# ducha-aiki/affnet

Hardware: AMD Instinct MI355X
Metric: keypoints/sec (detect+AffNet+OriNet+HardNet) per image, 2000 kp @1024x768 (higher is better)
Workload: dtype f32

## Files before the change

affnet_amd/_lib.py:

```python
import ctypes as C
import os

_HERE = os.path.dirname(os.path.abspath(__file__))
LIB_PATH = os.environ.get("AFFNET_HIP_LIB") or os.path.join(_HERE, "libaffnet_hip.so")
PROBES_LIB_PATH = os.path.join(_HERE, "libaffnet_hip_probes.so")

MAX_OCTAVES, MAX_LEVELS, MAX_TAPS = 16, 8, 37
NET_AFFNET, NET_ORINET, NET_HARDNET, NET_AFFNET_FULLCONV = 0, 1, 2, 3
ARITH_FP32_MFMA, ARITH_FP32_SPLIT3, ARITH_FP32_SPLIT2H = 0, 1, 2
ARITH_NAMES = {"fp32": ARITH_FP32_MFMA, "fp32_mfma": ARITH_FP32_MFMA, "fp32_split3": ARITH_FP32_SPLIT3, "split3": ARITH_FP32_SPLIT3,
               "fp32_split2h": ARITH_FP32_SPLIT2H, "split2h": ARITH_FP32_SPLIT2H}


def arith_code(arith):
    if arith is None:
        return ARITH_FP32_MFMA
    if isinstance(arith, str):
        if arith.lower() not in ARITH_NAMES:
            raise ValueError("arith must be one of %s" % sorted(ARITH_NAMES))
        return ARITH_NAMES[arith.lower()]
    if int(arith) not in (ARITH_FP32_MFMA, ARITH_FP32_SPLIT3, ARITH_FP32_SPLIT2H):
        raise ValueError("arith must be AFFNET_ARITH_FP32_MFMA (0), AFFNET_ARITH_FP32_SPLIT3 (1) or AFFNET_ARITH_FP32_SPLIT2H (2)")
    return int(arith)
SHAPE_FORM_DIRECT, SHAPE_FORM_WINOGRAD = 0, 1
DESC_FORM_DIRECT, DESC_FORM_POLYPHASE, DESC_FORM_F43 = 0, 1, 2
OK, ERR_INVALID, ERR_HIP, ERR_CAPACITY, ERR_EMPTY = 0, -1, -2, -3, -4


class Config(C.Structure):
    _fields_ = [
        ("height", C.c_int32), ("width", C.c_int32), ("n_octaves", C.c_int32), ("levels_per_octave", C.c_int32),
        ("oct_h", C.c_int32 * MAX_OCTAVES), ("oct_w", C.c_int32 * MAX_OCTAVES),
        ("level_sigma", (C.c_float * MAX_LEVELS) * MAX_OCTAVES),
        ("level_sigma4", (C.c_float * MAX_LEVELS) * MAX_OCTAVES),
        ("level_sigma_px", (C.c_double * MAX_LEVELS) * MAX_OCTAVES),
        ("first_blur_taps", C.c_int32), ("first_blur", C.c_float * (MAX_TAPS * MAX_TAPS)),
        ("level_blur_taps", C.c_int32 * MAX_LEVELS),
        ("level_blur", (C.c_float * (MAX_TAPS * MAX_TAPS)) * MAX_LEVELS),
        ("level_blur0_taps", C.c_int32 * MAX_LEVELS),
        ("level_blur0", (C.c_float * (MAX_TAPS * MAX_TAPS)) * MAX_LEVELS),
        ("lazy_shape_rows", C.c_int32),
        ("onepass", C.c_int32),
        ("mr_size", C.c_float), ("threshold", C.c_float),
        ("num_features", C.c_int32), ("num_prefilter", C.c_int32),
        ("max_raw_per_octave_div", C.c_int32), ("max_keep", C.c_int32), ("batch", C.c_int32), ("baum_iters", C.c_int32),
        ("arith", C.c_int32),
    ]


class Nets(C.Structure):
    _fields_ = [("d_affnet", C.c_void_p), ("d_orinet", C.c_void_p), ("d_hardnet", C.c_void_p),
                ("h_orientation_window", C.c_void_p), ("h_baumberg_window", C.c_void_p)]


_P, _I, _SZ = C.c_void_p, C.c_int, C.c_size_t
SYMBOLS = {
    "affnet_config_fill": (_I, [C.POINTER(Config), _I, _I, _I, C.c_double, _I, C.c_double, C.c_double, _I, _I, _I, _I]),
    "affnet_ctx_create": (_I, [C.POINTER(_P), _I, C.POINTER(Config)]),
    "affnet_ctx_destroy": (None, [_P]),
    "affnet_last_error": (C.c_char_p, [_P]),
    "affnet_version": (C.c_char_p, []),
    "affnet_set_arith": (_I, [_P, _I]),
    "affnet_get_arith": (_I, [_P]),
    "affnet_set_shape_form": (_I, [_P, _I]),
    "affnet_get_shape_form": (_I, [_P]),
    "affnet_set_desc_form": (_I, [_P, _I]),
    "affnet_get_desc_form": (_I, [_P]),
    "affnet_workspace_bytes": (_SZ, [_P]),
    "affnet_bind_workspace": (_I, [_P, _P, _SZ]),
    "affnet_pyramid_level_offset": (C.c_int64, [_P, _I, _I]),
    "affnet_pyramid_image_stride": (C.c_int64, [_P]),
    "affnet_batch": (_I, [_P]),
    "affnet_capacity_prefilter": (_I, [_P]),
    "affnet_capacity_final": (_I, [_P]),
    "affnet_gauss_blur": (_I, [_P, _P, _P, _I, _I, C.POINTER(C.c_float), _I, _P]),
    "affnet_pyramid_build": (_I, [_P, _P, _P]),
    "affnet_hessian_response": (_I, [_P, _P, _P, _I, _I, C.c_float, _P]),
    "affnet_detect": (_I, [_P, _P, _P, _P, _P, _P]),
    "affnet_detect_responses": (_I, [_P, _P, _P, _P, _P, _P, _P]),
    "affnet_laf_grid_sample": (_I, [_P, _P, _I, _I, _P, _I, _I, _P, _P]),
    "affnet_pyr_grid_sample": (_I, [_P, _P, _P, _P, _I, _I, _P, _P]),
    "affnet_cnn32_packed_floats": (_SZ, [_I]),
    "affnet_cnn32_winograd_offset": (C.c_int64, [_I, _I]),
    "affnet_cnn32_pack_weights": (_I, [_I, C.POINTER(_P), C.POINTER(_P), C.POINTER(_P), _P, _P, _P, _P, _P]),
    "affnet_cnn32_forward": (_I, [_P, _I, _P, _P, _P, _I, _P, _P, _P]),
    "affnet_cnn32_forward_pyr": (_I, [_P, _I, _P, _P, _P, _P, _I, _P, _P, _P]),
    "affnet_local_norm": (_I, [_P, _P, _P, _I, _I, _P]),
    "affnet_fullconv_scratch_bytes": (_SZ, [_I, _I]),
    "affnet_fullconv_forward": (_I, [_P, _P, _P, _I, _I, _P, _P, _P]),
    "affnet_nms2d": (_I, [_P, _P, _P, _I, _I, C.c_float, _P]),
    "affnet_shape_filter_select": (_I, [_P, _P, _P, _P, _P, _P, _P, _P, _P, _P, _P]),
    "affnet_apply_rotation": (_I, [_P, _P, _P, _P, _I, _P]),
    "affnet_scale_lafs": (_I, [_P, _P, _P, _P, _I, _I, _I, _I, _P]),
    "affnet_lafs_to_ellipses": (_I, [_P, _P, _P, _I, _P, _P]),
    "affnet_ellipses_to_lafs": (_I, [_P, _P, _P, _I, _P, _P]),
    "affnet_level_select": (_I, [_P, _P, _P, _I, _I, _P, _P, _P]),
    "affnet_handcrafted_forward": (_I, [_P, _I, _P, _I, _P, _P, _P, _P]),
    "affnet_handcrafted_forward_pyr": (_I, [_P, _I, _P, _P, _P, _I, _P, _P, _P]),
    "affnet_sift_host_window": (_I, [_I, C.POINTER(C.c_float)]),
    "affnet_sift_forward": (_I, [_P, _P, _I, _P, C.c_float, _P, _P]),
    "affnet_sift_forward_pyr": (_I, [_P, _P, _P, _P, _I, _P, C.c_float, _P, _P]),
    "affnet_tfeat_packed_floats": (_SZ, []),
    "affnet_tfeat_pack_weights": (_I, [_P, _P, _P, _P, _P, _P, _P]),
    "affnet_tfeat_scratch_floats": (_SZ, [_I]),
    "affnet_tfeat_forward": (_I, [_P, _P, _P, _P, _I, _P, _P, _P]),
    "affnet_tfeat_forward_pyr": (_I, [_P, _P, _P, _P, _P, _I, _P, _P, _P]),
    "affnet_match_scratch_bytes": (_SZ, [_I, _I]),
    "affnet_distance_matrix": (_I, [_P, _P, _I, _P, _I, _I, _P, _P, _P]),
    "affnet_match_snn": (_I, [_P, _P, _I, _P, _I, _I, C.c_float, _P, _P, _P, _P, _P, _P, _P]),
    "affnet_reproject_lafs": (_I, [_P, _P, _I, C.POINTER(C.c_float), _P, _P]),
    "affnet_centre_nn": (_I, [_P, _P, _I, _P, _I, _P, _P, _P]),
    "affnet_extract_features": (_I, [_P, C.POINTER(Nets), _P, _I, _P, _P, _P, _P, _P, _P]),
    "affnet_detect_image": (_I, [_P, _P, _P]),
    "affnet_detect_image_responses": (_I, [_P, _P, _P]),
    "affnet_detect_image_onepass": (_I, [_P, _P, _P, _P]),
    "affnet_detect_image_onepass_responses": (_I, [_P, _P, _P, _P]),
    "affnet_detected_list": (_I, [_P, _P, _P, _P, _P, _P]),
    "affnet_load_frames": (_I, [_P, _P, _I, _P, _P, _P, _I, _I, _P]),
    "affnet_describe_frames": (_I, [_P, C.POINTER(Nets), _P, _P, _P, _P, _I, _I, _P, _P, _P, _P, _P, _P]),
    "affnet_shape_iterate": (_I, [_P, _P, _P, _P, _P, _I, _P, _P]),
    "affnet_affmap_offset": (C.c_int64, [_P, _I]),
    "affnet_affmap_image_stride": (C.c_int64, [_P]),
    "affnet_describe_detected": (_I, [_P, C.POINTER(Nets), _I, _P, _P, _P, _P, _P, _P]),
    "affnet_graph_capture_extract": (_I, [_P, C.POINTER(Nets), _P, _I, _P, _P, _P, _P, _P, _P]),
    "affnet_graph_launch": (_I, [_P, _P]),
    "affnet_profile_enable": (_I, [_P, _I]),
    "affnet_profile_read": (_I, [_P, C.POINTER(C.c_double * 8), C.POINTER(C.c_int32)]),
    "affnet_read_counts": (_I, [_P, C.POINTER(C.c_int32 * 4), _P]),
    "affnet_counter_offset": (C.c_int64, [_P, _I]),
    "affnet_counter_stride": (C.c_int64, [_P]),
    "affnet_host_base_grid": (_I, [_I, C.POINTER(C.c_float)]),
}

DEBUG_SYMBOLS = {
    "affnet_cnn32_debug_timing": (_I, [_P, _P]),
    "affnet_cnn32_debug_layer": (_I, [_P, _I, _P, _P, _I, _P, _P]),
    "affnet_cnn32_debug_winograd_u": (_I, [_P, _I, _P, _I, _P, _P]),
    "affnet_selftest_mfma": (_I, [_P, _P, _P, _P]),
    "affnet_debug_split3_variant": (_I, [_P, _I]),
}

PROBE_SYMBOLS = {
    "affnet_cnn32_probe": (_I, [_P, _I, _I, _I, _I, _P, _P]),
    "affnet_split3_gemm": (_I, [_P, _P, _I, _I, _I, _I, _P, _P]),
    "affnet_split3_rate": (_I, [_I, _I, _I, _P, _P]),
    "affnet_debug_stream": (_I, [_P, _P, _SZ, _I, _I, _I, _P]),
    "affnet_probe_shape_offsets": (_I, [_P, C.POINTER(C.c_int64 * 3)]),
    "affnet_probe_affnet_wino_layer": (_I, [_P, _I, _P, _P, _I, _P, _P]),
    "affnet_probe_affnet_wino_partials": (_I, [_P, _P, _P, _I, _P, _P]),
    "affnet_probe_hardnet_poly_layer": (_I, [_P, _P, _P, _I, _P, _P]),
    "affnet_probe_hardnet_poly_forward": (_I, [_P, _P, _P, _I, _P, _P, _P]),
    "affnet_probe_hardnet_poly_u": (_I, [_P, _P, _I, _P, _P]),
    "affnet_probe_hardnet_f43_layer": (_I, [_P, _P, _P, _I, _P, _P]),
    "affnet_probe_hardnet_f43_forward": (_I, [_P, _P, _P, _I, _P, _P, _P]),
    "affnet_probe_hardnet_f43_u": (_I, [_P, _P, _I, _P, _P]),
}


class AffnetHipError(RuntimeError):
    pass


class AffnetEmptyError(AffnetHipError):
    """AFFNET_ERR_EMPTY: no image of the call produced a detection (the reference raises in torch.cat([]),
    SparseImgRepresenter.py:100)."""


def _load():
    if not os.path.isfile(LIB_PATH):
        if os.path.basename(LIB_PATH) == os.path.basename(PROBES_LIB_PATH):
            raise ImportError("affnet_amd: %s is missing - the tools under tools/ need the probe build of the library: "
                              "AFFNET_PROBES=1 bash affnet_amd/csrc/build.sh" % LIB_PATH)
        raise ImportError(
            "affnet_amd: %s is missing - the HIP extension is the only implementation of this path "
            "(no CPU fallback). Build it: bash affnet_amd/csrc/build.sh" % LIB_PATH)
    lib = C.CDLL(LIB_PATH)
    for table in (SYMBOLS, DEBUG_SYMBOLS):
        for name, (res, args) in table.items():
            fn = getattr(lib, name)
            fn.restype, fn.argtypes = res, args
    for name, (res, args) in PROBE_SYMBOLS.items():
        if hasattr(lib, name):
            fn = getattr(lib, name)
            fn.restype, fn.argtypes = res, args
    return lib


lib = _load()


def check(rc, ctx=None, what=""):
    if rc != OK:
        msg = lib.affnet_last_error(ctx).decode() if ctx else ""
        if rc == ERR_EMPTY:
            raise AffnetEmptyError("%s: %s" % (what or "libaffnet_hip call", msg))
        raise AffnetHipError("%s failed (code %d): %s" % (what or "libaffnet_hip call", rc, msg))


def ptr(t):
    return None if t is None else C.c_void_p(t.data_ptr())


def current_stream(device):
    import torch
    return C.c_void_p(torch.cuda.current_stream(device).cuda_stream)
```

affnet_amd/csrc/cnn32.hip:

```cpp
#include "common.h"

static void aff_fill_pyr_src(const affnet_ctx* ctx, PyrSrc* s) {
    memset(s, 0, sizeof(*s));
    if (ctx->ws) aff_fill_pyr_table(ctx, &s->t);
    aff_base_grid(32, s->base);
}

static int cnn_check(affnet_ctx* ctx, const CnnCall& c, int* rows) {
    *rows = 0;
    if (c.kind < 0 || c.kind > 2) return aff_fail(ctx, AFFNET_ERR_INVALID, "cnn32: unknown net kind %d", c.kind);
    if (!c.packed || !c.out || c.n_max < 0 || (!c.patches && (!c.lafs || !c.ids))) return aff_fail(ctx, AFFNET_ERR_INVALID, "cnn32: null argument");
    if (!c.patches && !ctx->ws) return aff_fail(ctx, AFFNET_ERR_INVALID, "cnn32: sampling from the pyramid needs a bound workspace");
    if (c.dbg_layer < 0 && !c.scratch)
        return aff_fail(ctx, AFFNET_ERR_INVALID, "cnn32: d_scratch is required (HardNet n*(8192+512) floats, AffNet / OriNet n*144 floats)");
    if (c.dbg_layer >= 0 && ctx->arith != AFFNET_ARITH_FP32_MFMA)
        return aff_fail(ctx, AFFNET_ERR_INVALID, "cnn32: layer dumps exist for AFFNET_ARITH_FP32_MFMA only (context is in arithmetic mode %d)", ctx->arith);
    if (c.n_max == 0) return AFFNET_OK;
    if (c.kind == AFFNET_NET_HARDNET && c.n_max > 65535)
        return aff_fail(ctx, AFFNET_ERR_INVALID, "cnn32: n_max=%d (HardNet head: max 65535 rows per image)", c.n_max);
    const int row_count = c.row_count < 0 ? c.n_max - c.row_begin : c.row_count;
    if (c.row_begin < 0 || row_count < 0 || c.row_begin + row_count > c.n_max) return aff_fail(ctx, AFFNET_ERR_INVALID, "cnn32: bad row window");
    *rows = row_count;
    return AFFNET_OK;
}

int aff_arith_index(const affnet_ctx* ctx) {
    return ctx->arith == AFFNET_ARITH_FP32_SPLIT2H ? 2 : (ctx->arith == AFFNET_ARITH_FP32_SPLIT3 ? 1 : 0);
}

static int trunk_launch(affnet_ctx* ctx, const CnnCall& c, const NetLayout& L, dim3 grid, bool wino, const int32_t* reeval, int shape_op) {
    CnnArgs a;
    a.packed = c.packed; a.off = to_offsets(L, ctx->arith);
    a.wino_u = nullptr; a.reeval = reeval;
    if ((c.kind == AFFNET_NET_ORINET || wino) && ctx->arith == AFFNET_ARITH_FP32_MFMA) {
        const int rc = aff_wino_derive_u(ctx, c.kind, c.packed, L, c.st, &a.wino_u);
        if (rc) return rc;
    }
    const bool poly = c.desc_form != AFFNET_DESC_FORM_DIRECT && c.kind == AFFNET_NET_HARDNET && ctx->arith == AFFNET_ARITH_FP32_MFMA;
    const bool f43 = poly && c.desc_form == AFFNET_DESC_FORM_F43;
    if (poly) {
        int rc = aff_poly_derive_u(ctx, c.packed, L, c.st, &a.wino_u);
        if (!rc && f43) rc = aff_f43_derive_u(ctx, c.packed, L, c.st);
        if (rc) return rc;
    }
    a.patches = c.patches; a.lafs = c.lafs; a.ids = c.ids; a.count = c.count; a.n_max = c.n_max;
    a.out = (c.dbg_layer < 0) ? c.scratch : c.out;
    a.dbg_layer = c.dbg_layer; a.dbg_out = c.dbg_out; a.dbg_time = ctx->dbg_time;
    a.row_begin = c.row_begin; a.skip_cnt = c.skip_cnt; a.skip_n = c.skip_n;
    a.shape_cnt = (c.fuse && shape_op) ? c.fuse->cnt : nullptr; a.shape_op = shape_op;
    a.s3_alt = ctx->split3_variant;
    PyrSrc ps;
    aff_fill_pyr_src(ctx, &ps);
    static_assert(AFFNET_NET_AFFNET == 0 && AFFNET_NET_ORINET == 1 && AFFNET_NET_HARDNET == 2, "trunk getter order");
    static TrunkKernel (*const trunk_of[3])(int, bool) = {aff_trunk_affnet, aff_trunk_orinet, aff_trunk_hardnet};
    const bool stamps = a.dbg_time || c.dbg_layer >= 0;
    hipLaunchKernelGGL(wino ? aff_trunk_affnet_wino(stamps) : (poly ? (f43 ? aff_trunk_hardnet_f43(stamps) : aff_trunk_hardnet_poly(stamps)) : trunk_of[c.kind](aff_arith_index(ctx), stamps)), grid, dim3(512), 0, c.st, a, ps);
    AFF_LAUNCH_CHECK(ctx);
    return AFFNET_OK;
}

static int cnn_launch(affnet_ctx* ctx, const CnnCall& c) {
    int rows;
    int rc = cnn_check(ctx, c, &rows);
    if (rc || rows == 0) return rc;
    const NetLayout L = net_layout(c.kind);
    const int B = c.patches ? 1 : ctx->B;
    const bool form1 = c.wino_reeval && c.kind == AFFNET_NET_AFFNET && c.fuse && c.dbg_layer < 0 && ctx->arith == AFFNET_ARITH_FP32_MFMA;
    rc = trunk_launch(ctx, c, L, dim3(rows, B), form1, nullptr, c.shape_op);
    if (rc) return rc;
    if (form1) {
        int32_t* flags = reinterpret_cast<int32_t*>(c.scratch + (size_t)B * c.n_max * HEAD_PART_AFF);
        rc = aff_margin_affnet(ctx, c, L, rows, B, flags);
        if (rc) return rc;
        rc = trunk_launch(ctx, c, L, dim3(rows, B), false, flags, 0);
        if (rc) return rc;
    }
    if (c.dbg_layer < 0 && c.kind != AFFNET_NET_HARDNET) {
        rc = c.kind == AFFNET_NET_AFFNET ? aff_finish_affnet(ctx, c, L, rows, B) : aff_finish_orinet(ctx, c, L, rows, B);
        if (rc) return rc;
    }
    if (c.mark_head) aff_prof_mark(ctx, 7, c.st);
    if (c.dbg_layer < 0 && c.kind == AFFNET_NET_HARDNET) return aff_hardnet_head(ctx, c, L, B);
    return AFFNET_OK;
}

extern "C" int affnet_cnn32_forward(affnet_ctx* ctx, int net_kind, const float* d_packed, const float* d_patches, const int32_t* d_count,
                                    int n_max, float* d_out, float* d_scratch, void* stream) {
    AFF_DEVICE(ctx);
    if (!ctx || !d_patches) return aff_fail(ctx, AFFNET_ERR_INVALID, "cnn32_forward: null argument");
    CnnCall c;
    c.kind = net_kind; c.packed = d_packed; c.patches = d_patches; c.count = d_count; c.n_max = n_max; c.out = d_out; c.scratch = d_scratch; c.st = (hipStream_t)stream;
    return cnn_launch(ctx, c);
}

extern "C" int affnet_cnn32_forward_pyr(affnet_ctx* ctx, int net_kind, const float* d_packed, const float* d_lafs, const int32_t* d_ids,
                                        const int32_t* d_count, int n_max, float* d_out, float* d_scratch, void* stream) {
    AFF_DEVICE(ctx);
    if (!ctx) return AFFNET_ERR_INVALID;
    CnnCall c;
    c.kind = net_kind; c.packed = d_packed; c.lafs = d_lafs; c.ids = d_ids; c.count = d_count; c.n_max = n_max; c.out = d_out; c.scratch = d_scratch; c.st = (hipStream_t)stream;
    return cnn_launch(ctx, c);
}

int aff_affnet_filter_rows(affnet_ctx* ctx, const float* packed, const float* resp, const float* lafs, const int32_t* ids, const int32_t* count,
                           float* out, float* scratch, int row_begin, int row_count, bool lazy, int shape_op, hipStream_t st) {
    ShapeFuse sf;
    sf.resp = resp; sf.lafs = lafs; sf.key = ctx->st_key; sf.good = ctx->st_good; sf.cnt = ctx->cnt;
    CnnCall c;
    c.kind = AFFNET_NET_AFFNET; c.packed = packed; c.lafs = lafs; c.ids = ids; c.count = count; c.n_max = ctx->cap_pre; c.out = out; c.scratch = scratch; c.st = st;
    c.row_begin = row_begin; c.row_count = row_count;
    c.skip_cnt = lazy ? ctx->cnt : nullptr; c.skip_n = ctx->cfg.num_features;
    c.fuse = &sf; c.shape_op = shape_op;
    c.wino_reeval = ctx->shape_form == AFFNET_SHAPE_FORM_WINOGRAD;
    return cnn_launch(ctx, c);
}

int aff_orinet_rotate(affnet_ctx* ctx, const float* packed, float* lafs, const int32_t* ids, const int32_t* count, int n_max, float* out, float* scratch,
                      hipStream_t st, const DenormSel* denorm) {
    CnnCall c;
    c.kind = AFFNET_NET_ORINET; c.packed = packed; c.lafs = lafs; c.ids = ids; c.count = count; c.n_max = n_max; c.out = out; c.scratch = scratch; c.st = st;
    c.rot_lafs = lafs; c.denorm = denorm;
    return cnn_launch(ctx, c);
}

int aff_hardnet_forward_pyr_marked(affnet_ctx* ctx, const float* packed, const float* lafs, const int32_t* ids, const int32_t* count,
                                   int n_max, float* out, float* scratch, hipStream_t st) {
    CnnCall c;
    c.kind = AFFNET_NET_HARDNET; c.packed = packed; c.lafs = lafs; c.ids = ids; c.count = count; c.n_max = n_max; c.out = out; c.scratch = scratch; c.st = st;
    c.mark_head = true;
    c.desc_form = ctx->cfg.onepass ? AFFNET_DESC_FORM_DIRECT : ctx->desc_form;
    return cnn_launch(ctx, c);
}

int aff_hardnet_poly_patches(affnet_ctx* ctx, const float* packed, const float* patches, int n, float* out, float* scratch, int dbg_layer, hipStream_t st, int form) {
    if (ctx->arith != AFFNET_ARITH_FP32_MFMA) return aff_fail(ctx, AFFNET_ERR_INVALID, "hardnet_poly: AFFNET_ARITH_FP32_MFMA only");
    CnnCall c;
    c.kind = AFFNET_NET_HARDNET; c.packed = packed; c.patches = patches; c.n_max = n; c.out = out; c.scratch = scratch; c.st = st;
    c.dbg_layer = dbg_layer; c.dbg_out = dbg_layer >= 0 ? out : nullptr;
    c.desc_form = form;
    return cnn_launch(ctx, c);
}

extern "C" int affnet_debug_split3_variant(affnet_ctx* ctx, int bits) {
    if (!ctx) return AFFNET_ERR_INVALID;
    ctx->split3_variant = bits;
    return AFFNET_OK;
}

extern "C" int affnet_cnn32_debug_timing(affnet_ctx* ctx, unsigned long long* d_stamps) {
    if (!ctx) return AFFNET_ERR_INVALID;
    ctx->dbg_time = d_stamps;
    return AFFNET_OK;
}

extern "C" int affnet_cnn32_debug_layer(affnet_ctx* ctx, int net_kind, const float* d_packed, const float* d_patch, int layer, float* d_out,
                                        void* stream) {
    AFF_DEVICE(ctx);
    if (!ctx || !d_patch || !d_out || layer < 0 || layer > 5) return aff_fail(ctx, AFFNET_ERR_INVALID, "cnn32_debug_layer: bad argument");
    CnnCall c;
    c.kind = net_kind; c.packed = d_packed; c.patches = d_patch; c.n_max = 1; c.out = d_out; c.st = (hipStream_t)stream;
    c.dbg_layer = layer; c.dbg_out = d_out;
    return cnn_launch(ctx, c);
}

extern "C" int affnet_cnn32_debug_winograd_u(affnet_ctx* ctx, int net_kind, const float* d_packed, int layer, float* d_out, void* stream) {
    AFF_DEVICE(ctx);
    if (!ctx || !d_packed || !d_out || (net_kind != AFFNET_NET_AFFNET && net_kind != AFFNET_NET_ORINET) || (layer != 1 && layer != 3 && layer != 5))
        return aff_fail(ctx, AFFNET_ERR_INVALID, "cnn32_debug_winograd_u: AffNet / OriNet, layer 1, 3 or 5");
    const float* u;
    const int rc = aff_wino_derive_u(ctx, net_kind, d_packed, net_layout(net_kind), (hipStream_t)stream, &u);
    if (rc) return rc;
    return aff_copy_async(ctx, d_out, u + Wino16::offset(layer), (size_t)Wino16::floats(layer) * sizeof(float), (hipStream_t)stream);
}
```

affnet_amd/csrc/cnn_mfma.h:

```cpp
#pragma once
#include <math.h>
#include <stdlib.h>

#include <utility>

#include "common.h"
#include "weights_layout.h"

typedef float f32x4 __attribute__((ext_vector_type(4)));

typedef __attribute__((address_space(3))) const f32x4 LdsF4;
__device__ __forceinline__ unsigned lds_byte_addr(const float* p) {
    return (unsigned)(size_t)(__attribute__((address_space(3))) const float*)p;
}
__device__ __forceinline__ f32x4 lds_read4(unsigned byte_addr) { return *(LdsF4*)(size_t)byte_addr; }

typedef unsigned u32x4 __attribute__((ext_vector_type(4)));
__device__ __forceinline__ __amdgpu_buffer_rsrc_t weight_rsrc(const float* base, int n_floats) {
    return __builtin_amdgcn_make_buffer_rsrc(const_cast<float*>(base), 0, n_floats * 4, 0x00020000);
}
__device__ __forceinline__ f32x4 buf_read4(__amdgpu_buffer_rsrc_t r, int lane_byte_off, int uniform_byte_off) {
    return __builtin_bit_cast(f32x4, __builtin_amdgcn_raw_buffer_load_b128(r, lane_byte_off, uniform_byte_off, 0));
}

// ... 1280 lines not shown
    static constexpr int U_HALF = 8 * 4 * 16 * 64 * 4;
};
__device__ __forceinline__ void wino5_prefetch_u(const float* __restrict__ Wu, f32x4 (&U)[4], int wave, int lane) {
    const __amdgpu_buffer_rsrc_t r = weight_rsrc(Wu, 16 * 64 * 64);
    const int u_lane = ((lane >> 4) * 64 + (wave >> 1) * 16 + (lane & 15)) * 16 + (wave & 1) * Wino5::U_HALF;
#pragma unroll
    for (int k = 0; k < 4; ++k) U[k] = wino_load_u<64, 64>(r, u_lane, k, 0);
}

template <int NW, typename LI>
__device__ __forceinline__ void conv3x3_wino_mfma_half_rows(const float* act, const float* __restrict__ Wu, f32x4 (&U)[4], f32x4 (&acc)[2][4], int wave, int lane) {
    constexpr int CIN = 64, COUT = 64, NGRP = CIN / 16, NSTEP = 2 * NGRP;
    static_assert(NW == 8 && LI::H == 8, "one tile block; a wave pair per channel block");
    const int m = lane & 15, kq = lane >> 4, p = wave >> 1;
    const __amdgpu_buffer_rsrc_t wrsrc = weight_rsrc(Wu, 16 * CIN * COUT);
    const int u_lane = (kq * COUT + p * 16 + m) * 16;
    const unsigned a0 = lds_byte_addr(act) + ((kq * LI::PSG + (2 * (m >> 2) * LI::WP + 2 * (m & 3)) * 4) * 4);
    auto rows = [&](auto hc) {
        constexpr int H2 = decltype(hc)::v;
#pragma unroll
        for (int s = 0; s < NSTEP; ++s) {
            const int il = s / NGRP, i = 2 * H2 + il, G = s % NGRP;
            const int sn = s + 1 < NSTEP ? s + 1 : s;
            const int in = 2 * H2 + sn / NGRP, Gn = sn % NGRP;
            unsigned ab = a0 + 4 * G * LI::PSG * 4;
            asm("" : "+v"(ab));
            f32x4 da[4], db[4], V[4];
            wino_read_rows<LI>(ab, i, da, db);
            wino_transform_row(i, da, db, V);
            if (G == 0) {
#pragma unroll
                for (int k = 0; k < 4; ++k) acc[il][k] = (f32x4){0.f, 0.f, 0.f, 0.f};
            }
            __builtin_amdgcn_sched_barrier(0);
#pragma unroll
            for (int k = 0; k < 4; k += 2) {
#pragma unroll
                for (int s4 = 0; s4 < 4; ++s4) {
                    acc[il][k] = __builtin_amdgcn_mfma_f32_16x16x4f32(U[k][s4], V[k][s4], acc[il][k], 0, 0, 0);
                    acc[il][k + 1] = __builtin_amdgcn_mfma_f32_16x16x4f32(U[k + 1][s4], V[k + 1][s4], acc[il][k + 1], 0, 0, 0);
                }
                U[k] = wino_load_u<CIN, COUT>(wrsrc, u_lane, 4 * in + k, Gn);
                U[k + 1] = wino_load_u<CIN, COUT>(wrsrc, u_lane, 4 * in + k + 1, Gn);
                __builtin_amdgcn_sched_barrier(0);
            }
        }
    };
    if ((wave & 1) == 0) rows(IntC<0>{}); else rows(IntC<1>{});
}

__device__ __forceinline__ void wino5_combine(float* lds, const f32x4 (&acc)[2][4], f32x4 (&y)[2], int wave, int lane) {
    const int h = wave & 1;
    float* xw = lds + Wino5::X + (wave * 4 * 64 + lane) * 4;
    const float* xr = lds + Wino5::X + ((wave ^ 1) * 4 * 64 + lane) * 4;
    if (h == 0) {
#pragma unroll
        for (int j = 0; j < 4; ++j) *reinterpret_cast<f32x4*>(&xw[j * 256]) = acc[1][j];
    } else {
#pragma unroll
        for (int j = 0; j < 4; ++j) *reinterpret_cast<f32x4*>(&xw[j * 256]) = acc[0][j];
    }
    __syncthreads();
    f32x4 o[4], t[4];
#pragma unroll
    for (int j = 0; j < 4; ++j) o[j] = *reinterpret_cast<const f32x4*>(&xr[j * 256]);
    if (h == 0) {
#pragma unroll
        for (int j = 0; j < 4; ++j)
#pragma unroll
            for (int e = 0; e < 4; ++e) t[j][e] = wadd(wadd(acc[0][j][e], acc[1][j][e]), o[j][e]);
    } else {
#pragma unroll
        for (int j = 0; j < 4; ++j)
#pragma unroll
            for (int e = 0; e < 4; ++e) t[j][e] = wsub(wsub(o[j][e], acc[0][j][e]), acc[1][j][e]);
    }
#pragma unroll
    for (int e = 0; e < 4; ++e) {
        y[0][e] = wadd(wadd(t[0][e], t[1][e]), t[2][e]);
        y[1][e] = wsub(wsub(t[1][e], t[2][e]), t[3][e]);
    }
}

template <int ROW, int PIX, int GRP>
__device__ __forceinline__ void wino5_store_lds(float* dst, f32x4 bias, const f32x4 (&y)[2], int wave, int lane) {
    const int m = lane & 15, oy = 2 * (m >> 2) + (wave & 1), ox = 2 * (m & 3);
#pragma unroll
    for (int k = 0; k < 2; ++k) {
        const f32x4 v = bias_relu(y[k], bias);
        *reinterpret_cast<f32x4*>(&dst[(oy * ROW + ox + k) * PIX + ((wave >> 1) * 4 + (lane >> 4)) * GRP]) = v;
    }
}

template <int NW, int H, int COUT, int NB>
__device__ __forceinline__ void wino_bias(const float* __restrict__ bias, f32x4 (&bv)[NB], int wave, int lane) {
#pragma unroll
    for (int q = 0; q < NB; ++q) {
        int ty, tx, cb;
        wino_tile<H, COUT, NB>(wave, q, lane & 15, ty, tx, cb);
        bv[q] = *reinterpret_cast<const f32x4*>(&bias[cb * 16 + 4 * (lane >> 4)]);
    }
}

template <int COUT, typename LO, int NB>
__device__ __forceinline__ void wino_store_lds(float* act, const f32x4 (&bias)[NB], const f32x4 (&y)[NB][4], int wave, int lane) {
    const int g = lane >> 4;
#pragma unroll
    for (int q = 0; q < NB; ++q) {
        int ty, tx, cb;
        wino_tile<LO::H, COUT, NB>(wave, q, lane & 15, ty, tx, cb);
#pragma unroll
        for (int k = 0; k < 4; ++k) {
            const int oy = 2 * ty + (k >> 1), ox = 2 * tx + (k & 1);
            const f32x4 v = bias_relu(y[q][k], bias[q]);
            *reinterpret_cast<f32x4*>(&act[(cb * 4 + g) * LO::PSG + ((oy + 1) * LO::WP + ox + 1) * 4]) = v;
        }
    }
}

template <int COUT, int H, int NB>
__device__ __forceinline__ void wino_store_global(float* __restrict__ dst, const f32x4 (&bias)[NB], const f32x4 (&y)[NB][4], int wave, int lane) {
    const int g = lane >> 4;
#pragma unroll
    for (int q = 0; q < NB; ++q) {
        int ty, tx, cb;
        wino_tile<H, COUT, NB>(wave, q, lane & 15, ty, tx, cb);
#pragma unroll
        for (int k = 0; k < 4; ++k) {
            const int p = (2 * ty + (k >> 1)) * H + 2 * tx + (k & 1);
            const f32x4 v = bias_relu(y[q][k], bias[q]);
            *reinterpret_cast<f32x4*>(dst + p * COUT + cb * 16 + 4 * g) = v;
        }
    }
}

constexpr int poly_row_np(int r) { return (r < 3 || (r >= 6 && r < 8)) ? 3 : 2; }
constexpr int poly_row_xi0(int r) { return r < 3 ? 3 * r : (r < 6 ? 9 + 2 * (r - 3) : (r < 8 ? 15 + 3 * (r - 6) : 21 + 2 * (r - 8))); }
constexpr bool poly_row_oddy(int r) { return r < 6; }
constexpr int poly_row_yi(int r) { return r < 3 ? r : (r < 6 ? r - 3 : (r < 8 ? r - 6 : r - 8)); }
constexpr int poly_row_ra(int r) { return poly_row_oddy(r) ? (poly_row_yi(r) == 0 ? 0 : 2) : 1 + 2 * poly_row_yi(r); }
constexpr int poly_row_rb(int r) { return (poly_row_oddy(r) && poly_row_yi(r) != 1) ? (poly_row_yi(r) == 0 ? 2 : 4) : -1; }
constexpr int poly_row_reads(int r) { return poly_row_np(r) * (poly_row_rb(r) >= 0 ? 2 : 1); }
constexpr int poly_row_valu(int r) { return 4 * ((poly_row_rb(r) >= 0 ? poly_row_np(r) : 0) + (poly_row_np(r) == 3 ? 2 : 0)); }

template <int... I, typename F>
__device__ __forceinline__ void static_for_seq(std::integer_sequence<int, I...>, F&& f) { (f(IntC<I>{}), ...); }
template <int N, typename F>
__device__ __forceinline__ void static_for(F&& f) { static_for_seq(std::make_integer_sequence<int, N>{}, f); }

template <typename LI, int R>
__device__ __forceinline__ void poly_read_row(unsigned ab, f32x4 (&da)[3], f32x4 (&db)[3]) {
    constexpr int NC = poly_row_np(R), C0 = NC == 3 ? 0 : 1, RA = poly_row_ra(R), RB = poly_row_rb(R);
#pragma unroll
    for (int c = 0; c < NC; ++c) {
        da[c] = lds_read4(ab + (RA * LI::WP + C0 + 2 * c) * 16);
        if constexpr (RB >= 0) db[c] = lds_read4(ab + (RB * LI::WP + C0 + 2 * c) * 16);
    }
}

template <int R>
__device__ __forceinline__ void poly_transform_row(const f32x4 (&da)[3], const f32x4 (&db)[3], f32x4 (&V)[3]) {
    constexpr int NC = poly_row_np(R), RB = poly_row_rb(R);
#pragma unroll
    for (int e = 0; e < 4; ++e) {
        float t[3];
#pragma unroll
        for (int c = 0; c < NC; ++c) t[c] = RB >= 0 ? wsub(da[c][e], db[c][e]) : da[c][e];
        if constexpr (NC == 3) { V[0][e] = wsub(t[0], t[1]); V[1][e] = t[1]; V[2][e] = wsub(t[1], t[2]); }
        else { V[0][e] = t[0]; V[1][e] = t[1]; }
    }
}

template <int NW, int CIN, int COUT, int HOUT, int NB, int NCB>
__device__ __forceinline__ void poly_prefetch_u(const float* __restrict__ Wu, f32x4 (&Ua)[NCB][3], f32x4 (&Ub)[NCB][3], int wave, int lane) {
    constexpr int NGRP = CIN / 16;
    const __amdgpu_buffer_rsrc_t r = weight_rsrc(Wu, POLY_XI * CIN * COUT);
    const int u_lane = wino_u_lane<HOUT, COUT, NB>(wave, 0, lane);
    constexpr int R1 = 1 / NGRP, G1 = 1 % NGRP;
#pragma unroll
    for (int k = 0; k < 3; ++k)
#pragma unroll
        for (int c = 0; c < NCB; ++c) {
            Ua[c][k] = wino_load_u<CIN, COUT>(r, u_lane, k, 0, c);
            if (k < poly_row_np(R1)) Ub[c][k] = wino_load_u<CIN, COUT>(r, u_lane, poly_row_xi0(R1) + k, G1, c);
        }
}

template <int NW, int CIN, int COUT, typename LI, int NB, int NCB>
__device__ __forceinline__ void conv3x3_poly_mfma_rows(const float* act, const float* __restrict__ Wu, f32x4 (&Ua)[NCB][3], f32x4 (&Ub)[NCB][3], f32x4 (&y)[NB][4],
                                                       int wave, int lane) {
    constexpr int HOUT = LI::H / 2, HT = HOUT / 2, NGRP = CIN / 16, NSTEP = (NB / NCB) * 10 * NGRP;
    static_assert(LI::H % 4 == 0 && (HT * HT) % 16 == 0 && COUT % 16 == 0 && CIN % 16 == 0, "polyphase tiling");
    static_assert((HT * HT / 16) * (COUT / 16) == NW * NB, "the waves' passes must tile the layer exactly");
    static_assert((NCB == 1 || NCB == 2) && NB % NCB == 0 && (COUT / 16) % NCB == 0 && NSTEP % 2 == 0, "the passes of a unit must share their tile block");
    const int m = lane & 15, kq = lane >> 4;
    const __amdgpu_buffer_rsrc_t wrsrc = weight_rsrc(Wu, POLY_XI * CIN * COUT);
    f32x4 t0[NCB][5], t1[NCB][5], acc[NCB][3], Va[3], Vb[3];
    auto window_addr = [&](int u, int G) {
        int ty, tx, cb;
        wino_tile<HOUT, COUT, NB>(wave, NCB * u, m, ty, tx, cb);
        unsigned ab = lds_byte_addr(act) + (((4 * G + kq) * LI::PSG + (4 * ty * LI::WP + 4 * tx) * 4) * 4);
        asm("" : "+v"(ab));
        return ab;
    };
    auto step = [&](auto sc, const f32x4 (&V)[3], f32x4 (&Vn)[3], f32x4 (&U)[NCB][3]) {
        constexpr int S = decltype(sc)::v;
        constexpr int u = S / (10 * NGRP), R = (S / NGRP) % 10, G = S % NGRP;
        constexpr bool more = S + 1 < NSTEP;
        constexpr int Sn = more ? S + 1 : S, un = Sn / (10 * NGRP), Rn = (Sn / NGRP) % 10, Gn = Sn % NGRP;
        constexpr int S2 = S + 2 < NSTEP ? S + 2 : S, u2 = S2 / (10 * NGRP), R2 = (S2 / NGRP) % 10, G2 = S2 % NGRP;
        constexpr int NP = poly_row_np(R), NP2 = poly_row_np(R2), XI2 = poly_row_xi0(R2);
        constexpr int NM = NP * 4 * NCB, NRn = more ? poly_row_reads(Rn) : 0, VPM = NCB == 2 ? 2 : 4, NVM = more ? (poly_row_valu(Rn) + VPM - 1) / VPM : 0;
        static_assert(NM >= NRn + NVM, "the next step's reads and transform fit between this step's MFMAs");
        const int u_next = wino_u_lane<HOUT, COUT, NB>(wave, NCB * u2, lane);
        unsigned abn = 0;
        if constexpr (more) abn = window_addr(un, Gn);
        if constexpr (G == 0) {
#pragma unroll
            for (int c = 0; c < NCB; ++c)
#pragma unroll
                for (int k = 0; k < NP; ++k) acc[c][k] = (f32x4){0.f, 0.f, 0.f, 0.f};
        }
        __builtin_amdgcn_sched_barrier(0);
        f32x4 da[3], db[3];
        if constexpr (more) poly_read_row<LI, Rn>(abn, da, db);
        if constexpr (NCB == 2) {
#pragma unroll
            for (int k = 0; k < NP; ++k) {
#pragma unroll
                for (int s4 = 0; s4 < 4; ++s4) {
                    acc[0][k] = __builtin_amdgcn_mfma_f32_16x16x4f32(U[0][k][s4], V[k][s4], acc[0][k], 0, 0, 0);
                    acc[1][k] = __builtin_amdgcn_mfma_f32_16x16x4f32(U[1][k][s4], V[k][s4], acc[1][k], 0, 0, 0);
                }
#pragma unroll
                for (int k2 = k; k2 < (k == NP - 1 ? 3 : k + 1); ++k2)
                    if (k2 < NP2) {
                        U[0][k2] = wino_load_u<CIN, COUT>(wrsrc, u_next, XI2 + k2, G2, 0);
                        U[1][k2] = wino_load_u<CIN, COUT>(wrsrc, u_next, XI2 + k2, G2, 1);
                    }
            }
        } else {
#pragma unroll
            for (int s4 = 0; s4 < 4; ++s4)
#pragma unroll
                for (int k = 0; k < NP; ++k) acc[0][k] = __builtin_amdgcn_mfma_f32_16x16x4f32(U[0][k][s4], V[k][s4], acc[0][k], 0, 0, 0);
#pragma unroll
            for (int k2 = 0; k2 < NP2; ++k2) U[0][k2] = wino_load_u<CIN, COUT>(wrsrc, u_next, XI2 + k2, G2, 0);
        }
        if constexpr (more) poly_transform_row<Rn>(da, db, Vn);
#pragma unroll
        for (int mi = 0; mi < NM; ++mi) {
            __builtin_amdgcn_sched_group_barrier(0x008, 1, 0);
            if (mi < NRn) __builtin_amdgcn_sched_group_barrier(0x100, 1, 0);
            if (mi >= NM - NVM) __builtin_amdgcn_sched_group_barrier(0x002, VPM, 0);
            if (NCB == 2 && (mi + 1) % 8 == 0) {
                const int k = mi / 8;
                if (k < NP2) __builtin_amdgcn_sched_group_barrier(0x020, 2, 0);
                if (k == NP - 1 && NP2 > NP) __builtin_amdgcn_sched_group_barrier(0x020, 2, 0);
            }
            if (NCB == 1 && mi == NM - 1) __builtin_amdgcn_sched_group_barrier(0x020, NP2 == 3 ? 3 : 2, 0);
        }
        __builtin_amdgcn_sched_barrier(0);
        if constexpr (G == NGRP - 1) {
            constexpr int C0 = NP == 3 ? 0 : 3, yi = poly_row_yi(R);
#pragma unroll
            for (int c = 0; c < NCB; ++c) {
#pragma unroll
                for (int j = 0; j < NP; ++j)
#pragma unroll
                    for (int e = 0; e < 4; ++e) {
                        if constexpr (poly_row_oddy(R)) {
                            if (yi == 0) t0[c][C0 + j][e] = acc[c][j][e];
                            else if (yi == 1) { t0[c][C0 + j][e] = wadd(t0[c][C0 + j][e], acc[c][j][e]); t1[c][C0 + j][e] = acc[c][j][e]; }
                            else t1[c][C0 + j][e] = wsub(t1[c][C0 + j][e], acc[c][j][e]);
                        } else {
                            if (yi == 0) t0[c][C0 + j][e] = wadd(t0[c][C0 + j][e], acc[c][j][e]);
                            else t1[c][C0 + j][e] = wadd(t1[c][C0 + j][e], acc[c][j][e]);
                        }
                    }
                if constexpr (R == 9) {
#pragma unroll
                    for (int e = 0; e < 4; ++e) {
                        y[NCB * u + c][0][e] = wadd(wadd(t0[c][0][e], t0[c][1][e]), t0[c][3][e]);
                        y[NCB * u + c][1][e] = wadd(wsub(t0[c][1][e], t0[c][2][e]), t0[c][4][e]);
                        y[NCB * u + c][2][e] = wadd(wadd(t1[c][0][e], t1[c][1][e]), t1[c][3][e]);
                        y[NCB * u + c][3][e] = wadd(wsub(t1[c][1][e], t1[c][2][e]), t1[c][4][e]);
                    }
                }
            }
            __builtin_amdgcn_sched_barrier(0);
        }
    };
    {
        f32x4 da[3], db[3];
        poly_read_row<LI, 0>(window_addr(0, 0), da, db);
        poly_transform_row<0>(da, db, Va);
    }
    static_for<NSTEP / 2>([&](auto hc) {
        constexpr int S = 2 * decltype(hc)::v;
        step(IntC<S>{}, Va, Vb, Ua);
        step(IntC<S + 1>{}, Vb, Va, Ub);
    });
}
```

affnet_amd/csrc/cnn_trunk.h:

```cpp
#pragma once
#include <math.h>

#include <type_traits>

#include "common.h"

#include "cnn_mfma.h"

template <int TM>
__device__ __forceinline__ void head_partials(const float* __restrict__ hw, const f32x4 (&bias)[1], const f32x4 (&acc)[TM][1],
                                              float* __restrict__ part, int wave, int lane) {
    constexpr int MT = 4, MG = MT / TM;
    const int mg = wave % MG, ng = wave / MG;
    const int n = lane & 15, g = lane >> 4;
    const int c4 = ng * 16 + 4 * g;
    f32x4 v[TM];
#pragma unroll
    for (int i = 0; i < TM; ++i) v[i] = bias_relu(acc[i][0], bias[0]);
    const __amdgpu_buffer_rsrc_t r = weight_rsrc(hw, 3 * 4096);
    f32x4 w[3][TM];
#pragma unroll
    for (int o = 0; o < 3; ++o)
#pragma unroll
        for (int i = 0; i < TM; ++i) w[o][i] = buf_read4(r, (n * 64 + c4) * 4, (o * 4096 + (mg * TM + i) * 16 * 64) * 4);
#pragma unroll
    for (int o = 0; o < 3; ++o) {
        float sacc = 0.f;
#pragma unroll
        for (int i = 0; i < TM; ++i)
#pragma unroll
            for (int j = 0; j < 4; ++j) sacc = fmaf(v[i][j], w[o][i][j], sacc);
        sacc = wave_sum(sacc);
        if (lane == 0) part[wave * 4 + o] = sacc;
    }
}

__device__ __forceinline__ void aff_head_weights_wino(const float* __restrict__ hw, f32x4 (&w)[3][2], int wave, int lane) {
    const __amdgpu_buffer_rsrc_t r = weight_rsrc(hw, 3 * 4096);
    const int m = lane & 15, c4 = (wave >> 1) * 16 + 4 * (lane >> 4);
    const int pix = (2 * (m >> 2) + (wave & 1)) * 8 + 2 * (m & 3);
#pragma unroll
    for (int o = 0; o < 3; ++o)
#pragma unroll
        for (int k = 0; k < 2; ++k) w[o][k] = buf_read4(r, (pix * 64 + c4) * 4, (o * 4096 + k * 64) * 4);
}
__device__ __forceinline__ void head_partials_wino(const f32x4 (&w)[3][2], f32x4 bias, const f32x4 (&y)[2], float* __restrict__ part, int wave, int lane) {
    f32x4 v[2];
#pragma unroll
    for (int k = 0; k < 2; ++k) v[k] = bias_relu(y[k], bias);
#pragma unroll
    for (int o = 0; o < 3; ++o) {
        float sacc = 0.f;
#pragma unroll
        for (int k = 0; k < 2; ++k)
#pragma unroll
            for (int j = 0; j < 4; ++j) sacc = fmaf(v[k][j], w[o][k][j], sacc);
        sacc = wave_sum(sacc);
        if (lane == 0) part[wave * 4 + o] = sacc;
    }
}

#define ORI_HP 68
struct OriHeadLane {
    int mg, n, c4;
    template <int TM>
    __device__ __forceinline__ static OriHeadLane of(int wave, int lane) {
        constexpr int MT = 4, MG = MT / TM;
        const int mg = wave % MG, ng = wave / MG;
        const int n = lane & 15, g = lane >> 4;
        return {mg, n, ng * 16 + 4 * g};
    }
};
template <int TM>
__device__ __forceinline__ void ori_head_weights(const float* __restrict__ hw, const OriHeadLane& L, f32x4 (&w)[2][TM]) {
    const __amdgpu_buffer_rsrc_t r = weight_rsrc(hw, 2 * 4096);
#pragma unroll
    for (int o = 0; o < 2; ++o)
#pragma unroll
        for (int i = 0; i < TM; ++i) w[o][i] = buf_read4(r, (L.n * 64 + L.c4) * 4, (o * 4096 + (L.mg * TM + i) * 16 * 64) * 4);
}
template <int NTHR>
__device__ __forceinline__ void ori_head_zero_halo(float* act, int tid) {
    for (int e = tid; e < 36 * 16; e += NTHR) {
        const int hp = e >> 4, q4 = e & 15;
        const int y = hp < 10 ? 0 : (hp < 20 ? 9 : 1 + ((hp - 20) >> 1)), x = hp < 10 ? hp : (hp < 20 ? hp - 10 : ((hp - 20) & 1) * 9);
        *reinterpret_cast<f32x4*>(&act[(y * 10 + x) * ORI_HP + 4 * q4]) = (f32x4){0.f, 0.f, 0.f, 0.f};
    }
}
template <int TM>
__device__ __forceinline__ void ori_head_pbase(const OriHeadLane& L, int (&pbase)[TM]) {
#pragma unroll
    for (int i = 0; i < TM; ++i) {
        const int p = (L.mg * TM + i) * 16 + L.n;
        pbase[i] = ((p >> 3) * 10 + (p & 7)) * ORI_HP + L.c4;
    }
}
template <int TM>
__device__ __forceinline__ void ori_head_reduce(const f32x4 (&w)[2][TM], const int (&pbase)[TM], float* __restrict__ part, const float* act, int wave, int lane) {
    __syncthreads();
#pragma unroll
    for (int q = 0; q < 9; ++q) {
        float s0 = 0.f, s1 = 0.f;
#pragma unroll
        for (int i = 0; i < TM; ++i) {
            const f32x4 av = *reinterpret_cast<const f32x4*>(&act[pbase[i] + ((q / 3) * 10 + q % 3) * ORI_HP]);
#pragma unroll
            for (int j = 0; j < 4; ++j) { s0 = fmaf(av[j], w[0][i][j], s0); s1 = fmaf(av[j], w[1][i][j], s1); }
        }
        s0 = wave_sum(s0);
        s1 = wave_sum(s1);
        if (lane == 0) { part[wave * 18 + q] = s0; part[wave * 18 + 9 + q] = s1; }
    }
}
template <int TM, int NTHR>
__device__ __forceinline__ void head_partials_ori_lds(const float* __restrict__ hw, const f32x4 (&bias)[1], const f32x4 (&acc)[TM][1],
                                                      float* __restrict__ part, float* act, int wave, int lane, int tid) {
    constexpr int MT = 4, MG = MT / TM;
    const int mg = wave % MG, ng = wave / MG;
    const int n = lane & 15, g = lane >> 4;
    const int c4 = ng * 16 + 4 * g;
    f32x4 v[TM];
#pragma unroll
    for (int i = 0; i < TM; ++i) v[i] = bias_relu(acc[i][0], bias[0]);
    const __amdgpu_buffer_rsrc_t r = weight_rsrc(hw, 2 * 4096);
    f32x4 w[2][TM];
#pragma unroll
    for (int o = 0; o < 2; ++o)
#pragma unroll
        for (int i = 0; i < TM; ++i) w[o][i] = buf_read4(r, (n * 64 + c4) * 4, (o * 4096 + (mg * TM + i) * 16 * 64) * 4);
    __syncthreads();
    ori_head_zero_halo<NTHR>(act, tid);
    int pbase[TM];
#pragma unroll
    for (int i = 0; i < TM; ++i) {
        const int p = (mg * TM + i) * 16 + n;
        pbase[i] = ((p >> 3) * 10 + (p & 7)) * ORI_HP + c4;
        *reinterpret_cast<f32x4*>(&act[pbase[i] + 11 * ORI_HP]) = v[i];
    }
    ori_head_reduce<TM>(w, pbase, part, act, wave, lane);
}

#define CNN_STAMP(k)                                                                                     \
    do {                                                                                                 \
        if (STAMPS && a.dbg_time && lane == 0) a.dbg_time[((size_t)pidx * NW + wave) * 32 + (k)] = __builtin_readcyclecounter(); \
    } while (0)

template <int CB>
struct TrunkLds {
    static constexpr int ACT = (CB / 4) * LayC0::PSG;
    static constexpr int PATCH = WP32 * WP32;
    static constexpr int RED = 256;
    static constexpr int TOTAL = ACT + PATCH + RED;
};

template <int KIND, int NW>
struct TrunkShape {
    static constexpr int CB = (KIND == AFFNET_NET_HARDNET) ? 32 : 16;
    static constexpr int NTHR = NW * 64;
    static constexpr int T1M = (CB == 16) ? 8 : 64 / NW, T1N = CB / 16;
    static constexpr int T2M = (CB == 16) ? 4 : 64 / NW, T2N = 1;
    static constexpr int T4M = (CB == 16) ? 2 : 32 / NW, T4N = 1;
    static constexpr int AREG = (NW == 8 && CB == 32) ? 128 : 48;
    static constexpr int G2 = pick_groups(CB, T2M, T2N, 32, AREG), G3 = pick_groups(2 * CB, T2M, T2N, 32, AREG);
    static constexpr int G4 = pick_groups(2 * CB, T4M, T4N, 32, AREG), G5 = pick_groups(4 * CB, T4M, T4N, 32, AREG);
};

template <int C, typename L, int NTHR>
__device__ __forceinline__ void dump_planes(const float* act, float* dst) {
    constexpr int H = L::H;
    for (int i = threadIdx.x; i < C * H * H; i += NTHR) {
        const int c = i / (H * H), r = i - c * H * H, y = r / H, x = r - y * H;
        dst[i] = act[L::at(c, y, x)];
    }
}

template <int CB>
struct SplitLays {
    typedef LayQ<16, 32, 34, CB, 0, 3> LQH;
    typedef LayQ<16, 32, 34, CB, 16, 3> LQH2;
    using LR0 = LayR<32, 32, 34, CB, 0>;
    using LR0H = LayR<16, 32, 34, CB, 0, 34>;
    using LR1 = LayR<32, 32, 34, CB, 16>;
    using LR1H = LayR<16, 32, 34, CB, 16, 34>;
    static_assert(LR0::BYTES <= TrunkLds<CB>::ACT * 4 && LR1::BYTES <= TrunkLds<CB>::ACT * 4 && LR0H::GS == LR0::GS && LR1H::GS == LR1::GS, "whole-patch split layouts");
    static_assert(LQH::BYTES <= TrunkLds<CB>::ACT * 4 && LQH2::BYTES <= TrunkLds<CB>::ACT * 4, "pre-split layouts must fit the activation buffer");
};

template <int KIND, int NW, bool STAMPS, int S3 = 0>
__global__ __launch_bounds__(NW * 64, (KIND == AFFNET_NET_HARDNET) ? NW / 4 : 4) void cnn32_trunk_kernel(CnnArgs a, PyrSrc ps) {
    static_assert(S3 == 0 || S3 == 2 || S3 == 3 || (S3 == 1 && KIND != AFFNET_NET_ORINET) || (S3 == 4 && KIND == AFFNET_NET_HARDNET),
                  "S3 = number of terms of the split arithmetic; 1 = exact AffNet with Winograd conv1 / conv3 / conv5, exact HardNet with polyphase conv2 / conv4; "
                  "4 = exact HardNet as 1 with conv3 as Winograd F(4x4, 3x3)");
    constexpr bool EXACT = S3 <= 1 || S3 == 4;
    constexpr bool WINO13 = (S3 == 0 && KIND == AFFNET_NET_ORINET) || (S3 == 1 && KIND == AFFNET_NET_AFFNET);
    constexpr bool WINO5 = WINO13;
    constexpr bool POLY = (S3 == 1 || S3 == 4) && KIND == AFFNET_NET_HARDNET;
    constexpr bool F43_1 = false;
    constexpr bool F43_3 = S3 == 4 && KIND == AFFNET_NET_HARDNET;
    static_assert(!F43_1, "conv1 in F(4x4, 3x3) has no loop yet");
    using S = TrunkShape<KIND, NW>;
    constexpr int CB = S::CB, NTHR = S::NTHR;
    static_assert((CB / 4) * LayC1::PSG <= TrunkLds<CB>::ACT && (CB / 2) * LayC3::PSG <= TrunkLds<CB>::ACT, "LDS layout");
    __shared__ __attribute__((aligned(16))) float lds[TrunkLds<CB>::TOTAL];
    float* act = lds;
    float* patch = lds + TrunkLds<CB>::ACT;
    float* red = patch + TrunkLds<CB>::PATCH;
    const int n = a.count ? min(a.count[blockIdx.y], a.n_max) : a.n_max;
    const int prow = blockIdx.x + a.row_begin;
    if (KIND == AFFNET_NET_AFFNET && a.shape_cnt && blockIdx.x == 0 && threadIdx.x == 0) {
        int32_t* c = a.shape_cnt + (size_t)blockIdx.y * CNT_TOTAL;
        if (a.shape_op == 1) { c[CNT_SURVIVED] = 0; c[CNT_SURVIVED1] = 0; c[CNT_AFF_EVAL] = 0; c[CNT_AFF_REEVAL] = 0; }
        else if (a.shape_op == 2) c[CNT_SURVIVED1] = c[CNT_SURVIVED];
    }
    if (prow >= n || lazy_skip(a.skip_cnt, a.skip_n, blockIdx.y, CNT_SURVIVED)) return;
    const size_t pidx = (size_t)blockIdx.y * a.n_max + prow;
    if (KIND == AFFNET_NET_AFFNET && a.reeval && a.reeval[pidx] == 0) return;
    const int tid = threadIdx.x, wave = tid >> 6, lane = tid & 63;
    if (KIND == AFFNET_NET_HARDNET) __builtin_amdgcn_s_setprio(3);
    CNN_STAMP(0);
    if (STAMPS && a.dbg_time && lane == 0) {
        a.dbg_time[((size_t)pidx * NW + wave) * 32 + 14] = __builtin_amdgcn_s_getreg((31 << 11) | 4);
        a.dbg_time[((size_t)pidx * NW + wave) * 32 + 15] = __builtin_amdgcn_s_getreg((31 << 11) | 20);
    }
    float w0[3][S::T1N];
    f32x4 bias0[S::T1N];
    conv0_load_w<NW, CB, S::T1M, S::T1N>(a.packed + a.off.w[0], a.packed + a.off.b[0], w0, bias0, wave, lane);
    f32x4 b1[1][S::T1N];
    f32x4 Ur[4];
    if constexpr (S3 == 0 && KIND == AFFNET_NET_AFFNET) prefetch_b0<NW, CB, 32, S::T1M, S::T1N, 1>(a.packed + a.off.w[1], b1, wave, lane);
    if constexpr (WINO13) wino_prefetch_u_row<NW, CB, CB, 32, Wino16::NB1>(a.wino_u, Ur, wave, lane);

    constexpr int PPT = 1024 / NTHR;
    constexpr int RPT = 32 / PPT;
    float v[PPT];
    if (a.patches) {
        const float* src = a.patches + pidx * 1024;
#pragma unroll
        for (int q = 0; q < PPT; ++q) v[q] = src[tid + q * NTHR];
    } else {
        int o = a.ids[3 * pidx], l = a.ids[3 * pidx + 1];
        o = o < 0 ? 0 : (o >= ps.t.n_octaves ? ps.t.n_octaves - 1 : o);
        l = l < 0 ? 0 : (l >= ps.t.n_levels ? ps.t.n_levels - 1 : l);
        const float* img = ps.t.lvl[o][l] + blockIdx.y * ps.t.img_stride;
        const int h = ps.t.h[o], w = ps.t.w[o];
        const float* L = a.lafs + 6 * pidx;
        const float m = (float)(h < w ? h : w);
        const float t00 = L[0] * m, t01 = L[1] * m, t02 = L[2] * (float)w;
        const float t10 = L[3] * m, t11 = L[4] * m, t12 = L[5] * (float)h;
#pragma unroll
        for (int q = 0; q < PPT; ++q)
            v[q] = aff_sample_bilinear(img, h, w, t00, t01, t02, t10, t11, t12, ps.base[tid & 31], ps.base[(tid >> 5) + q * RPT]);
    }
    CNN_STAMP(16);
    if (tid < 4 * 33) {
        const int e = tid;
        const int y = e < 34 ? 0 : (e < 68 ? 33 : 1 + ((e - 68) >> 1)), x = e < 34 ? e : (e < 68 ? e - 34 : ((e - 68) & 1) * 33);
        patch[y * WP32 + x] = 0.0f;
    }
    if constexpr (EXACT) zero_halo<LayC0, NTHR>(act, CB);
    else if constexpr (S3 == 2) zero_halo_q<typename SplitLays<CB>::LR0, NTHR>(act);
    else zero_halo_q<typename SplitLays<CB>::LQH, NTHR>(act);
    float sum = 0.f;
#pragma unroll
    for (int q = 0; q < PPT; ++q) sum += v[q];
    const float mean = block_sum<NW>(sum, red) * (1.0f / 1024.0f);
    CNN_STAMP(17);
    float sq = 0.f;
#pragma unroll
    for (int q = 0; q < PPT; ++q) { v[q] -= mean; sq += v[q] * v[q]; }
    const float var = block_sum<NW>(sq, red + NW) * (1.0f / 1023.0f);
    const float sd = sqrtf(var) + 1e-7f;
    CNN_STAMP(18);
#pragma unroll
    for (int q = 0; q < PPT; ++q) patch[((tid >> 5) + q * RPT + 1) * WP32 + (tid & 31) + 1] = v[q] / sd;
    __syncthreads();
    CNN_STAMP(1);

    if constexpr (EXACT && KIND == AFFNET_NET_HARDNET) {
        constexpr int T1M = S::T1M, T1N = S::T1N, T2M = S::T2M, T2N = S::T2N, T4M = S::T4M, T4N = S::T4N;
        constexpr int NB1 = (16 * 16 / 16) * (CB / 16) / NW, NB3 = (8 * 8 / 16) * (2 * CB / 16) / NW, NB5 = (4 * 4 / 16) * (4 * CB / 16) / NW;
        constexpr int NBP2 = (8 * 8 / 16) * (2 * CB / 16) / NW, NBP4 = (4 * 4 / 16) * (4 * CB / 16) / NW;

        f32x4 Up[2][4];
        f32x4 Uw[16];
        f32x4 Uf[18];
        {
            f32x4 acc[T1M][T1N];
            conv0_mfma<NW, CB, T1M, T1N>(patch, w0, bias0, acc, wave, lane);
            CNN_STAMP(19);
            store_tiles_lds<CB, LayC0, T1M, T1N, false>(act, bias0, acc, wave, lane);
            CNN_STAMP(20);
            wino_prefetch_u_pair<NW, CB, CB, 32, NB1>(a.packed + a.off.w_wino[0], Up, wave, lane);
            __syncthreads();
        }
        if (STAMPS && a.dbg_layer == 0) { dump_planes<CB, LayC0, NTHR>(act, a.dbg_out); return; }
        CNN_STAMP(2);

        f32x4 b2[S::G2][T2N];
        f32x4 bias2[T2N];
        f32x4 P2a[2][3], P2b[2][3];
        {
            f32x4 y[NB1][4], bw[NB1];
            __builtin_amdgcn_s_setprio(0);
            conv3x3_wino_mfma_pair_rows<NW, CB, CB, LayC0, NB1>(act, a.packed + a.off.w_wino[0], Up, y, wave, lane);
            __builtin_amdgcn_s_setprio(3);
            CNN_STAMP(3);
            if constexpr (POLY) poly_prefetch_u<NW, CB, 2 * CB, 16, NBP2, 2>(a.wino_u + Poly32::offset(2), P2a, P2b, wave, lane);
            else {
                prefetch_b0<NW, 2 * CB, 16, T2M, T2N, S::G2>(a.packed + a.off.w[2], b2, wave, lane);
                prefetch_bias<NW, 16, T2M, T2N>(a.packed + a.off.b[2], bias2, wave, lane);
            }
            wino_bias<NW, 32, CB, NB1>(a.packed + a.off.b[1], bw, wave, lane);
            __syncthreads();
            CNN_STAMP(21);
            zero_halo<LayC1, NTHR>(act, CB);
            wino_store_lds<CB, LayC1, NB1>(act, bw, y, wave, lane);
            CNN_STAMP(22);
            __syncthreads();
            CNN_STAMP(4);
        }
        if (STAMPS && a.dbg_layer == 1) { dump_planes<CB, LayC1, NTHR>(act, a.dbg_out); return; }

        if constexpr (POLY) {
            f32x4 y[NBP2][4], bw[NBP2];
            __builtin_amdgcn_s_setprio(0);
            conv3x3_poly_mfma_rows<NW, CB, 2 * CB, LayC1, NBP2, 2>(act, a.wino_u + Poly32::offset(2), P2a, P2b, y, wave, lane);
            __builtin_amdgcn_s_setprio(3);
            CNN_STAMP(5);
            if constexpr (F43_3) f43_prefetch_u<2 * CB, 2 * CB>(a.wino_u + F43::BASE + F43::offset(3), Uf, wave, lane);
            else wino_prefetch_u_pair<NW, 2 * CB, 2 * CB, 16, NB3>(a.packed + a.off.w_wino[1], Up, wave, lane);
            wino_bias<NW, 16, 2 * CB, NBP2>(a.packed + a.off.b[2], bw, wave, lane);
            __syncthreads();
            zero_halo<LayC2, NTHR>(act, 2 * CB);
            wino_store_lds<2 * CB, LayC2, NBP2>(act, bw, y, wave, lane);
            __syncthreads();
            CNN_STAMP(6);
        } else {
            f32x4 acc[T2M][T2N];
            __builtin_amdgcn_s_setprio(0);
            conv3x3_mfma<NW, CB, 2 * CB, LayC1, 2, T2M, T2N, S::G2>(act, a.packed + a.off.w[2], b2, acc, wave, lane);
            __builtin_amdgcn_s_setprio(3);
            CNN_STAMP(5);
            wino_prefetch_u_pair<NW, 2 * CB, 2 * CB, 16, NB3>(a.packed + a.off.w_wino[1], Up, wave, lane);
            __syncthreads();
            zero_halo<LayC2, NTHR>(act, 2 * CB);
            store_tiles_lds<2 * CB, LayC2, T2M, T2N>(act, bias2, acc, wave, lane);
            __syncthreads();
            CNN_STAMP(6);
        }
        if (STAMPS && a.dbg_layer == 2) { dump_planes<2 * CB, LayC2, NTHR>(act, a.dbg_out); return; }

        f32x4 b4[S::G4][T4N];
        f32x4 bias4[T4N];
        f32x4 P4a[1][3], P4b[1][3];
        if constexpr (F43_3) {
            static_assert(F43L::V_FLOATS <= TrunkLds<CB>::ACT && F43L::X + F43L::X_FLOATS <= F43L::V_FLOATS, "conv3: V of the layer fits the activation buffer");
            f32x4 tf[3][4], y[8];
            __builtin_amdgcn_s_setprio(0);
            conv3x3_f43_mfma_shared_v<NW, 2 * CB, 2 * CB, LayC2>(act, a.wino_u + F43::BASE + F43::offset(3), Uf, tf, wave, lane);
            __builtin_amdgcn_s_setprio(3);
            CNN_STAMP(23);
            poly_prefetch_u<NW, 2 * CB, 4 * CB, 8, NBP4, 1>(a.wino_u + Poly32::offset(4), P4a, P4b, wave, lane);
            const f32x4 bf = *reinterpret_cast<const f32x4*>(&a.packed[a.off.b[3] + (wave >> 1) * 16 + 4 * (lane >> 4)]);
            __syncthreads();
            f43_combine(act, tf, y, wave, lane);
            CNN_STAMP(7);
            __syncthreads();
            zero_halo<LayC3, NTHR>(act, 2 * CB);
            f43_store_lds<LayC3>(act, bf, y, wave, lane);
            __syncthreads();
            CNN_STAMP(8);
        } else {
            f32x4 y[NB3][4], bw[NB3];
            __builtin_amdgcn_s_setprio(0);
            conv3x3_wino_mfma_pair_rows<NW, 2 * CB, 2 * CB, LayC2, NB3>(act, a.packed + a.off.w_wino[1], Up, y, wave, lane);
            __builtin_amdgcn_s_setprio(3);
            CNN_STAMP(7);
            if constexpr (POLY) poly_prefetch_u<NW, 2 * CB, 4 * CB, 8, NBP4, 1>(a.wino_u + Poly32::offset(4), P4a, P4b, wave, lane);
            else {
                prefetch_b0<NW, 4 * CB, 8, T4M, T4N, S::G4>(a.packed + a.off.w[4], b4, wave, lane);
                prefetch_bias<NW, 8, T4M, T4N>(a.packed + a.off.b[4], bias4, wave, lane);
            }
            wino_bias<NW, 16, 2 * CB, NB3>(a.packed + a.off.b[3], bw, wave, lane);
            __syncthreads();
            zero_halo<LayC3, NTHR>(act, 2 * CB);
            wino_store_lds<2 * CB, LayC3, NB3>(act, bw, y, wave, lane);
            __syncthreads();
            CNN_STAMP(8);
        }
        if (STAMPS && a.dbg_layer == 3) { dump_planes<2 * CB, LayC3, NTHR>(act, a.dbg_out); return; }

        if constexpr (POLY) {
            f32x4 y[NBP4][4], bw[NBP4];
            __builtin_amdgcn_s_setprio(0);
            conv3x3_poly_mfma_rows<NW, 2 * CB, 4 * CB, LayC3, NBP4, 1>(act, a.wino_u + Poly32::offset(4), P4a, P4b, y, wave, lane);
            __builtin_amdgcn_s_setprio(3);
            CNN_STAMP(9);
            wino_prefetch_u<NW, 4 * CB, 4 * CB, 8, NB5>(a.packed + a.off.w_wino[2], Uw, wave, lane);
            wino_bias<NW, 8, 4 * CB, NBP4>(a.packed + a.off.b[4], bw, wave, lane);
            __syncthreads();
            zero_halo<LayC4, NTHR>(act, 4 * CB);
            wino_store_lds<4 * CB, LayC4, NBP4>(act, bw, y, wave, lane);
            __syncthreads();
            CNN_STAMP(10);
        } else {
            f32x4 acc[T4M][T4N];
            __builtin_amdgcn_s_setprio(0);
            conv3x3_mfma<NW, 2 * CB, 4 * CB, LayC3, 2, T4M, T4N, S::G4>(act, a.packed + a.off.w[4], b4, acc, wave, lane);
            __builtin_amdgcn_s_setprio(3);
            CNN_STAMP(9);
            wino_prefetch_u<NW, 4 * CB, 4 * CB, 8, NB5>(a.packed + a.off.w_wino[2], Uw, wave, lane);
            __syncthreads();
            zero_halo<LayC4, NTHR>(act, 4 * CB);
            store_tiles_lds<4 * CB, LayC4, T4M, T4N>(act, bias4, acc, wave, lane);
            __syncthreads();
            CNN_STAMP(10);
        }
        if (STAMPS && a.dbg_layer == 4) { dump_planes<4 * CB, LayC4, NTHR>(act, a.dbg_out); return; }

        f32x4 y[NB5][4], bw[NB5];
        __builtin_amdgcn_s_setprio(0);
        static_assert(NB5 == 1 && (4 * CB / 16) * 4096 <= TrunkLds<CB>::ACT, "conv5: one pass per wave, V of the layer fits the activation buffer");
        conv3x3_wino_mfma_shared_v<NW, 4 * CB, 4 * CB, LayC4>(act, a.packed + a.off.w_wino[2], Uw, y, wave, lane);
        __builtin_amdgcn_s_setprio(3);
        CNN_STAMP(11);
        wino_bias<NW, 8, 4 * CB, NB5>(a.packed + a.off.b[5], bw, wave, lane);
        if (!STAMPS || a.dbg_layer < 0) {
            wino_store_global<4 * CB, 8, NB5>(a.out + pidx * (64 * 4 * CB), bw, y, wave, lane);
            CNN_STAMP(13);
            return;
        }
        __syncthreads();
        wino_store_lds<4 * CB, LayC5, NB5>(act, bw, y, wave, lane);
        __syncthreads();
        CNN_STAMP(12);
        if (STAMPS && a.dbg_layer == 5) { dump_planes<4 * CB, LayC5, NTHR>(act, a.dbg_out); return; }
    } else if constexpr (EXACT) {
        constexpr int T1M = S::T1M, T1N = S::T1N, T2M = S::T2M, T2N = S::T2N, T4M = S::T4M, T4N = S::T4N;
        static_assert(NW == 8 && CB == 16, "Wino16 describes the 16-channel trunks on 8 waves");
        constexpr int NB1 = Wino16::NB1, NB3 = Wino16::NB3;
        static_assert(WINO13 || T1M * 8 > S::AREG, "conv1: two A sets of T1M float4 do not fit -> rolling single set (conv3x3_mfma_roll)");
        f32x4 b4[S::G4][T4N];
        f32x4 bias4[T4N];
        f32x4 bias1[T1N];
        f32x4 b3[S::G3][T2N];
        f32x4 bias3[T2N];
        {
            f32x4 acc[T1M][T1N];
            conv0_mfma<NW, CB, T1M, T1N>(patch, w0, bias0, acc, wave, lane);
            CNN_STAMP(19);
            if constexpr (!WINO13) prefetch_bias<NW, 32, T1M, T1N>(a.packed + a.off.b[1], bias1, wave, lane);
            store_tiles_lds<CB, LayC0, T1M, T1N, false>(act, bias0, acc, wave, lane);
            CNN_STAMP(20);
            __syncthreads();
        }
        if (STAMPS && a.dbg_layer == 0) { dump_planes<CB, LayC0, NTHR>(act, a.dbg_out); return; }
        CNN_STAMP(2);

        f32x4 b2[S::G2][T2N];
        f32x4 bias2[T2N];
        if constexpr (WINO13) {
            f32x4 y[NB1][4], bw[NB1];
            conv3x3_wino_mfma_rows<NW, CB, CB, LayC0, NB1>(act, a.wino_u, Ur, y, wave, lane);
            CNN_STAMP(3);
            prefetch_b0<NW, 2 * CB, 16, T2M, T2N, S::G2>(a.packed + a.off.w[2], b2, wave, lane);
            prefetch_bias<NW, 16, T2M, T2N>(a.packed + a.off.b[2], bias2, wave, lane);
            wino_bias<NW, 32, CB, NB1>(a.packed + a.off.b[1], bw, wave, lane);
            __syncthreads();
            CNN_STAMP(21);
            zero_halo<LayC1, NTHR>(act, CB);
            wino_store_lds<CB, LayC1, NB1>(act, bw, y, wave, lane);
            CNN_STAMP(22);
            __syncthreads();
            CNN_STAMP(4);
        } else {
            f32x4 acc[T1M][T1N];
            conv3x3_mfma_roll<NW, CB, CB, LayC0, 1, T1M, T1N>(act, a.packed + a.off.w[1], b1, acc, wave, lane);
            CNN_STAMP(3);
            prefetch_b0<NW, 2 * CB, 16, T2M, T2N, S::G2>(a.packed + a.off.w[2], b2, wave, lane);
            prefetch_bias<NW, 16, T2M, T2N>(a.packed + a.off.b[2], bias2, wave, lane);
            __syncthreads();
            CNN_STAMP(21);
            zero_halo<LayC1, NTHR>(act, CB);
            store_tiles_lds<CB, LayC1, T1M, T1N>(act, bias1, acc, wave, lane);
            CNN_STAMP(22);
            __syncthreads();
            CNN_STAMP(4);
        }
        if (STAMPS && a.dbg_layer == 1) { dump_planes<CB, LayC1, NTHR>(act, a.dbg_out); return; }

        {
            f32x4 acc[T2M][T2N];
            conv3x3_mfma<NW, CB, 2 * CB, LayC1, 2, T2M, T2N, S::G2>(act, a.packed + a.off.w[2], b2, acc, wave, lane);
            CNN_STAMP(5);
            if constexpr (WINO13) wino_prefetch_u_row<NW, 2 * CB, 2 * CB, 16, NB3>(a.wino_u + Wino16::offset(3), Ur, wave, lane);
            else {
                prefetch_b0<NW, 2 * CB, 16, T2M, T2N, S::G3>(a.packed + a.off.w[3], b3, wave, lane);
                prefetch_bias<NW, 16, T2M, T2N>(a.packed + a.off.b[3], bias3, wave, lane);
            }
            __syncthreads();
            zero_halo<LayC2, NTHR>(act, 2 * CB);
            store_tiles_lds<2 * CB, LayC2, T2M, T2N>(act, bias2, acc, wave, lane);
            __syncthreads();
            CNN_STAMP(6);
        }
        if (STAMPS && a.dbg_layer == 2) { dump_planes<2 * CB, LayC2, NTHR>(act, a.dbg_out); return; }

        if constexpr (WINO13) {
            f32x4 y[NB3][4], bw[NB3];
            conv3x3_wino_mfma_rows<NW, 2 * CB, 2 * CB, LayC2, NB3>(act, a.wino_u + Wino16::offset(3), Ur, y, wave, lane);
            CNN_STAMP(7);
            prefetch_b0<NW, 4 * CB, 8, T4M, T4N, S::G4>(a.packed + a.off.w[4], b4, wave, lane);
            prefetch_bias<NW, 8, T4M, T4N>(a.packed + a.off.b[4], bias4, wave, lane);
            wino_bias<NW, 16, 2 * CB, NB3>(a.packed + a.off.b[3], bw, wave, lane);
            __syncthreads();
            zero_halo<LayC3, NTHR>(act, 2 * CB);
            wino_store_lds<2 * CB, LayC3, NB3>(act, bw, y, wave, lane);
            __syncthreads();
            CNN_STAMP(8);
        } else {
            f32x4 acc[T2M][T2N];
            conv3x3_mfma<NW, 2 * CB, 2 * CB, LayC2, 1, T2M, T2N, S::G3>(act, a.packed + a.off.w[3], b3, acc, wave, lane);
            CNN_STAMP(7);
            prefetch_b0<NW, 4 * CB, 8, T4M, T4N, S::G4>(a.packed + a.off.w[4], b4, wave, lane);
            prefetch_bias<NW, 8, T4M, T4N>(a.packed + a.off.b[4], bias4, wave, lane);
            __syncthreads();
            zero_halo<LayC3, NTHR>(act, 2 * CB);
            store_tiles_lds<2 * CB, LayC3, T2M, T2N>(act, bias3, acc, wave, lane);
            __syncthreads();
            CNN_STAMP(8);
        }
        if (STAMPS && a.dbg_layer == 3) { dump_planes<2 * CB, LayC3, NTHR>(act, a.dbg_out); return; }

        f32x4 b5[S::G5][T4N];
        f32x4 bias5[T4N];
        {
            f32x4 acc[T4M][T4N];
            conv3x3_mfma<NW, 2 * CB, 4 * CB, LayC3, 2, T4M, T4N, S::G4>(act, a.packed + a.off.w[4], b4, acc, wave, lane);
            CNN_STAMP(9);
            if constexpr (WINO5) {
                wino5_prefetch_u(a.wino_u + Wino16::offset(5), Ur, wave, lane);
            } else {
                prefetch_b0<NW, 4 * CB, 8, T4M, T4N, S::G5>(a.packed + a.off.w[5], b5, wave, lane);
                prefetch_bias<NW, 8, T4M, T4N>(a.packed + a.off.b[5], bias5, wave, lane);
            }
            __syncthreads();
            zero_halo<LayC4, NTHR>(act, 4 * CB);
            store_tiles_lds<4 * CB, LayC4, T4M, T4N>(act, bias4, acc, wave, lane);
            __syncthreads();
            CNN_STAMP(10);
        }
        if (STAMPS && a.dbg_layer == 4) { dump_planes<4 * CB, LayC4, NTHR>(act, a.dbg_out); return; }

        static_assert(!WINO5 || (Wino5::X >= 16 * LayC4::PSG && Wino5::X + Wino5::X_FLOATS <= TrunkLds<CB>::TOTAL),
                      "Winograd conv5: the exchange lies behind conv4's output inside the LDS array");
        if constexpr (WINO5) {
            constexpr bool ORI = KIND == AFFNET_NET_ORINET;
            static_assert(T4M == 2, "hw: one weight vector per (output, pixel tile) for OriNet, per (output, fragment pixel) for AffNet");
            static_assert(!ORI || Wino5::HEAD + 100 * ORI_HP <= Wino5::X, "conv5: the head copy in front of the exchange");
            f32x4 acc[2][4], y[2], hw[ORI ? 2 : 3][2];
            conv3x3_wino_mfma_half_rows<NW, LayC4>(act, a.wino_u + Wino16::offset(5), Ur, acc, wave, lane);
            CNN_STAMP(11);
            const f32x4 bw = *reinterpret_cast<const f32x4*>(&a.packed[a.off.b[5] + (wave >> 1) * 16 + 4 * (lane >> 4)]);
            const OriHeadLane HL = OriHeadLane::of<T4M>(wave, lane);
            if (!STAMPS || a.dbg_layer < 0) {
                if constexpr (ORI) ori_head_weights<T4M>(a.packed + a.off.head_w, HL, hw);
                else aff_head_weights_wino(a.packed + a.off.head_w, hw, wave, lane);
            }
            wino5_combine(lds, acc, y, wave, lane);
            if (!STAMPS || a.dbg_layer < 0) {
                if constexpr (ORI) {
                    float* copy = lds + Wino5::HEAD;
                    ori_head_zero_halo<NTHR>(copy, tid);
                    wino5_store_lds<10, ORI_HP, 4>(copy + 11 * ORI_HP, bw, y, wave, lane);
                    int pbase[T4M];
                    ori_head_pbase<T4M>(HL, pbase);
                    ori_head_reduce<T4M>(hw, pbase, a.out + pidx * HEAD_PART_ORI, copy, wave, lane);
                } else {
                    head_partials_wino(hw, bw, y, a.out + pidx * HEAD_PART_AFF, wave, lane);
                }
                CNN_STAMP(13);
                return;
            }
            __syncthreads();
            wino5_store_lds<LayC5::WP, 4, LayC5::PSG>(act + (LayC5::WP + 1) * 4, bw, y, wave, lane);
            __syncthreads();
            CNN_STAMP(12);
            if (STAMPS && a.dbg_layer == 5) { dump_planes<4 * CB, LayC5, NTHR>(act, a.dbg_out); return; }
            return;
        }
        f32x4 acc[T4M][T4N];
        conv3x3_mfma<NW, 4 * CB, 4 * CB, LayC4, 1, T4M, T4N, S::G5>(act, a.packed + a.off.w[5], b5, acc, wave, lane);
        CNN_STAMP(11);
        if (!STAMPS || a.dbg_layer < 0) {
            head_partials<T4M>(a.packed + a.off.head_w, bias5, acc, a.out + pidx * HEAD_PART_AFF, wave, lane);
            CNN_STAMP(13);
            return;
        }
        __syncthreads();
        store_tiles_lds<4 * CB, LayC5, T4M, T4N>(act, bias5, acc, wave, lane);
        __syncthreads();
        CNN_STAMP(12);
        if (STAMPS && a.dbg_layer == 5) { dump_planes<4 * CB, LayC5, NTHR>(act, a.dbg_out); return; }
    } else if constexpr (KIND == AFFNET_NET_HARDNET) {
        using SL = SplitLays<CB>;
        using LQH = typename SL::LQH;
        using LQH2 = typename SL::LQH2;
        using LR0 = typename SL::LR0;
        using LR1 = typename SL::LR1;
        constexpr int TERMS = S3;
        constexpr bool WHOLE = TERMS == 2;
        f32x4 bias1[2];
        const int s3_alt = a.s3_alt;
        using LQ2 = std::conditional_t<TERMS == 2, LayR<16, 16, 20, 2 * CB, 16>, LayQ<16, 16, 18, 2 * CB, 0, 3>>;
        using LQ4 = std::conditional_t<TERMS == 2, LayR<8, 8, 12, 4 * CB, 0>, LayQ<8, 8, 16, 4 * CB, 128, 3>>;
        static_assert(LQ2::BYTES <= TrunkLds<CB>::ACT * 4 && LQ4::BYTES <= TrunkLds<CB>::ACT * 4, "pre-split layouts must fit the activation buffer");
        char* base = reinterpret_cast<char*>(act);
        f32x4 acc_a[4][2], acc_b[4][2];
        S3W<2> wf1;
        S3W<1> wf2;
        f32x4 acc2_a[4][1], acc2_b[4][1], bias2[1];
        f32x4 acc2w[4][2], bias2w[2];
        if constexpr (WHOLE) {
            f32x4 acc1[8][2];
            S3W<2> wf2w;
            s3_prefetch_w0<NW, CB, CB, 64, 8, 2, TERMS>(a.packed + a.off.w_s3[1], wf1, wave, lane);
            prefetch_bias<NW, 32, 8, 2>(a.packed + a.off.b[1], bias1, wave, lane);
            conv0_whole_split_q<NW, LR0, 2>(patch, w0, bias0, act, wave, lane);
            __syncthreads();
            CNN_STAMP(2);
            __builtin_amdgcn_s_setprio(0);
            conv3x3_mfma_s3q<NW, CB, CB, LR0, 1, 8, 2>(act, a.packed + a.off.w_s3[1], wf1, acc1, wave, lane, s3_alt);
            __builtin_amdgcn_s_setprio(3);
            CNN_STAMP(3);
            s3_prefetch_w0<NW, CB, 2 * CB, 16, 4, 2, TERMS>(a.packed + a.off.w_s3[2], wf2w, wave, lane);
            prefetch_bias<NW, 16, 4, 2>(a.packed + a.off.b[2], bias2w, wave, lane);
            __syncthreads();
            zero_halo_q<LR1, NTHR>(act);
            store_tiles_split_q<CB, LR1, 8, 2>(act, bias1, acc1, wave, lane);
            __syncthreads();
            CNN_STAMP(4);
            __builtin_amdgcn_s_setprio(0);
            conv3x3_mfma_s3q<NW, CB, 2 * CB, LR1, 2, 4, 2>(act, a.packed + a.off.w_s3[2], wf2w, acc2w, wave, lane, s3_alt);
            __builtin_amdgcn_s_setprio(3);
        } else {
            s3_prefetch_w0<NW, CB, CB, 32, 4, 2, TERMS>(a.packed + a.off.w_s3[1], wf1, wave, lane);
            prefetch_bias<NW, 32, 8, 2>(a.packed + a.off.b[1], bias1, wave, lane);
            conv0_half_split_q<NW, LQH, 2>(patch, w0, bias0, act, 0, wave, lane);
            __syncthreads();
            CNN_STAMP(2);
            __builtin_amdgcn_s_setprio(0);
            conv3x3_mfma_s3q<NW, CB, CB, LQH, 1, 4, 2>(act, a.packed + a.off.w_s3[1], wf1, acc_a, wave, lane, s3_alt);
            __builtin_amdgcn_s_setprio(3);
            __syncthreads();
            if (tid < LQH::SLOTS * 4 * 32) {
                const int t = tid / 128, g = (tid >> 5) & 3, x = tid & 31;
                *reinterpret_cast<f32x4*>(base + g * LQH::GS + LQH::at(17, x + 1) + t * LQH::TSTEP) = (f32x4){0.f, 0.f, 0.f, 0.f};
            }
            conv0_half_split_q<NW, LQH, 2>(patch, w0, bias0, act, 1, wave, lane);
            __syncthreads();
            __builtin_amdgcn_s_setprio(0);
            conv3x3_mfma_s3q<NW, CB, CB, LQH, 1, 4, 2>(act, a.packed + a.off.w_s3[1], wf1, acc_b, wave, lane, s3_alt);
            __builtin_amdgcn_s_setprio(3);
            CNN_STAMP(3);
            s3_prefetch_w0<NW, CB, 2 * CB, 8, 4, 1, TERMS>(a.packed + a.off.w_s3[2], wf2, wave, lane);
            bias2[0] = *reinterpret_cast<const f32x4*>(&a.packed[a.off.b[2] + (wave >> 1) * 16 + 4 * (lane >> 4)]);
            __syncthreads();
            zero_halo_q<LQH2, NTHR>(act);
            store_tiles_split_q<CB, LQH2, 4, 2>(act, bias1, acc_a, wave, lane);
            __syncthreads();
            CNN_STAMP(4);
            __builtin_amdgcn_s_setprio(0);
            conv3x3_mfma_s3q<NW, CB, 2 * CB, LQH2, 2, 4, 1>(act, a.packed + a.off.w_s3[2], wf2, acc2_a, wave, lane, s3_alt);
            __builtin_amdgcn_s_setprio(3);
            __syncthreads();
            store_tiles_split_q<CB, LQH2, 4, 2>(act, bias1, acc_b, wave, lane);
            if (wave == 7) {
                const int n = lane & 15;
#pragma unroll
                for (int i = 2; i < 4; ++i) split_store_tile_q<LQH2, 2>(base, LQH2::at(0, (i - 2) * 16 + n + 1), 0, bias1, acc_a[i], lane >> 4);
            }
            __syncthreads();
            __builtin_amdgcn_s_setprio(0);
            conv3x3_mfma_s3q<NW, CB, 2 * CB, LQH2, 2, 4, 1>(act, a.packed + a.off.w_s3[2], wf2, acc2_b, wave, lane, s3_alt);
            __builtin_amdgcn_s_setprio(3);
        }
        CNN_STAMP(5);
        S3W<2> wf3;
        S3W<1> wf4, wf5;
        f32x4 bias3[2], bias4[1], bias5s[1];
        s3_prefetch_w0<NW, 2 * CB, 2 * CB, 16, 4, 2, TERMS>(a.packed + a.off.w_s3[3], wf3, wave, lane);
        prefetch_bias<NW, 16, 4, 2>(a.packed + a.off.b[3], bias3, wave, lane);
        __syncthreads();
        zero_halo_q<LQ2, NTHR>(act);
        if constexpr (WHOLE) store_tiles_split_q<2 * CB, LQ2, 4, 2>(act, bias2w, acc2w, wave, lane);
        else {
            store_tiles_split_q<2 * CB, LQ2, 4, 1, 8>(act, bias2, acc2_a, wave, lane, 0);
            store_tiles_split_q<2 * CB, LQ2, 4, 1, 8>(act, bias2, acc2_b, wave, lane, 8);
        }
        __syncthreads();
        CNN_STAMP(6);
        {
            f32x4 acc_[4][2];
            __builtin_amdgcn_s_setprio(0);
            conv3x3_mfma_s3q<NW, 2 * CB, 2 * CB, LQ2, 1, 4, 2>(act, a.packed + a.off.w_s3[3], wf3, acc_, wave, lane, s3_alt);
            __builtin_amdgcn_s_setprio(3);
            CNN_STAMP(7);
            s3_prefetch_w0<NW, 2 * CB, 4 * CB, 4, 4, 1, TERMS>(a.packed + a.off.w_s3[4], wf4, wave, lane);
            prefetch_bias<NW, 8, 4, 1>(a.packed + a.off.b[4], bias4, wave, lane);
            __syncthreads();
            store_tiles_split_q<2 * CB, LQ2, 4, 2>(act, bias3, acc_, wave, lane);
            __syncthreads();
            CNN_STAMP(8);
        }
        {
            f32x4 acc_[4][1];
            __builtin_amdgcn_s_setprio(0);
            conv3x3_mfma_s3q<NW, 2 * CB, 4 * CB, LQ2, 2, 4, 1>(act, a.packed + a.off.w_s3[4], wf4, acc_, wave, lane, s3_alt);
            __builtin_amdgcn_s_setprio(3);
            CNN_STAMP(9);
            s3_prefetch_w0<NW, 4 * CB, 4 * CB, 4, 4, 1, TERMS>(a.packed + a.off.w_s3[5], wf5, wave, lane);
            prefetch_bias<NW, 8, 4, 1>(a.packed + a.off.b[5], bias5s, wave, lane);
            __syncthreads();
            zero_halo_q<LQ4, NTHR>(act);
            store_tiles_split_q<4 * CB, LQ4, 4, 1>(act, bias4, acc_, wave, lane);
            __syncthreads();
            CNN_STAMP(10);
        }
        f32x4 acc5[4][1];
        __builtin_amdgcn_s_setprio(0);
        conv3x3_mfma_s3q<NW, 4 * CB, 4 * CB, LQ4, 1, 4, 1>(act, a.packed + a.off.w_s3[5], wf5, acc5, wave, lane, s3_alt);
        __builtin_amdgcn_s_setprio(3);
        CNN_STAMP(11);
        store_tiles_global<4 * CB, 4, 1>(a.out + pidx * (64 * 4 * CB), bias5s, acc5, wave, lane);
    } else {
        constexpr int T4M = S::T4M, T4N = S::T4N;
        using SL = SplitLays<CB>;
        using LQH = typename SL::LQH;
        using LQH2 = typename SL::LQH2;
        using LR0 = typename SL::LR0;
        using LR0H = typename SL::LR0H;
        using LR1 = typename SL::LR1;
        using LR1H = typename SL::LR1H;
        constexpr int TERMS = S3;
        constexpr bool WHOLE = TERMS == 2;
        f32x4 bias1[1];
        using LQ2 = std::conditional_t<TERMS == 2, LayR<16, 16, 20, 2 * CB, 0>, LayQ<16, 16, 18, 2 * CB, 0, 3>>;
        using LQ4 = std::conditional_t<TERMS == 2, LayR<8, 8, 12, 4 * CB, 0>, LayQ<8, 8, 16, 4 * CB, 128, 3>>;
        static_assert(LQ2::BYTES <= TrunkLds<CB>::ACT * 4 && LQ4::BYTES <= TrunkLds<CB>::ACT * 4, "pre-split layouts must fit the activation buffer");
        char* base = reinterpret_cast<char*>(act);
        f32x4 acc_a[4][1], acc_b[4][1];
        S3W<1> wf1, wf2;
        f32x4 acc2_a[2][1], acc2_b[2][1], bias2[1];
        if constexpr (WHOLE) {
            prefetch_bias_fresh<NW, 32, 8, 1>(a.packed + a.off.b[1], bias1, wave, lane);
            conv0_whole_split_q<NW, LR0, 1>(patch, w0, bias0, act, wave, lane);
            s3_prefetch_w0<NW, CB, CB, 32, 4, 1, TERMS>(a.packed + a.off.w_s3[1], wf1, wave, lane);
            __syncthreads();
            CNN_STAMP(2);
            conv3x3_mfma_s3q<NW, CB, CB, LR0H, 1, 4, 1>(act, a.packed + a.off.w_s3[1], wf1, acc_a, wave, lane, false);
            conv3x3_mfma_s3q<NW, CB, CB, LR0H, 1, 4, 1>(act + LR0::at(16, 0) / 4, a.packed + a.off.w_s3[1], wf1, acc_b, wave, lane, false);
            CNN_STAMP(3);
            {
                int l2 = lane;
                asm volatile("" : "+v"(l2));
                bias2[0] = *reinterpret_cast<const f32x4*>(&a.packed[a.off.b[2] + (wave >> 2) * 16 + 4 * (l2 >> 4)]);
            }
            __syncthreads();
            zero_halo_q<LR1, NTHR>(act);
            store_tiles_split_q<CB, LR1, 4, 1, 16>(act, bias1, acc_a, wave, lane, 0);
            store_tiles_split_q<CB, LR1, 4, 1, 16>(act, bias1, acc_b, wave, lane, 16);
            s3_prefetch_w0<NW, CB, 2 * CB, 8, 2, 1, TERMS>(a.packed + a.off.w_s3[2], wf2, wave, lane);
            __syncthreads();
            CNN_STAMP(4);
            conv3x3_mfma_s3q<NW, CB, 2 * CB, LR1H, 2, 2, 1>(act, a.packed + a.off.w_s3[2], wf2, acc2_a, wave, lane, false);
            conv3x3_mfma_s3q<NW, CB, 2 * CB, LR1H, 2, 2, 1>(act + LR1::at(16, 0) / 4, a.packed + a.off.w_s3[2], wf2, acc2_b, wave, lane, false);
        } else {
            prefetch_bias_fresh<NW, 32, 8, 1>(a.packed + a.off.b[1], bias1, wave, lane);
            conv0_half_split_q<NW, LQH, 1>(patch, w0, bias0, act, 0, wave, lane);
            s3_prefetch_w0<NW, CB, CB, 32, 4, 1, TERMS>(a.packed + a.off.w_s3[1], wf1, wave, lane);
            __syncthreads();
            CNN_STAMP(2);
            conv3x3_mfma_s3q<NW, CB, CB, LQH, 1, 4, 1>(act, a.packed + a.off.w_s3[1], wf1, acc_a, wave, lane, false);
            __syncthreads();
            if (tid < LQH::SLOTS * 2 * 32) {
                const int t = tid >> 6, g = (tid >> 5) & 1, x = tid & 31;
                *reinterpret_cast<f32x4*>(base + g * LQH::GS + LQH::at(17, x + 1) + t * LQH::TSTEP) = (f32x4){0.f, 0.f, 0.f, 0.f};
            }
            conv0_half_split_q<NW, LQH, 1>(patch, w0, bias0, act, 1, wave, lane);
            s3_prefetch_w0<NW, CB, CB, 32, 4, 1, TERMS>(a.packed + a.off.w_s3[1], wf1, wave, lane);
            __syncthreads();
            conv3x3_mfma_s3q<NW, CB, CB, LQH, 1, 4, 1>(act, a.packed + a.off.w_s3[1], wf1, acc_b, wave, lane, false);
            CNN_STAMP(3);
            {
                int l2 = lane;
                asm volatile("" : "+v"(l2));
                bias2[0] = *reinterpret_cast<const f32x4*>(&a.packed[a.off.b[2] + (wave >> 2) * 16 + 4 * (l2 >> 4)]);
            }
            __syncthreads();
            zero_halo_q<LQH2, NTHR>(act);
            store_tiles_split_q<CB, LQH2, 4, 1>(act, bias1, acc_a, wave, lane);
            s3_prefetch_w0<NW, CB, 2 * CB, 8, 2, 1, TERMS>(a.packed + a.off.w_s3[2], wf2, wave, lane);
            __syncthreads();
            CNN_STAMP(4);
            conv3x3_mfma_s3q<NW, CB, 2 * CB, LQH2, 2, 2, 1>(act, a.packed + a.off.w_s3[2], wf2, acc2_a, wave, lane, false);
            __syncthreads();
            store_tiles_split_q<CB, LQH2, 4, 1>(act, bias1, acc_b, wave, lane);
            if (wave == 7) {
                const int n = lane & 15;
#pragma unroll
                for (int i = 2; i < 4; ++i) split_store_tile_q<LQH2, 1>(base, LQH2::at(0, (i - 2) * 16 + n + 1), 0, bias1, acc_a[i], lane >> 4);
            }
            s3_prefetch_w0<NW, CB, 2 * CB, 8, 2, 1, TERMS>(a.packed + a.off.w_s3[2], wf2, wave, lane);
            __syncthreads();
            conv3x3_mfma_s3q<NW, CB, 2 * CB, LQH2, 2, 2, 1>(act, a.packed + a.off.w_s3[2], wf2, acc2_b, wave, lane, false);
        }
        CNN_STAMP(5);
        S3W<1> wf3, wf4;
        f32x4 bias3[1], bias4[1];
        __syncthreads();
        zero_halo_q<LQ2, NTHR>(act);
        store_tiles_split_q<2 * CB, LQ2, 2, 1, 8>(act, bias2, acc2_a, wave, lane, 0);
        store_tiles_split_q<2 * CB, LQ2, 2, 1, 8>(act, bias2, acc2_b, wave, lane, 8);
        s3_prefetch_w0<NW, 2 * CB, 2 * CB, 16, 4, 1, TERMS>(a.packed + a.off.w_s3[3], wf3, wave, lane);
        prefetch_bias_fresh<NW, 16, 4, 1>(a.packed + a.off.b[3], bias3, wave, lane);
        __syncthreads();
        CNN_STAMP(6);
        {
            f32x4 acc_[4][1];
            conv3x3_mfma_s3q<NW, 2 * CB, 2 * CB, LQ2, 1, 4, 1>(act, a.packed + a.off.w_s3[3], wf3, acc_, wave, lane, false);
            CNN_STAMP(7);
            __syncthreads();
            store_tiles_split_q<2 * CB, LQ2, 4, 1>(act, bias3, acc_, wave, lane);
            s3_prefetch_w0<NW, 2 * CB, 4 * CB, 4, 2, 1, TERMS>(a.packed + a.off.w_s3[4], wf4, wave, lane);
            prefetch_bias_fresh<NW, 8, 2, 1>(a.packed + a.off.b[4], bias4, wave, lane);
            __syncthreads();
            CNN_STAMP(8);
        }
        S3W<T4N> wf5;
// ... 26 lines not shown
```

affnet_amd/csrc/cnn_trunk_orinet.hip:

```cpp
#include "cnn_trunk.h"

__global__ __launch_bounds__(256) void wino_derive_u_kernel(const float* __restrict__ packed, int w1, int w3, int w5, float* __restrict__ U) {
    int e = blockIdx.x * 256 + threadIdx.x;
    if (e >= Wino16::PAIRS) return;
    const int l = e >= 256 + 1024 ? 5 : (e >= 256 ? 3 : 1);
    const int ch = 8 << ((l + 1) >> 1);
    const float* src = packed + (l == 5 ? w5 : (l == 3 ? w3 : w1));
    float* dst = U + Wino16::offset(l);
    e -= l == 5 ? 256 + 1024 : (l == 3 ? 256 : 0);
    const int n = (e >> 2) % ch, c = (e >> 2) / ch * 4 + (e & 3);
    float g[9], u[16];
#pragma unroll
    for (int t = 0; t < 9; ++t) g[t] = src[w_tap_index(t, c, n, ch, ch)];
    wino_weight_transform(g, u);
#pragma unroll
    for (int xi = 0; xi < 16; ++xi) dst[w_tap_index(xi, c, n, ch, ch)] = u[xi];
}

int aff_wino_u_ensure(affnet_ctx* ctx) {
    if (ctx->wino_u) return AFFNET_OK;
    AFF_HIP(ctx, hipMalloc((void**)&ctx->wino_u, (size_t)2 * Wino16::FLOATS * sizeof(float)));
    return AFFNET_OK;
}

int aff_wino_derive_u(affnet_ctx* ctx, int kind, const float* packed, const NetLayout& L, hipStream_t st, const float** u) {
    const int rc = aff_wino_u_ensure(ctx);
    if (rc) return rc;
    float* dst = ctx->wino_u + (size_t)kind * Wino16::FLOATS;
    hipLaunchKernelGGL(wino_derive_u_kernel, dim3((Wino16::PAIRS + 255) / 256), dim3(256), 0, st, packed, (int)L.w_off[1], (int)L.w_off[3], (int)L.w_off[5], dst);
    AFF_LAUNCH_CHECK(ctx);
    *u = dst;
    return AFFNET_OK;
}

TrunkKernel aff_trunk_orinet(int arith_index, bool stamps) {
    static const TrunkKernel k[3][2] = {{cnn32_trunk_kernel<AFFNET_NET_ORINET, 8, false>, cnn32_trunk_kernel<AFFNET_NET_ORINET, 8, true>},
                                        {cnn32_trunk_kernel<AFFNET_NET_ORINET, 8, false, 3>, cnn32_trunk_kernel<AFFNET_NET_ORINET, 8, true, 3>},
                                        {cnn32_trunk_kernel<AFFNET_NET_ORINET, 8, false, 2>, cnn32_trunk_kernel<AFFNET_NET_ORINET, 8, true, 2>}};
    return k[arith_index][stamps];
}
```

affnet_amd/csrc/common.h:

```cpp
#pragma once
#include <hip/hip_runtime.h>
#include <stdint.h>
#include <stdio.h>
#include <string.h>

#include <string>
#include <vector>

#include "../../include/affnet_hip.h"
#include "../../include/affnet_hip_debug.h"
#include "weights_layout.h"

#define AFF_WAVE 64

enum {
    CNT_RAW0 = 0,
    CNT_CAND = AFFNET_MAX_OCTAVES,
    CNT_OVERFLOW,
    CNT_SEL,
    CNT_EQ_TAKEN,
    CNT_SEL_MODE,
    CNT_SEL_THRESH,
    CNT_SEL_NEED_EQ,
    CNT_DET,
    CNT_SHAPED,
    CNT_SURVIVED,
    CNT_CAND2,
    CNT_AFF_EVAL,
    CNT_SURVIVED1,
    CNT_SEL_EQ_TOTAL,
    CNT_SEL_TIE_LO, CNT_SEL_TIE_HI,
    CNT_AFF_REEVAL,
    CNT_POS0 = AFFNET_MAX_OCTAVES + 24,
    CNT_HYP0 = AFFNET_MAX_OCTAVES + 24 + (AFFNET_MAX_LEVELS - 2) * AFFNET_MAX_OCTAVES,
    CNT_TOTAL = AFFNET_MAX_OCTAVES + 24 + (AFFNET_MAX_LEVELS - 2) * AFFNET_MAX_OCTAVES + 8 * AFFNET_MAX_OCTAVES
};

#define OVF_FRAMES_COUNT 16
#define OVF_FRAMES_NONFINITE 32

#define SEL_HIST_BINS 2048

struct RawMax {
    int32_t pix;
    int32_t lvl;
    float val;
    float s, y, x;
    float prev[2];
};

struct OctaveGeom {
    int32_t h, w;
    int64_t pyr_off;
    int64_t map_off;
    int64_t raw_off;
    int32_t raw_cap;
};

struct affnet_ctx {
    int device = 0;
    affnet_config cfg;
    int B = 1;
    size_t pyr_stride = 0;
    size_t map_stride = 0;
    size_t raw_stride = 0;
    std::string err;
    OctaveGeom oct[AFFNET_MAX_OCTAVES];
    size_t off_pyr = 0, off_map = 0, off_raw = 0, off_cnt = 0, off_hist = 0, off_cand = 0, off_sel = 0, off_stage = 0;
    size_t off_affmap = 0, off_dense = 0, off_cand2 = 0, off_lvltab = 0;
    size_t aff_stride = 0;
    size_t aff_off[AFFNET_MAX_OCTAVES] = {0};
    size_t dense_stride = 0;
    float* affmap = nullptr; float* dense = nullptr;
    float* cand2_resp = nullptr; float* cand2_syx = nullptr; int32_t* cand2_ids = nullptr;
    int32_t* lvltab = nullptr;
    size_t ws_bytes = 0;
    size_t pyr_floats = 0, map_bytes = 0, raw_total = 0, cand_cap = 0;
    int cap_pre = 0, cap_final = 0;
    char* ws = nullptr;
    float* pyr = nullptr;
    uint8_t* omap = nullptr;
    RawMax* raw = nullptr;
    int32_t* cnt = nullptr;
    uint32_t* sel_hist = nullptr;
    float* cand_resp = nullptr; float* cand_syx = nullptr; int32_t* cand_ids = nullptr;
    float* sel_resp = nullptr; float* sel_syx = nullptr; int32_t* sel_ids = nullptr;
    float* st_det_resp = nullptr; float* st_det_lafs = nullptr; int32_t* st_det_ids = nullptr;
    int32_t* st_det_count = nullptr;
    float* st_A = nullptr; float* st_key = nullptr; int32_t* st_good = nullptr;
    float* st_A2 = nullptr; float* st_lafs_iter = nullptr;
    float* st_R = nullptr; float* st_lafs_norm = nullptr; int32_t* st_lvl_ids = nullptr;
    float* st_hard_scratch = nullptr;
    float* st_lafs_shaped = nullptr;
    int32_t* st_rank = nullptr;
    bool prof_on = false;
    std::vector<hipEvent_t> prof_ev;
    int prof_calls = 0;
    unsigned long long* dbg_time = nullptr;
    int shape_form = AFFNET_SHAPE_FORM_WINOGRAD;
    int arith = AFFNET_ARITH_FP32_MFMA;
    int split3_variant = 0;
    hipGraph_t graph = nullptr;
    hipGraphExec_t graph_exec = nullptr;
    float* wino_u = nullptr;
    float* poly_u = nullptr;
    int desc_form = AFFNET_DESC_FORM_F43;
    ~affnet_ctx() {
        if (wino_u) (void)hipFree(wino_u);
        if (poly_u) (void)hipFree(poly_u);
        if (graph_exec) (void)hipGraphExecDestroy(graph_exec);
        if (graph) (void)hipGraphDestroy(graph);
        for (auto& e : prof_ev) (void)hipEventDestroy(e);
    }
};

struct AffDeviceGuard {
    int prev = -1;
    bool switched = false;
    explicit AffDeviceGuard(const affnet_ctx* ctx) {
        if (!ctx) return;
        if (hipGetDevice(&prev) != hipSuccess) { (void)hipGetLastError(); prev = -1; return; }
        if (prev != ctx->device) switched = hipSetDevice(ctx->device) == hipSuccess;
    }
    ~AffDeviceGuard() {
        if (switched) (void)hipSetDevice(prev);
    }
    AffDeviceGuard(const AffDeviceGuard&) = delete;
    AffDeviceGuard& operator=(const AffDeviceGuard&) = delete;
};
#define AFF_DEVICE(ctx) AffDeviceGuard aff_device_guard_(ctx)

#define PROF_RING 256
#define PROF_EVENTS (AFFNET_PROFILE_STAGES + 2)

#define AFF_HIP(ctx, expr)                                                                         \
    do {                                                                                           \
        hipError_t e_ = (expr);                                                                    \
        if (e_ != hipSuccess)                                                                      \
            return aff_fail(ctx, AFFNET_ERR_HIP, "%s failed: %s (%s:%d)", #expr, hipGetErrorString(e_), \
                            __FILE__, __LINE__);                                                   \
    } while (0)

#define AFF_LAUNCH_CHECK(ctx)                                                                      \
    do {                                                                                           \
        hipError_t e_ = hipGetLastError();                                                         \
        if (e_ != hipSuccess)                                                                      \
            return aff_fail(ctx, AFFNET_ERR_HIP, "kernel launch failed: %s (%s:%d)",                \
                            hipGetErrorString(e_), __FILE__, __LINE__);                            \
    } while (0)

struct AffZeroSegs {
    unsigned char* p[8];
    size_t bytes[8];
    int n = 0;
    bool overflow = false;
    void add(void* ptr, size_t nbytes) {
        if (!ptr || !nbytes) return;
        if (n >= 8) { overflow = true; return; }
        p[n] = (unsigned char*)ptr; bytes[n] = nbytes; ++n;
    }
};

static inline size_t aff_align(size_t x, size_t a = 256) { return (x + a - 1) / a * a; }
static inline int aff_cdiv(int a, int b) { return (a + b - 1) / b; }

struct PyrTable {
    const float* lvl[AFFNET_MAX_OCTAVES][AFFNET_MAX_LEVELS];
    int h[AFFNET_MAX_OCTAVES], w[AFFNET_MAX_OCTAVES];
    int n_octaves, n_levels;
    size_t img_stride;
};

struct LevelTable { double sig[AFFNET_MAX_OCTAVES * AFFNET_MAX_LEVELS]; int n_oct, n_lvl; };
struct DenormSel {
    float* out_px; int32_t* ids; float* lafs_norm;
    float c_a, c_x, c_y, ps, ca, cx, cy;
    LevelTable lt;
};


#define HEAD_PART_AFF 32
#define HEAD_PART_ORI 144
#define HEAD_KSPLIT 4
#define HEAD_KC 128
#define HEAD_AS (HEAD_KC + 4)

struct PyrSrc {
    PyrTable t;
    float base[32];
};

struct CnnArgs {
    const float* packed;
    NetOffsets off;
    const float* wino_u;
    const int32_t* reeval;
    const float* patches;
    const float* lafs;
    const int32_t* ids;
    const int32_t* count;
    int n_max;
    float* out;
    int dbg_layer;
    int s3_alt;
    float* dbg_out;
    unsigned long long* dbg_time;
    int row_begin;
    const int32_t* skip_cnt;
    int skip_n;
    int32_t* shape_cnt;
    int shape_op;
};

__device__ __forceinline__ bool lazy_skip(const int32_t* skip_cnt, int skip_n, int image, int which = CNT_SURVIVED1) {
    if (!skip_cnt) return false;
    const int32_t* c = skip_cnt + (size_t)image * CNT_TOTAL;
    return c[CNT_SEL_MODE] == 1 && c[which] >= skip_n;
}

struct Wino16 {
    static constexpr int U1 = 16 * 16 * 16, U3 = 16 * 32 * 32, U5 = 16 * 64 * 64, FLOATS = U1 + U3 + U5;
    static constexpr int PAIRS = 16 * 16 + 32 * 32 + 64 * 64;
    static constexpr int NB1 = 2, NB3 = 1;
    static constexpr int offset(int layer) { return layer == 1 ? 0 : (layer == 3 ? U1 : U1 + U3); }
    static constexpr int floats(int layer) { return layer == 1 ? U1 : (layer == 3 ? U3 : U5); }
};

struct ShapeFuse {
    const float* resp; const float* lafs; float* key; int32_t* good; int32_t* cnt;
};

struct CnnCall {
    int kind = -1;
    const float* packed = nullptr;
    const float* patches = nullptr;
    const float* lafs = nullptr; const int32_t* ids = nullptr;
    const int32_t* count = nullptr; int n_max = 0;
    float* out = nullptr; float* scratch = nullptr;
    hipStream_t st = nullptr;
    int dbg_layer = -1; float* dbg_out = nullptr;
    bool mark_head = false;
    int row_begin = 0, row_count = -1;
    const int32_t* skip_cnt = nullptr; int skip_n = 0;
    const ShapeFuse* fuse = nullptr; int shape_op = 0;
    int desc_form = AFFNET_DESC_FORM_DIRECT;
    bool wino_reeval = false;
    float* rot_lafs = nullptr; const DenormSel* denorm = nullptr;
};

typedef void (*TrunkKernel)(CnnArgs, PyrSrc);

int aff_fail(affnet_ctx* ctx, int code, const char* fmt, ...);
int aff_zero_async(affnet_ctx* ctx, void* dst, size_t bytes, hipStream_t st);
int aff_zero_multi_async(affnet_ctx* ctx, const AffZeroSegs& z, hipStream_t st);
int aff_copy_async(affnet_ctx* ctx, void* dst, const void* src, size_t bytes, hipStream_t st);
int aff_copy2d_async(affnet_ctx* ctx, void* dst, size_t dpitch, const void* src, size_t spitch, size_t width_bytes, size_t rows, hipStream_t st);
void aff_base_grid(int ps, float* base);

void aff_prof_mark(affnet_ctx* ctx, int idx, hipStream_t st);

int aff_detect_impl(affnet_ctx* ctx, const float* d_responses, float* d_resp, float* d_lafs, int32_t* d_ids, int32_t* d_count, void* stream);
int aff_detect_onepass_impl(affnet_ctx* ctx, const float* d_packed_fullconv, const float* d_responses, hipStream_t st);

int aff_fullconv_launch(affnet_ctx* ctx, const float* packed, const float* img, size_t img_stride, int h, int w, float* out, size_t out_stride,
                        float* scratch, size_t scratch_stride, int B, hipStream_t st);

int aff_handcrafted_launch(affnet_ctx* ctx, int kind, const float* patches, const float* lafs, const int32_t* ids, const int32_t* count,
                           int n_max, const float* h_weights, float* out, float* out_angle, hipStream_t st);

void aff_fill_pyr_table(const affnet_ctx* ctx, PyrTable* t);
int aff_shape_select(affnet_ctx* ctx, const float* d_resp_in, const float* d_lafs_in, const int32_t* d_ids_in, const float* d_A,
                     const int32_t* d_count_in, float* d_resp_out, float* d_lafs_out, int32_t* d_ids_out, int32_t* d_count_out, hipStream_t st);
int aff_shape_iterate(affnet_ctx* ctx, const float* A, float* base, const float* lafs, const int32_t* count, int mode, float* lafs_out,
                      hipStream_t st);
void aff_denorm_sel_fill(affnet_ctx* ctx, int ps, float* d_lafs_px, int32_t* d_ids, float* d_lafs_norm, DenormSel* ds);
int aff_denorm_level_select(affnet_ctx* ctx, const float* d_lafs_norm_in, float* d_lafs_px, const int32_t* d_count, int n_max, int ps, int32_t* d_ids,
                            float* d_lafs_norm, hipStream_t st);

int aff_arith_index(const affnet_ctx* ctx);
int aff_affnet_filter_rows(affnet_ctx* ctx, const float* packed, const float* resp, const float* lafs, const int32_t* ids, const int32_t* count,
                           float* out, float* scratch, int row_begin, int row_count, bool lazy, int shape_op, hipStream_t st);
int aff_orinet_rotate(affnet_ctx* ctx, const float* packed, float* lafs, const int32_t* ids, const int32_t* count, int n_max, float* out, float* scratch,
                      hipStream_t st, const DenormSel* denorm);
int aff_hardnet_forward_pyr_marked(affnet_ctx* ctx, const float* packed, const float* lafs, const int32_t* ids, const int32_t* count,
                                   int n_max, float* out, float* scratch, hipStream_t st);

int aff_hardnet_poly_patches(affnet_ctx* ctx, const float* packed, const float* patches, int n, float* out, float* scratch, int dbg_layer, hipStream_t st,
                             int form = AFFNET_DESC_FORM_POLYPHASE);

TrunkKernel aff_trunk_affnet(int arith_index, bool stamps);
TrunkKernel aff_trunk_affnet_wino(bool stamps);
TrunkKernel aff_trunk_orinet(int arith_index, bool stamps);
TrunkKernel aff_trunk_hardnet(int arith_index, bool stamps);
TrunkKernel aff_trunk_hardnet_poly(bool stamps);
int aff_poly_u_ensure(affnet_ctx* ctx);
int aff_poly_derive_u(affnet_ctx* ctx, const float* packed, const NetLayout& L, hipStream_t st, const float** u);
TrunkKernel aff_trunk_hardnet_f43(bool stamps);
int aff_f43_derive_u(affnet_ctx* ctx, const float* packed, const NetLayout& L, hipStream_t st);
int aff_wino_u_ensure(affnet_ctx* ctx);
int aff_wino_derive_u(affnet_ctx* ctx, int kind, const float* packed, const NetLayout& L, hipStream_t st, const float** u);

int aff_finish_affnet(affnet_ctx* ctx, const CnnCall& c, const NetLayout& L, int rows, int B);
int aff_margin_affnet(affnet_ctx* ctx, const CnnCall& c, const NetLayout& L, int rows, int B, int32_t* flags);
int aff_finish_orinet(affnet_ctx* ctx, const CnnCall& c, const NetLayout& L, int rows, int B);
int aff_hardnet_head(affnet_ctx* ctx, const CnnCall& c, const NetLayout& L, int B);

struct AffTile {
    int x0, y0, tw, th;
};

__device__ __forceinline__ AffTile aff_tile_box(float t00, float t01, float t02, float t10, float t11, float t12, int ps, int cap) {
    const float um = (float)(ps - 1) / (float)ps;
    const float hx = (fabsf(t00) + fabsf(t01)) * um, hy = (fabsf(t10) + fabsf(t11)) * um;
    const float cx = t02 - 0.5f, cy = t12 - 0.5f;
    AffTile t;
    t.tw = 0; t.th = 0; t.x0 = 0; t.y0 = 0;
    if (!(hx < 4096.0f && hy < 4096.0f && fabsf(cx) < 1.0e6f && fabsf(cy) < 1.0e6f)) return t;
    const int x0 = (int)floorf(cx - hx) - 1, x1 = (int)floorf(cx + hx) + 2;
    const int y0 = (int)floorf(cy - hy) - 1, y1 = (int)floorf(cy + hy) + 2;
    const int tw = x1 - x0 + 1, th = y1 - y0 + 1;
    if (tw * th > cap || tw * th > 2 * ps * ps) return t;
    t.x0 = x0; t.y0 = y0; t.tw = tw; t.th = th;
    return t;
}

template <int NTHR>
__device__ __forceinline__ void aff_tile_load(float* tile, const AffTile t, const float* __restrict__ img, int h, int w, int tid) {
    const int n = t.tw * t.th;
    for (int i = tid; i < n; i += NTHR) {
        const int ty = i / t.tw, tx = i - ty * t.tw;
        const int gy = t.y0 + ty, gx = t.x0 + tx;
        tile[i] = (gy >= 0 && gy < h && gx >= 0 && gx < w) ? img[(size_t)gy * w + gx] : 0.0f;
    }
}

__device__ __forceinline__ float aff_sample_bilinear(const float* __restrict__ img, int h, int w,
                                                     float t00, float t01, float t02, float t10,
                                                     float t11, float t12, float u, float v) {
    float gx = fmaf(1.0f, t02, fmaf(v, t01, u * t00));
    float gy = fmaf(1.0f, t12, fmaf(v, t11, u * t10));
    const float fw = (float)w, fh = (float)h;
    gx = 2.0f * gx / fw - 1.0f;
    gy = 2.0f * gy / fh - 1.0f;
    const float ix = fmaf(gx + 1.0f, fw * 0.5f, -0.5f);
    const float iy = fmaf(gy + 1.0f, fh * 0.5f, -0.5f);
    const float x0f = floorf(ix), y0f = floorf(iy);
    const float x1f = x0f + 1.0f, y1f = y0f + 1.0f;
    const float wx1 = ix - x0f, wx0 = x1f - ix, wy1 = iy - y0f, wy0 = y1f - iy;
    const float nw = wx0 * wy0, ne = wx1 * wy0, sw = wx0 * wy1, se = wx1 * wy1;
    const float cx0 = fminf(fmaxf(x0f, -2.0f), fw + 1.0f), cy0 = fminf(fmaxf(y0f, -2.0f), fh + 1.0f);
    const int x0 = (int)cx0, y0 = (int)cy0, x1 = x0 + 1, y1 = y0 + 1;
    const bool xin0 = (x0 >= 0) & (x0 < w), xin1 = (x1 >= 0) & (x1 < w);
    const bool yin0 = (y0 >= 0) & (y0 < h), yin1 = (y1 >= 0) & (y1 < h);
    const float vnw = (xin0 & yin0) ? img[(size_t)y0 * w + x0] : 0.0f;
    const float vne = (xin1 & yin0) ? img[(size_t)y0 * w + x1] : 0.0f;
    const float vsw = (xin0 & yin1) ? img[(size_t)y1 * w + x0] : 0.0f;
    const float vse = (xin1 & yin1) ? img[(size_t)y1 * w + x1] : 0.0f;
    return fmaf(vse, se, fmaf(vsw, sw, fmaf(vne, ne, vnw * nw)));
}

__device__ __forceinline__ float aff_sample_bilinear_tile(const float* tile, const AffTile tl, const float* __restrict__ img, int h, int w,
                                                          float t00, float t01, float t02, float t10, float t11, float t12, float u, float v) {
    float gx = fmaf(1.0f, t02, fmaf(v, t01, u * t00));
    float gy = fmaf(1.0f, t12, fmaf(v, t11, u * t10));
    const float fw = (float)w, fh = (float)h;
    gx = 2.0f * gx / fw - 1.0f;
    gy = 2.0f * gy / fh - 1.0f;
    const float ix = fmaf(gx + 1.0f, fw * 0.5f, -0.5f);
    const float iy = fmaf(gy + 1.0f, fh * 0.5f, -0.5f);
    const float x0f = floorf(ix), y0f = floorf(iy);
    const float x1f = x0f + 1.0f, y1f = y0f + 1.0f;
    const float wx1 = ix - x0f, wx0 = x1f - ix, wy1 = iy - y0f, wy0 = y1f - iy;
    const float nw = wx0 * wy0, ne = wx1 * wy0, sw = wx0 * wy1, se = wx1 * wy1;
    const float cx0 = fminf(fmaxf(x0f, -2.0f), fw + 1.0f), cy0 = fminf(fmaxf(y0f, -2.0f), fh + 1.0f);
    const int x0 = (int)cx0, y0 = (int)cy0;
    const int lx = x0 - tl.x0, ly = y0 - tl.y0;
    float vnw, vne, vsw, vse;
    if (lx >= 0 && ly >= 0 && lx + 1 < tl.tw && ly + 1 < tl.th) {
        const float* p = tile + ly * tl.tw + lx;
        vnw = p[0]; vne = p[1]; vsw = p[tl.tw]; vse = p[tl.tw + 1];
    } else {
        const int x1 = x0 + 1, y1 = y0 + 1;
        const bool xin0 = (x0 >= 0) & (x0 < w), xin1 = (x1 >= 0) & (x1 < w);
        const bool yin0 = (y0 >= 0) & (y0 < h), yin1 = (y1 >= 0) & (y1 < h);
        vnw = (xin0 & yin0) ? img[(size_t)y0 * w + x0] : 0.0f;
        vne = (xin1 & yin0) ? img[(size_t)y0 * w + x1] : 0.0f;
        vsw = (xin0 & yin1) ? img[(size_t)y1 * w + x0] : 0.0f;
        vse = (xin1 & yin1) ? img[(size_t)y1 * w + x1] : 0.0f;
    }
    return fmaf(vse, se, fmaf(vsw, sw, fmaf(vne, ne, vnw * nw)));
}
```

affnet_amd/csrc/context.hip:

```cpp
#include <stdarg.h>

#include "common.h"

int aff_fail(affnet_ctx* ctx, int code, const char* fmt, ...) {
    char buf[1024];
    va_list ap;
    va_start(ap, fmt);
    vsnprintf(buf, sizeof(buf), fmt, ap);
    va_end(ap);
    if (ctx) ctx->err = buf;
    return code;
}

__global__ __launch_bounds__(256) void aff_zero_kernel(unsigned char* __restrict__ p, size_t bytes) {
    const size_t head = ((16 - ((size_t)p & 15)) & 15) < bytes ? ((16 - ((size_t)p & 15)) & 15) : bytes;
    const size_t n16 = (bytes - head) / 16, tail0 = head + n16 * 16;
    uint4* q = reinterpret_cast<uint4*>(p + head);
    for (size_t i = (size_t)blockIdx.x * 256 + threadIdx.x; i < n16; i += (size_t)gridDim.x * 256) q[i] = make_uint4(0u, 0u, 0u, 0u);
    if (blockIdx.x == 0) {
        for (size_t i = threadIdx.x; i < head; i += 256) p[i] = 0;
        for (size_t i = tail0 + threadIdx.x; i < bytes; i += 256) p[i] = 0;
    }
}

__global__ __launch_bounds__(256) void aff_zero_multi_kernel(AffZeroSegs z) {
    unsigned char* p = z.p[blockIdx.y];
    const size_t bytes = z.bytes[blockIdx.y];
    const size_t head = ((16 - ((size_t)p & 15)) & 15) < bytes ? ((16 - ((size_t)p & 15)) & 15) : bytes;
    const size_t n16 = (bytes - head) / 16, tail0 = head + n16 * 16;
    uint4* q = reinterpret_cast<uint4*>(p + head);
    for (size_t i = (size_t)blockIdx.x * 256 + threadIdx.x; i < n16; i += (size_t)gridDim.x * 256) q[i] = make_uint4(0u, 0u, 0u, 0u);
    if (blockIdx.x == 0) {
        for (size_t i = threadIdx.x; i < head; i += 256) p[i] = 0;
        for (size_t i = tail0 + threadIdx.x; i < bytes; i += 256) p[i] = 0;
    }
}

int aff_zero_multi_async(affnet_ctx* ctx, const AffZeroSegs& z, hipStream_t st) {
    if (z.overflow) return aff_fail(ctx, AFFNET_ERR_INVALID, "internal: more than 8 areas in one fused clear (AffZeroSegs)");
    if (z.n <= 0) return AFFNET_OK;
    size_t blocks = 1;
    for (int i = 0; i < z.n; ++i) {
        const size_t b = (z.bytes[i] / 16 + 255) / 256;
        blocks = b > blocks ? b : blocks;
    }
    blocks = blocks > 2048 ? 2048 : blocks;
    hipLaunchKernelGGL(aff_zero_multi_kernel, dim3((unsigned)blocks, (unsigned)z.n), dim3(256), 0, st, z);
    AFF_LAUNCH_CHECK(ctx);
    return AFFNET_OK;
}

__global__ __launch_bounds__(256) void aff_copy2d_kernel(uint32_t* __restrict__ dst, size_t dpitch_w, const uint32_t* __restrict__ src, size_t spitch_w,
                                                         size_t width_w) {
    const uint32_t* s = src + (size_t)blockIdx.y * spitch_w;
    uint32_t* d = dst + (size_t)blockIdx.y * dpitch_w;
    for (size_t i = (size_t)blockIdx.x * 256 + threadIdx.x; i < width_w; i += (size_t)gridDim.x * 256) d[i] = s[i];
}

int aff_zero_async(affnet_ctx* ctx, void* dst, size_t bytes, hipStream_t st) {
    if (!dst || bytes == 0) return AFFNET_OK;
    size_t blocks = (bytes / 16 + 255) / 256;
    blocks = blocks < 1 ? 1 : (blocks > 4096 ? 4096 : blocks);
    hipLaunchKernelGGL(aff_zero_kernel, dim3((unsigned)blocks), dim3(256), 0, st, (unsigned char*)dst, bytes);
    AFF_LAUNCH_CHECK(ctx);
    return AFFNET_OK;
}

int aff_copy2d_async(affnet_ctx* ctx, void* dst, size_t dpitch, const void* src, size_t spitch, size_t width_bytes, size_t rows, hipStream_t st) {
    if (rows == 0 || width_bytes == 0) return AFFNET_OK;
    if (!dst || !src || ((size_t)dst & 3) || ((size_t)src & 3) || (dpitch & 3) || (spitch & 3) || (width_bytes & 3) || rows > 65535)
        return aff_fail(ctx, AFFNET_ERR_INVALID, "copy2d: pointers, pitches and width must be multiples of 4 bytes, rows <= 65535");
    size_t bx = (width_bytes / 4 + 255) / 256;
    bx = bx < 1 ? 1 : (bx > 2048 ? 2048 : bx);
    hipLaunchKernelGGL(aff_copy2d_kernel, dim3((unsigned)bx, (unsigned)rows), dim3(256), 0, st, (uint32_t*)dst, dpitch / 4, (const uint32_t*)src, spitch / 4,
                       width_bytes / 4);
    AFF_LAUNCH_CHECK(ctx);
    return AFFNET_OK;
}

int aff_copy_async(affnet_ctx* ctx, void* dst, const void* src, size_t bytes, hipStream_t st) {
    return aff_copy2d_async(ctx, dst, bytes, src, bytes, bytes, 1, st);
}

extern "C" const char* affnet_version(void) { return "affnet_hip 0.2 (gfx950, hipcc, fp32 MFMA 16x16x4)"; }

extern "C" const char* affnet_last_error(const affnet_ctx* ctx) { return ctx ? ctx->err.c_str() : "null context"; }

void aff_base_grid(int ps, float* base) {
    if (ps == 1) { base[0] = 0.0f; return; }
    const float step = 2.0f / (float)(ps - 1);
    const int half = ps / 2;
    for (int i = 0; i < ps; ++i) {
        float v = (i < half) ? fmaf(step, (float)i, -1.0f) : fmaf(-step, (float)(ps - 1 - i), 1.0f);
        base[i] = (v * (float)(ps - 1)) / (float)ps;
    }
}

extern "C" int affnet_host_base_grid(int ps, float* out) {
    if (ps < 1 || !out) return AFFNET_ERR_INVALID;
    aff_base_grid(ps, out);
    return AFFNET_OK;
}

static int validate(affnet_ctx* ctx, const affnet_config* c) {
    if (c->height < 8 || c->width < 8) return aff_fail(ctx, AFFNET_ERR_INVALID, "image %dx%d too small", c->height, c->width);
    if (c->batch > 4096) return aff_fail(ctx, AFFNET_ERR_INVALID, "batch=%d (max 4096)", c->batch);
    if (c->arith < AFFNET_ARITH_FP32_MFMA || c->arith > AFFNET_ARITH_FP32_SPLIT2H) return aff_fail(ctx, AFFNET_ERR_INVALID, "arith=%d (AFFNET_ARITH_*)", c->arith);
    if (c->n_octaves < 1 || c->n_octaves > AFFNET_MAX_OCTAVES) return aff_fail(ctx, AFFNET_ERR_INVALID, "n_octaves=%d", c->n_octaves);
    if (c->levels_per_octave < 3 || c->levels_per_octave > AFFNET_MAX_LEVELS)
        return aff_fail(ctx, AFFNET_ERR_INVALID, "levels_per_octave=%d", c->levels_per_octave);
    if (c->oct_h[0] != c->height || c->oct_w[0] != c->width) return aff_fail(ctx, AFFNET_ERR_INVALID, "octave 0 size mismatch");
    for (int o = 1; o < c->n_octaves; ++o)
        if (c->oct_h[o] != (c->oct_h[o - 1] - 1) / 2 + 1 || c->oct_w[o] != (c->oct_w[o - 1] - 1) / 2 + 1)
            return aff_fail(ctx, AFFNET_ERR_INVALID, "octave %d size is not ceil(prev/2)", o);
    if (c->first_blur_taps != 0 && (c->first_blur_taps % 2 == 0 || c->first_blur_taps > AFFNET_MAX_TAPS))
        return aff_fail(ctx, AFFNET_ERR_INVALID, "first_blur_taps=%d", c->first_blur_taps);
    for (int l = 1; l < c->levels_per_octave; ++l)
        if (c->level_blur_taps[l] % 2 == 0 || c->level_blur_taps[l] < 1 || c->level_blur_taps[l] > AFFNET_MAX_TAPS)
            return aff_fail(ctx, AFFNET_ERR_INVALID, "level_blur_taps[%d]=%d", l, c->level_blur_taps[l]);
    if (c->level_blur0_taps[1] != 0)
        for (int l = 1; l < c->levels_per_octave; ++l)
            if (c->level_blur0_taps[l] % 2 == 0 || c->level_blur0_taps[l] < 1 || c->level_blur0_taps[l] > AFFNET_MAX_TAPS)
                return aff_fail(ctx, AFFNET_ERR_INVALID, "level_blur0_taps[%d]=%d", l, c->level_blur0_taps[l]);
    return AFFNET_OK;
}

extern "C" int affnet_ctx_create(affnet_ctx** out, int device, const affnet_config* cfg) {
    if (!out) return AFFNET_ERR_INVALID;
    affnet_ctx* ctx = new affnet_ctx();
    ctx->device = device;
    if (!cfg) {
        memset(&ctx->cfg, 0, sizeof(ctx->cfg));
        *out = ctx;
        return AFFNET_OK;
    }
    ctx->cfg = *cfg;
    ctx->arith = cfg->arith;
    int rc = validate(ctx, cfg);
    if (rc != AFFNET_OK) { *out = ctx; return rc; }
    const affnet_config& c = ctx->cfg;
    const int div = c.max_raw_per_octave_div > 0 ? c.max_raw_per_octave_div : 4;
    size_t pyr = 0, mapb = 0, raw = 0;
    for (int o = 0; o < c.n_octaves; ++o) {
        OctaveGeom& g = ctx->oct[o];
        g.h = c.oct_h[o]; g.w = c.oct_w[o];
        g.pyr_off = (int64_t)pyr; pyr += (size_t)c.levels_per_octave * g.h * g.w;
        g.map_off = (int64_t)mapb; mapb += aff_align((size_t)g.h * g.w, 16);
        int cap = (int)((size_t)g.h * g.w / div); if (cap < 256) cap = 256;
        g.raw_off = (int64_t)raw; g.raw_cap = cap; raw += cap;
    }
    ctx->B = c.batch > 0 ? c.batch : 1;
    const size_t B = (size_t)ctx->B;
    ctx->pyr_floats = pyr; ctx->map_bytes = mapb; ctx->raw_total = raw; ctx->cand_cap = raw;
    ctx->pyr_stride = aff_align(pyr * sizeof(float)) / sizeof(float);
    ctx->map_stride = aff_align(mapb);
    ctx->raw_stride = raw;
    const int keep = c.max_keep > 0 ? c.max_keep : 65536;
    ctx->cap_pre = c.num_prefilter > 0 ? c.num_prefilter : keep;
    ctx->cap_final = c.num_features > 0 ? c.num_features : ctx->cap_pre;
    if (ctx->cap_final > ctx->cap_pre) ctx->cap_final = ctx->cap_pre;
    size_t off = 0;
    ctx->off_pyr = off; off += B * ctx->pyr_stride * sizeof(float);
    ctx->off_map = off; off += B * ctx->map_stride;
    ctx->off_raw = off; off += aff_align(B * raw * sizeof(RawMax));
    ctx->off_cnt = off; off += aff_align(B * CNT_TOTAL * sizeof(int32_t));
    ctx->off_hist = off; off += aff_align(B * SEL_HIST_BINS * sizeof(uint32_t));
    ctx->off_cand = off; off += aff_align(B * ctx->cand_cap * 7 * sizeof(float));
    ctx->off_sel = off; off += aff_align(B * (size_t)ctx->cap_pre * 7 * sizeof(float));
    ctx->off_stage = off;
    const size_t P = B * (size_t)ctx->cap_pre, F = B * (size_t)ctx->cap_final;
    off += aff_align(P * 10 * sizeof(float));
    off += aff_align(P * 4 * sizeof(float));
    off += aff_align(P * 10 * sizeof(float));
    off += aff_align(P * 2 * sizeof(float));
    off += aff_align(P * sizeof(int32_t));
    off += aff_align(B * sizeof(int32_t));
    off += aff_align(F * 6 * sizeof(float));
    off += aff_align(F * 4 * sizeof(float));
    off += aff_align(F * 9 * sizeof(float));
    {
        const size_t hard = F * (8192 + 4 * 128), aff = P * 144;
        off += aff_align((hard > aff ? hard : aff) * sizeof(float));
    }
    if (c.onepass) {
        if (c.num_prefilter != c.num_features) { *out = ctx; return aff_fail(ctx, AFFNET_ERR_INVALID, "onepass: num_prefilter must equal num_features"); }
        size_t aff = 0;
        for (int o = 0; o < c.n_octaves; ++o) {
            if (c.oct_h[o] < 34 || c.oct_w[o] < 34) {
                *out = ctx;
                return aff_fail(ctx, AFFNET_ERR_INVALID, "onepass: octave %d is %dx%d, LocalNorm2d(33) needs >= 34 px in this library (17 in the reference: use "
                                "border >= 15 like its scripts, so that the pyramid stops earlier)", o, c.oct_w[o], c.oct_h[o]);
            }
            ctx->aff_off[o] = aff; aff += aff_align((size_t)4 * c.oct_h[o] * c.oct_w[o] * sizeof(float)) / sizeof(float);
        }
        ctx->aff_stride = aff;
        ctx->dense_stride = affnet_fullconv_scratch_bytes(c.oct_h[0], c.oct_w[0]) / sizeof(float);
        ctx->off_affmap = off; off += aff_align(B * aff * sizeof(float));
        ctx->off_dense = off; off += aff_align(B * ctx->dense_stride * sizeof(float));
        ctx->off_cand2 = off; off += aff_align(B * ctx->cand_cap * 7 * sizeof(float));
        ctx->off_lvltab = off; off += aff_align(B * (size_t)AFFNET_MAX_OCTAVES * AFFNET_MAX_LEVELS * 4 * sizeof(int32_t));
    }
    ctx->ws_bytes = off;
    *out = ctx;
    return AFFNET_OK;
}

extern "C" void affnet_ctx_destroy(affnet_ctx* ctx) { delete ctx; }

extern "C" int affnet_set_arith(affnet_ctx* ctx, int arith) {
    if (!ctx) return AFFNET_ERR_INVALID;
    if (arith < AFFNET_ARITH_FP32_MFMA || arith > AFFNET_ARITH_FP32_SPLIT2H) return aff_fail(ctx, AFFNET_ERR_INVALID, "arith=%d (AFFNET_ARITH_*)", arith);
    ctx->arith = arith;
    ctx->cfg.arith = arith;
    return AFFNET_OK;
}
extern "C" int affnet_get_arith(const affnet_ctx* ctx) { return ctx ? ctx->arith : AFFNET_ERR_INVALID; }

extern "C" int affnet_set_shape_form(affnet_ctx* ctx, int form) {
    if (!ctx) return AFFNET_ERR_INVALID;
    if (form != AFFNET_SHAPE_FORM_DIRECT && form != AFFNET_SHAPE_FORM_WINOGRAD) return aff_fail(ctx, AFFNET_ERR_INVALID, "shape form=%d (AFFNET_SHAPE_FORM_*)", form);
    ctx->shape_form = form;
    return AFFNET_OK;
}
extern "C" int affnet_get_shape_form(const affnet_ctx* ctx) { return ctx ? ctx->shape_form : AFFNET_ERR_INVALID; }

extern "C" int affnet_set_desc_form(affnet_ctx* ctx, int form) {
    if (!ctx) return AFFNET_ERR_INVALID;
    if (form != AFFNET_DESC_FORM_DIRECT && form != AFFNET_DESC_FORM_POLYPHASE && form != AFFNET_DESC_FORM_F43) return aff_fail(ctx, AFFNET_ERR_INVALID, "descriptor form=%d (AFFNET_DESC_FORM_*)", form);
    ctx->desc_form = form;
    return AFFNET_OK;
}
extern "C" int affnet_get_desc_form(const affnet_ctx* ctx) { return ctx ? ctx->desc_form : AFFNET_ERR_INVALID; }

extern "C" size_t affnet_workspace_bytes(const affnet_ctx* ctx) { return ctx ? ctx->ws_bytes : 0; }

extern "C" int affnet_capacity_prefilter(const affnet_ctx* ctx) { return ctx ? ctx->cap_pre : 0; }
extern "C" int affnet_capacity_final(const affnet_ctx* ctx) { return ctx ? ctx->cap_final : 0; }

extern "C" int64_t affnet_pyramid_level_offset(const affnet_ctx* ctx, int octave, int level) {
    if (!ctx || octave < 0 || octave >= ctx->cfg.n_octaves || level < 0 || level >= ctx->cfg.levels_per_octave) return -1;
    const OctaveGeom& g = ctx->oct[octave];
    return (int64_t)(ctx->off_pyr / sizeof(float)) + g.pyr_off + (int64_t)level * g.h * g.w;
}

extern "C" int64_t affnet_pyramid_image_stride(const affnet_ctx* ctx) { return ctx ? (int64_t)ctx->pyr_stride : 0; }

extern "C" int64_t affnet_counter_offset(const affnet_ctx* ctx, int which) {
    if (!ctx || ctx->ws_bytes == 0 || which < 0 || which > 4) return -1;
    const int idx = which == 0 ? CNT_OVERFLOW : (which == 1 ? CNT_DET : (which == 2 ? CNT_SHAPED : (which == 3 ? CNT_AFF_EVAL : CNT_AFF_REEVAL)));
    return (int64_t)(ctx->off_cnt / sizeof(int32_t)) + idx;
}
extern "C" int64_t affnet_counter_stride(const affnet_ctx* ctx) { return ctx ? (int64_t)CNT_TOTAL : 0; }

extern "C" int64_t affnet_affmap_offset(const affnet_ctx* ctx, int octave) {
    if (!ctx || !ctx->cfg.onepass || octave < 0 || octave >= ctx->cfg.n_octaves) return -1;
    return (int64_t)(ctx->off_affmap / sizeof(float)) + (int64_t)ctx->aff_off[octave];
}
extern "C" int64_t affnet_affmap_image_stride(const affnet_ctx* ctx) { return (ctx && ctx->cfg.onepass) ? (int64_t)ctx->aff_stride : 0; }
extern "C" int affnet_batch(const affnet_ctx* ctx) { return ctx ? ctx->B : 0; }

extern "C" int affnet_bind_workspace(affnet_ctx* ctx, void* d_workspace, size_t bytes) {
    if (!ctx) return AFFNET_ERR_INVALID;
    if (!d_workspace || bytes < ctx->ws_bytes)
        return aff_fail(ctx, AFFNET_ERR_INVALID, "workspace too small: %zu < %zu", bytes, ctx->ws_bytes);
    if (((uintptr_t)d_workspace & 255) != 0) return aff_fail(ctx, AFFNET_ERR_INVALID, "workspace must be 256-byte aligned");
    {
        hipPointerAttribute_t at;
        if (hipPointerGetAttributes(&at, d_workspace) == hipSuccess) {
            if (at.type == hipMemoryTypeDevice && at.device != ctx->device)
                return aff_fail(ctx, AFFNET_ERR_INVALID, "workspace belongs to device %d, the context to device %d", at.device, ctx->device);
        } else {
            (void)hipGetLastError();
        }
    }
    char* b = (char*)d_workspace;
    ctx->ws = b;
    ctx->pyr = (float*)(b + ctx->off_pyr);
    ctx->omap = (uint8_t*)(b + ctx->off_map);
    ctx->raw = (RawMax*)(b + ctx->off_raw);
    ctx->cnt = (int32_t*)(b + ctx->off_cnt);
    ctx->sel_hist = (uint32_t*)(b + ctx->off_hist);
    const size_t B = (size_t)ctx->B;
    float* cand = (float*)(b + ctx->off_cand);
    const size_t CC = B * ctx->cand_cap;
    ctx->cand_resp = cand; ctx->cand_syx = cand + CC; ctx->cand_ids = (int32_t*)(cand + 4 * CC);
    float* sel = (float*)(b + ctx->off_sel);
    const size_t P = B * (size_t)ctx->cap_pre, F = B * (size_t)ctx->cap_final;
    ctx->sel_resp = sel; ctx->sel_syx = sel + P; ctx->sel_ids = (int32_t*)(sel + 4 * P);
    char* s = b + ctx->off_stage;
    ctx->st_det_resp = (float*)s; ctx->st_det_lafs = (float*)s + P; ctx->st_det_ids = (int32_t*)((float*)s + 7 * P);
    s += aff_align(P * 10 * sizeof(float));
    ctx->st_A = (float*)s; s += aff_align(P * 4 * sizeof(float));
    ctx->st_A2 = (float*)s; ctx->st_lafs_iter = (float*)s + 4 * P; s += aff_align(P * 10 * sizeof(float));
    ctx->st_key = (float*)s; ctx->st_good = (int32_t*)((float*)s + P); s += aff_align(P * 2 * sizeof(float));
    ctx->st_rank = (int32_t*)s; s += aff_align(P * sizeof(int32_t));
    ctx->st_det_count = (int32_t*)s; s += aff_align(B * sizeof(int32_t));
    ctx->st_lafs_shaped = (float*)s; s += aff_align(F * 6 * sizeof(float));
    ctx->st_R = (float*)s; s += aff_align(F * 4 * sizeof(float));
    ctx->st_lafs_norm = (float*)s; ctx->st_lvl_ids = (int32_t*)((float*)s + 6 * F); s += aff_align(F * 9 * sizeof(float));
    ctx->st_hard_scratch = (float*)s;
    if (ctx->cfg.onepass) {
        ctx->affmap = (float*)(b + ctx->off_affmap);
        ctx->dense = (float*)(b + ctx->off_dense);
        float* c2 = (float*)(b + ctx->off_cand2);
        ctx->cand2_resp = c2; ctx->cand2_syx = c2 + CC; ctx->cand2_ids = (int32_t*)(c2 + 4 * CC);
        ctx->lvltab = (int32_t*)(b + ctx->off_lvltab);
    }
    return AFFNET_OK;
}

extern "C" int affnet_read_counts(affnet_ctx* ctx, int32_t out[4], void* stream) {
    AFF_DEVICE(ctx);
    if (!ctx || !ctx->ws) return AFFNET_ERR_INVALID;
    std::vector<int32_t> all((size_t)ctx->B * CNT_TOTAL);
    AFF_HIP(ctx, hipMemcpyAsync(all.data(), ctx->cnt, all.size() * sizeof(int32_t), hipMemcpyDeviceToHost, (hipStream_t)stream));
    AFF_HIP(ctx, hipStreamSynchronize((hipStream_t)stream));
    int32_t host[CNT_TOTAL];
    memset(host, 0, sizeof(host));
    int raw = 0;
    for (int b = 0; b < ctx->B; ++b) {
        const int32_t* h = all.data() + (size_t)b * CNT_TOTAL;
        host[CNT_DET] += h[CNT_DET]; host[CNT_SHAPED] += h[CNT_SHAPED]; host[CNT_OVERFLOW] |= h[CNT_OVERFLOW];
        for (int o = 0; o < ctx->cfg.n_octaves; ++o) raw += h[CNT_RAW0 + o];
    }
    out[0] = host[CNT_DET]; out[1] = host[CNT_SHAPED]; out[2] = host[CNT_OVERFLOW];
    out[3] = raw;
    if (host[CNT_OVERFLOW] & OVF_FRAMES_NONFINITE)
        return aff_fail(ctx, AFFNET_ERR_INVALID, "load_frames: a caller-supplied frame or response was not finite (stored as a zero row; flag %d)",
                        host[CNT_OVERFLOW]);
    if (host[CNT_OVERFLOW]) return aff_fail(ctx, AFFNET_ERR_CAPACITY, "a fixed-capacity detector list overflowed (flag %d)", host[CNT_OVERFLOW]);
    if (host[CNT_DET] == 0)
        return aff_fail(ctx, AFFNET_ERR_EMPTY, "no keypoints detected in %d image(s) (the reference raises in torch.cat, SparseImgRepresenter.py:100)", ctx->B);
    return AFFNET_OK;
}
```

affnet_amd/csrc/debug.hip:

```cpp
#include "common.h"

#include "../../include/affnet_hip_probes.h"

template <typename T>
__global__ __launch_bounds__(256) void stream_read_kernel(const T* __restrict__ src, float* __restrict__ dst, size_t n_items) {
    float acc = 0.f;
    for (size_t i = (size_t)blockIdx.x * 256 + threadIdx.x; i < n_items; i += (size_t)gridDim.x * 256) {
        const T v = src[i];
        const float* f = reinterpret_cast<const float*>(&v);
#pragma unroll
        for (int k = 0; k < (int)(sizeof(T) / 4); ++k) acc += f[k];
    }
    if (acc == 123.456f) dst[blockIdx.x] = acc;
    if (threadIdx.x == 0 && blockIdx.x == 0) dst[0] = acc;
}

template <typename T>
__global__ __launch_bounds__(256) void stream_write_kernel(T* __restrict__ dst, size_t n_items) {
    T v;
    float* f = reinterpret_cast<float*>(&v);
#pragma unroll
    for (int k = 0; k < (int)(sizeof(T) / 4); ++k) f[k] = (float)(threadIdx.x + k);
    for (size_t i = (size_t)blockIdx.x * 256 + threadIdx.x; i < n_items; i += (size_t)gridDim.x * 256) dst[i] = v;
}

__global__ __launch_bounds__(256) void tile_read_kernel(const float* __restrict__ img, float* __restrict__ dst, int h, int w, int halo) {
    const int LW = 64 + 2 * halo, n_el = LW * LW;
    const int x0 = blockIdx.x * 64, y0 = blockIdx.y * 64;
    float acc = 0.f;
    for (int i = threadIdx.x; i < n_el; i += 256) {
        const int ty = i / LW, tx = i - ty * LW;
        int gy = y0 + ty - halo, gx = x0 + tx - halo;
        gy = gy < 0 ? 0 : (gy >= h ? h - 1 : gy);
        gx = gx < 0 ? 0 : (gx >= w ? w - 1 : gx);
        acc += img[(size_t)gy * w + gx];
    }
    if (acc == 123.456f) dst[blockIdx.x] = acc;
}

struct f32x2s { float a, b; };

extern "C" int affnet_debug_stream(const void* d_src, void* d_dst, size_t n_bytes, int width, int mode, int halo, void* stream) {
    if (!d_dst || n_bytes == 0 || (n_bytes & 65535) != 0) return AFFNET_ERR_INVALID;
    hipStream_t st = (hipStream_t)stream;
    const int blocks = 256 * 16;
    if (mode == 0) {
        if (!d_src) return AFFNET_ERR_INVALID;
        if (width == 4) hipLaunchKernelGGL(stream_read_kernel<float>, dim3(blocks), dim3(256), 0, st, (const float*)d_src, (float*)d_dst, n_bytes / 4);
        else if (width == 8) hipLaunchKernelGGL(stream_read_kernel<f32x2s>, dim3(blocks), dim3(256), 0, st, (const f32x2s*)d_src, (float*)d_dst, n_bytes / 8);
        else if (width == 16) hipLaunchKernelGGL(stream_read_kernel<float4>, dim3(blocks), dim3(256), 0, st, (const float4*)d_src, (float*)d_dst, n_bytes / 16);
        else return AFFNET_ERR_INVALID;
    } else if (mode == 1) {
        if (width == 4) hipLaunchKernelGGL(stream_write_kernel<float>, dim3(blocks), dim3(256), 0, st, (float*)d_dst, n_bytes / 4);
        else if (width == 8) hipLaunchKernelGGL(stream_write_kernel<f32x2s>, dim3(blocks), dim3(256), 0, st, (f32x2s*)d_dst, n_bytes / 8);
        else if (width == 16) hipLaunchKernelGGL(stream_write_kernel<float4>, dim3(blocks), dim3(256), 0, st, (float4*)d_dst, n_bytes / 16);
        else return AFFNET_ERR_INVALID;
    } else if (mode == 2) {
        if (!d_src || halo < 0 || halo > 16) return AFFNET_ERR_INVALID;
        const int w = 4096, h = (int)(n_bytes / 4 / w);
        hipLaunchKernelGGL(tile_read_kernel, dim3(w / 64, (h + 63) / 64), dim3(256), 0, st, (const float*)d_src, (float*)d_dst, h, w, halo);
    } else {
        return AFFNET_ERR_INVALID;
    }
    return hipGetLastError() == hipSuccess ? AFFNET_OK : AFFNET_ERR_HIP;
}

extern "C" int affnet_probe_shape_offsets(const affnet_ctx* ctx, int64_t out[3]) {
    if (!ctx || !ctx->ws || !out) return AFFNET_ERR_INVALID;
    out[0] = (int64_t)(reinterpret_cast<const char*>(ctx->st_A) - ctx->ws) / 4;
    out[1] = (int64_t)(reinterpret_cast<const char*>(ctx->st_hard_scratch) - ctx->ws) / 4 + (int64_t)ctx->B * ctx->cap_pre * HEAD_PART_AFF;
    out[2] = (int64_t)(reinterpret_cast<const char*>(ctx->st_det_lafs) - ctx->ws) / 4;
    return AFFNET_OK;
}

static int probe_affnet_wino(affnet_ctx* ctx, const float* d_packed, const float* d_patches, int n, float* d_out, int layer, hipStream_t st) {
    if (ctx->arith != AFFNET_ARITH_FP32_MFMA) return aff_fail(ctx, AFFNET_ERR_INVALID, "probe_affnet_wino: AFFNET_ARITH_FP32_MFMA only");
    const NetLayout L = net_layout(AFFNET_NET_AFFNET);
    CnnArgs a;
    memset(&a, 0, sizeof(a));
    a.packed = d_packed; a.off = to_offsets(L, ctx->arith);
    const int rc = aff_wino_derive_u(ctx, AFFNET_NET_AFFNET, d_packed, L, st, &a.wino_u);
    if (rc) return rc;
    a.patches = d_patches; a.n_max = n; a.out = d_out; a.dbg_layer = layer; a.dbg_out = d_out; a.dbg_time = ctx->dbg_time;
    PyrSrc ps;
    memset(&ps, 0, sizeof(ps));
    hipLaunchKernelGGL(aff_trunk_affnet_wino(layer >= 0 || a.dbg_time), dim3(n, 1), dim3(512), 0, st, a, ps);
    AFF_LAUNCH_CHECK(ctx);
    return AFFNET_OK;
}

extern "C" int affnet_probe_affnet_wino_layer(affnet_ctx* ctx, int net_kind, const float* d_packed, const float* d_patch, int layer, float* d_out, void* stream) {
    AFF_DEVICE(ctx);
    if (!ctx || !d_packed || !d_patch || !d_out || net_kind != AFFNET_NET_AFFNET || layer < 0 || layer > 5)
        return aff_fail(ctx, AFFNET_ERR_INVALID, "probe_affnet_wino_layer: AffNet, layer 0 .. 5");
    return probe_affnet_wino(ctx, d_packed, d_patch, 1, d_out, layer, (hipStream_t)stream);
}

extern "C" int affnet_probe_affnet_wino_partials(affnet_ctx* ctx, const float* d_packed, const float* d_patches, int n, float* d_partials, void* stream) {
    AFF_DEVICE(ctx);
    if (!ctx || !d_packed || !d_patches || !d_partials || n < 1 || n > 65535) return aff_fail(ctx, AFFNET_ERR_INVALID, "probe_affnet_wino_partials: bad argument");
    return probe_affnet_wino(ctx, d_packed, d_patches, n, d_partials, -1, (hipStream_t)stream);
}

extern "C" int affnet_probe_hardnet_poly_layer(affnet_ctx* ctx, const float* d_packed, const float* d_patch, int layer, float* d_out, void* stream) {
    AFF_DEVICE(ctx);
    if (!ctx || !d_packed || !d_patch || !d_out || layer < 0 || layer > 5) return aff_fail(ctx, AFFNET_ERR_INVALID, "probe_hardnet_poly_layer: layer 0 .. 5");
    return aff_hardnet_poly_patches(ctx, d_packed, d_patch, 1, d_out, nullptr, layer, (hipStream_t)stream);
}

extern "C" int affnet_probe_hardnet_poly_forward(affnet_ctx* ctx, const float* d_packed, const float* d_patches, int n, float* d_out, float* d_scratch, void* stream) {
    AFF_DEVICE(ctx);
    if (!ctx || !d_packed || !d_patches || !d_out || !d_scratch || n < 1 || n > 65535) return aff_fail(ctx, AFFNET_ERR_INVALID, "probe_hardnet_poly_forward: bad argument");
    return aff_hardnet_poly_patches(ctx, d_packed, d_patches, n, d_out, d_scratch, -1, (hipStream_t)stream);
}

extern "C" int affnet_probe_hardnet_poly_u(affnet_ctx* ctx, const float* d_packed, int layer, float* d_out, void* stream) {
    AFF_DEVICE(ctx);
    if (!ctx || !d_packed || !d_out || (layer != 2 && layer != 4)) return aff_fail(ctx, AFFNET_ERR_INVALID, "probe_hardnet_poly_u: layer 2 or 4");
    const float* u;
    const int rc = aff_poly_derive_u(ctx, d_packed, net_layout(AFFNET_NET_HARDNET), (hipStream_t)stream, &u);
    if (rc) return rc;
    return aff_copy_async(ctx, d_out, u + Poly32::offset(layer), (size_t)Poly32::floats(layer) * sizeof(float), (hipStream_t)stream);
}

extern "C" int affnet_probe_hardnet_f43_layer(affnet_ctx* ctx, const float* d_packed, const float* d_patch, int layer, float* d_out, void* stream) {
    AFF_DEVICE(ctx);
    if (!ctx || !d_packed || !d_patch || !d_out || layer < 0 || layer > 5) return aff_fail(ctx, AFFNET_ERR_INVALID, "probe_hardnet_f43_layer: layer 0 .. 5");
    return aff_hardnet_poly_patches(ctx, d_packed, d_patch, 1, d_out, nullptr, layer, (hipStream_t)stream, AFFNET_DESC_FORM_F43);
}

extern "C" int affnet_probe_hardnet_f43_forward(affnet_ctx* ctx, const float* d_packed, const float* d_patches, int n, float* d_out, float* d_scratch, void* stream) {
    AFF_DEVICE(ctx);
    if (!ctx || !d_packed || !d_patches || !d_out || !d_scratch || n < 1 || n > 65535) return aff_fail(ctx, AFFNET_ERR_INVALID, "probe_hardnet_f43_forward: bad argument");
    return aff_hardnet_poly_patches(ctx, d_packed, d_patches, n, d_out, d_scratch, -1, (hipStream_t)stream, AFFNET_DESC_FORM_F43);
}

extern "C" int affnet_probe_hardnet_f43_u(affnet_ctx* ctx, const float* d_packed, int layer, float* d_out, void* stream) {
    AFF_DEVICE(ctx);
    if (!ctx || !d_packed || !d_out || (layer != 1 && layer != 3)) return aff_fail(ctx, AFFNET_ERR_INVALID, "probe_hardnet_f43_u: layer 1 or 3");
    const int rc = aff_f43_derive_u(ctx, d_packed, net_layout(AFFNET_NET_HARDNET), (hipStream_t)stream);
    if (rc) return rc;
    return aff_copy_async(ctx, d_out, ctx->poly_u + F43::BASE + F43::offset(layer), (size_t)F43::floats(layer) * sizeof(float), (hipStream_t)stream);
}
```

include/affnet_hip.h:

```cpp
#ifndef AFFNET_HIP_H
#define AFFNET_HIP_H

#include <stddef.h>
#include <stdint.h>

#ifdef __cplusplus
extern "C" {
#endif

#define AFFNET_OK 0
#define AFFNET_ERR_INVALID (-1)
#define AFFNET_ERR_HIP (-2)
#define AFFNET_ERR_CAPACITY (-3)
#define AFFNET_ERR_EMPTY (-4)

#define AFFNET_MAX_OCTAVES 16
#define AFFNET_MAX_LEVELS 8
#define AFFNET_MAX_TAPS 37

#define AFFNET_NET_AFFNET 0
#define AFFNET_NET_ORINET 1
#define AFFNET_NET_HARDNET 2
#define AFFNET_NET_AFFNET_FULLCONV 3

#define AFFNET_ARITH_FP32_MFMA 0
#define AFFNET_ARITH_FP32_SPLIT3 1
#define AFFNET_ARITH_FP32_SPLIT2H 2

typedef struct affnet_ctx affnet_ctx;

typedef struct affnet_config {
    int32_t height, width;
    int32_t n_octaves;
    int32_t levels_per_octave;
    int32_t oct_h[AFFNET_MAX_OCTAVES];
    int32_t oct_w[AFFNET_MAX_OCTAVES];
    float level_sigma[AFFNET_MAX_OCTAVES][AFFNET_MAX_LEVELS];
    float level_sigma4[AFFNET_MAX_OCTAVES][AFFNET_MAX_LEVELS];
    double level_sigma_px[AFFNET_MAX_OCTAVES][AFFNET_MAX_LEVELS];
    int32_t first_blur_taps;
    float first_blur[AFFNET_MAX_TAPS * AFFNET_MAX_TAPS];
    int32_t level_blur_taps[AFFNET_MAX_LEVELS];
    float level_blur[AFFNET_MAX_LEVELS][AFFNET_MAX_TAPS * AFFNET_MAX_TAPS];
    int32_t level_blur0_taps[AFFNET_MAX_LEVELS];
    float level_blur0[AFFNET_MAX_LEVELS][AFFNET_MAX_TAPS * AFFNET_MAX_TAPS];
    int32_t lazy_shape_rows;
    int32_t onepass;
    float mr_size;
    float threshold;
    int32_t num_features;
    int32_t num_prefilter;
    int32_t max_raw_per_octave_div;
    int32_t max_keep;
    int32_t batch;
    int32_t baum_iters;
    int32_t arith;
} affnet_config;

int affnet_config_fill(affnet_config* cfg, int height, int width, int n_levels, double init_sigma, int border, double mr_size,
                       double threshold, int num_features, int num_prefilter, int batch, int baum_iters);


int affnet_ctx_create(affnet_ctx** out, int device, const affnet_config* cfg);
void affnet_ctx_destroy(affnet_ctx* ctx);
const char* affnet_last_error(const affnet_ctx* ctx);
const char* affnet_version(void);
int affnet_set_arith(affnet_ctx* ctx, int arith);
int affnet_get_arith(const affnet_ctx* ctx);

#define AFFNET_SHAPE_FORM_DIRECT 0
#define AFFNET_SHAPE_FORM_WINOGRAD 1
int affnet_set_shape_form(affnet_ctx* ctx, int form);
int affnet_get_shape_form(const affnet_ctx* ctx);

#define AFFNET_DESC_FORM_DIRECT 0
#define AFFNET_DESC_FORM_POLYPHASE 1
#define AFFNET_DESC_FORM_F43 2
int affnet_set_desc_form(affnet_ctx* ctx, int form);
int affnet_get_desc_form(const affnet_ctx* ctx);

size_t affnet_workspace_bytes(const affnet_ctx* ctx);
int affnet_bind_workspace(affnet_ctx* ctx, void* d_workspace, size_t bytes);
int64_t affnet_pyramid_level_offset(const affnet_ctx* ctx, int octave, int level);
int64_t affnet_pyramid_image_stride(const affnet_ctx* ctx);
int affnet_batch(const affnet_ctx* ctx);
int affnet_capacity_prefilter(const affnet_ctx* ctx);
int affnet_capacity_final(const affnet_ctx* ctx);


int affnet_gauss_blur(affnet_ctx* ctx, const float* d_in, float* d_out, int h, int w,
                      const float* h_taps, int k, void* stream);

int affnet_pyramid_build(affnet_ctx* ctx, const float* d_img, void* stream);

int affnet_hessian_response(affnet_ctx* ctx, const float* d_in, float* d_out, int h, int w,
                            float sigma4, void* stream);

int affnet_detect(affnet_ctx* ctx, float* d_resp, float* d_lafs, int32_t* d_ids,
                  int32_t* d_count, void* stream);

int affnet_detect_responses(affnet_ctx* ctx, const float* d_responses, float* d_resp, float* d_lafs, int32_t* d_ids,
                            int32_t* d_count, void* stream);

int affnet_laf_grid_sample(affnet_ctx* ctx, const float* d_img, int h, int w,
                           const float* d_lafs, int n, int ps, float* d_out, void* stream);

int affnet_pyr_grid_sample(affnet_ctx* ctx, const float* d_lafs, const int32_t* d_ids,
                           const int32_t* d_count, int n_max, int ps, float* d_out, void* stream);


size_t affnet_cnn32_packed_floats(int net_kind);
int64_t affnet_cnn32_winograd_offset(int net_kind, int layer);
int affnet_cnn32_pack_weights(int net_kind, const float* const* conv_w, const float* const* bn_mean,
                              const float* const* bn_var, const float* head_w, const float* head_b,
                              const float* head_bn_mean, const float* head_bn_var, float* h_out);

int affnet_cnn32_forward(affnet_ctx* ctx, int net_kind, const float* d_packed, const float* d_patches,
                         const int32_t* d_count, int n_max, float* d_out, float* d_scratch, void* stream);

int affnet_cnn32_forward_pyr(affnet_ctx* ctx, int net_kind, const float* d_packed, const float* d_lafs,
                             const int32_t* d_ids, const int32_t* d_count, int n_max, float* d_out,
                             float* d_scratch, void* stream);


int affnet_local_norm(affnet_ctx* ctx, const float* d_in, float* d_out, int h, int w, void* stream);

size_t affnet_fullconv_scratch_bytes(int h, int w);

int affnet_fullconv_forward(affnet_ctx* ctx, const float* d_packed, const float* d_img, int h, int w, float* d_out, float* d_scratch,
                            void* stream);

int affnet_nms2d(affnet_ctx* ctx, const float* d_in, float* d_out, int h, int w, float threshold, void* stream);


#define AFFNET_HC_ORIENTATION 0
#define AFFNET_HC_BAUMBERG 1

int affnet_handcrafted_forward(affnet_ctx* ctx, int kind, const float* d_patches, int n, const float* h_weights, float* d_out,
                               float* d_angles, void* stream);
int affnet_handcrafted_forward_pyr(affnet_ctx* ctx, int kind, const float* d_lafs, const int32_t* d_ids, const int32_t* d_count,
                                   int n_max, const float* h_weights, float* d_out, void* stream);


int affnet_sift_host_window(int patch_size, float* h_out);
int affnet_sift_forward(affnet_ctx* ctx, const float* d_patches, int n, const float* d_window, float clipval, float* d_desc, void* stream);
int affnet_sift_forward_pyr(affnet_ctx* ctx, const float* d_lafs_norm, const int32_t* d_ids, const int32_t* d_count, int n_max,
                            const float* d_window, float clipval, float* d_desc, void* stream);


size_t affnet_tfeat_packed_floats(void);
int affnet_tfeat_pack_weights(const float* conv1_w, const float* conv1_b, const float* conv2_w, const float* conv2_b, const float* cls_w,
                              const float* cls_b, float* h_out);
size_t affnet_tfeat_scratch_floats(int rows);
int affnet_tfeat_forward(affnet_ctx* ctx, const float* d_packed, const float* d_patches, const int32_t* d_count, int n_max, float* d_desc,
                         float* d_scratch, void* stream);
int affnet_tfeat_forward_pyr(affnet_ctx* ctx, const float* d_packed, const float* d_lafs_norm, const int32_t* d_ids, const int32_t* d_count,
                             int n_max, float* d_desc, float* d_scratch, void* stream);


int affnet_shape_filter_select(affnet_ctx* ctx, const float* d_resp_in, const float* d_lafs_in,
                               const int32_t* d_ids_in, const float* d_A, const int32_t* d_count_in,
                               float* d_resp_out, float* d_lafs_out, int32_t* d_ids_out,
                               int32_t* d_count_out, void* stream);

int affnet_shape_iterate(affnet_ctx* ctx, const float* d_A, float* d_base, const float* d_lafs, const int32_t* d_count, int mode,
                         float* d_lafs_out, void* stream);

int affnet_apply_rotation(affnet_ctx* ctx, float* d_lafs, const float* d_R, const int32_t* d_count,
                          int n_max, void* stream);

int affnet_scale_lafs(affnet_ctx* ctx, const float* d_in, float* d_out, const int32_t* d_count, int n_max,
                      int w, int h, int inverse, void* stream);

int affnet_lafs_to_ellipses(affnet_ctx* ctx, const float* d_lafs, const int32_t* d_count, int n_max, float* d_out, void* stream);

int affnet_ellipses_to_lafs(affnet_ctx* ctx, const float* d_ell, const int32_t* d_count, int n_max, float* d_lafs, void* stream);

int affnet_level_select(affnet_ctx* ctx, const float* d_lafs_px, const int32_t* d_count, int n_max,
                        int ps, int32_t* d_ids, float* d_lafs_norm, void* stream);


size_t affnet_match_scratch_bytes(int n1, int n2);

int affnet_distance_matrix(affnet_ctx* ctx, const float* d_desc1, int n1, const float* d_desc2, int n2, int dim, float* d_out,
                           void* d_scratch, void* stream);

int affnet_match_snn(affnet_ctx* ctx, const float* d_desc1, int n1, const float* d_desc2, int n2, int dim, float snn_threshold,
                     float* d_min_dist, int32_t* d_idx, float* d_min2_dist, int32_t* d_tent, int32_t* d_count, void* d_scratch,
                     void* stream);

int affnet_reproject_lafs(affnet_ctx* ctx, const float* d_lafs, int n, const float* h_H, float* d_out, void* stream);

int affnet_centre_nn(affnet_ctx* ctx, const float* d_query_lafs, int nq, const float* d_ref_lafs, int nr, float* d_min_dist,
                     int32_t* d_idx, void* stream);


typedef struct affnet_nets {
    const float* d_affnet;
    const float* d_orinet;
    const float* d_hardnet;
    const float* h_orientation_window;
    const float* h_baumberg_window;
} affnet_nets;

int affnet_extract_features(affnet_ctx* ctx, const affnet_nets* nets, const float* d_img, int do_ori,
                            float* d_lafs_px, float* d_resp, int32_t* d_ids, float* d_desc,
                            int32_t* d_count, void* stream);

int affnet_detect_image(affnet_ctx* ctx, const float* d_img, void* stream);
int affnet_detect_image_responses(affnet_ctx* ctx, const float* d_responses, void* stream);
int affnet_describe_detected(affnet_ctx* ctx, const affnet_nets* nets, int do_ori, float* d_lafs_px, float* d_resp,
                             int32_t* d_ids, float* d_desc, int32_t* d_count, void* stream);

int affnet_detect_image_onepass(affnet_ctx* ctx, const float* d_packed_fullconv, const float* d_img, void* stream);
int affnet_detect_image_onepass_responses(affnet_ctx* ctx, const float* d_packed_fullconv, const float* d_responses, void* stream);

int affnet_detected_list(affnet_ctx* ctx, float* d_resp, float* d_lafs, int32_t* d_ids, int32_t* d_count, void* stream);
int affnet_load_frames(affnet_ctx* ctx, const float* d_lafs, int normalised, const float* d_resp, const int32_t* d_ids,
                       const int32_t* d_count, int n_max, int ps, void* stream);

int affnet_describe_frames(affnet_ctx* ctx, const affnet_nets* nets, const float* d_img, const float* d_lafs_px, const float* d_resp_in,
                           const int32_t* d_count_in, int n_max, int do_ori, float* d_lafs_px_out, float* d_resp, int32_t* d_ids,
                           float* d_desc, int32_t* d_count, void* stream);

int64_t affnet_affmap_offset(const affnet_ctx* ctx, int octave);
int64_t affnet_affmap_image_stride(const affnet_ctx* ctx);

int affnet_graph_capture_extract(affnet_ctx* ctx, const affnet_nets* nets, const float* d_img, int do_ori, float* d_lafs_px, float* d_resp,
                                 int32_t* d_ids, float* d_desc, int32_t* d_count, void* stream);
int affnet_graph_launch(affnet_ctx* ctx, void* stream);

#define AFFNET_PROFILE_STAGES 8
int affnet_profile_enable(affnet_ctx* ctx, int on);
int affnet_profile_read(affnet_ctx* ctx, double sum_ms[AFFNET_PROFILE_STAGES], int32_t* n_calls);

int affnet_read_counts(affnet_ctx* ctx, int32_t out[4], void* stream);

int64_t affnet_counter_offset(const affnet_ctx* ctx, int which);
int64_t affnet_counter_stride(const affnet_ctx* ctx);

int affnet_host_base_grid(int ps, float* out);

#ifdef __cplusplus
}
#endif
#endif
```

include/affnet_hip_probes.h:

```cpp
#ifndef AFFNET_HIP_PROBES_H
#define AFFNET_HIP_PROBES_H

#include "affnet_hip.h"

#ifdef __cplusplus
extern "C" {
#endif

int affnet_cnn32_probe(const float* d_packed, int layer, int probe, int reps, int n_blocks, float* d_out, void* stream);

int affnet_debug_stream(const void* d_src, void* d_dst, size_t n_bytes, int width, int mode, int halo, void* stream);

int affnet_split3_gemm(const float* d_A, const float* d_Bt, int M, int N, int K, int mode, float* d_C, void* stream);
int affnet_split3_rate(int reps, int terms, int n_blocks, float* d_out, void* stream);

int affnet_probe_shape_offsets(const affnet_ctx* ctx, int64_t out[3]);

int affnet_probe_affnet_wino_layer(affnet_ctx* ctx, int net_kind, const float* d_packed, const float* d_patch, int layer, float* d_out, void* stream);

int affnet_probe_affnet_wino_partials(affnet_ctx* ctx, const float* d_packed, const float* d_patches, int n, float* d_partials, void* stream);

int affnet_probe_hardnet_poly_layer(affnet_ctx* ctx, const float* d_packed, const float* d_patch, int layer, float* d_out, void* stream);
int affnet_probe_hardnet_poly_forward(affnet_ctx* ctx, const float* d_packed, const float* d_patches, int n, float* d_out, float* d_scratch, void* stream);
int affnet_probe_hardnet_poly_u(affnet_ctx* ctx, const float* d_packed, int layer, float* d_out, void* stream);

int affnet_probe_hardnet_f43_layer(affnet_ctx* ctx, const float* d_packed, const float* d_patch, int layer, float* d_out, void* stream);
int affnet_probe_hardnet_f43_forward(affnet_ctx* ctx, const float* d_packed, const float* d_patches, int n, float* d_out, float* d_scratch, void* stream);
int affnet_probe_hardnet_f43_u(affnet_ctx* ctx, const float* d_packed, int layer, float* d_out, void* stream);

#ifdef __cplusplus
}
#endif
#endif
```

Baseline: 1.660 million.

## Add polyphase stride-2 conv2/conv4 for OriNet and optional AffNet trunk

Adds a polyphase (Winograd-like) formulation of the stride-2 3x3 conv2 and conv4 layers for the 32x32 trunks, using transformed weights derived alongside the existing Winograd weights. OriNet's fp32 MFMA kernel now uses it by default through a compile-time flag. AffNet gets it as a new shape form, selectable but not the default. The change aims to cut MFMA work in the strided layers, at the cost of extra transform arithmetic, a cross-wave LDS exchange with a barrier, and a larger derived-weight buffer.

Measured after the change: 1.679 million (median of 6 runs). 1.01x the previous value.

```diff
diff --git a/affnet_amd/_lib.py b/affnet_amd/_lib.py
--- a/affnet_amd/_lib.py
+++ b/affnet_amd/_lib.py
@@ -22,7 +22,7 @@
     if int(arith) not in (ARITH_FP32_MFMA, ARITH_FP32_SPLIT3, ARITH_FP32_SPLIT2H):
         raise ValueError("arith must be AFFNET_ARITH_FP32_MFMA (0), AFFNET_ARITH_FP32_SPLIT3 (1) or AFFNET_ARITH_FP32_SPLIT2H (2)")
     return int(arith)
-SHAPE_FORM_DIRECT, SHAPE_FORM_WINOGRAD = 0, 1
+SHAPE_FORM_DIRECT, SHAPE_FORM_WINOGRAD, SHAPE_FORM_POLYPHASE = 0, 1, 2
 DESC_FORM_DIRECT, DESC_FORM_POLYPHASE, DESC_FORM_F43 = 0, 1, 2
 OK, ERR_INVALID, ERR_HIP, ERR_CAPACITY, ERR_EMPTY = 0, -1, -2, -3, -4
 
@@ -148,6 +148,9 @@
     "affnet_probe_shape_offsets": (_I, [_P, C.POINTER(C.c_int64 * 3)]),
     "affnet_probe_affnet_wino_layer": (_I, [_P, _I, _P, _P, _I, _P, _P]),
     "affnet_probe_affnet_wino_partials": (_I, [_P, _P, _P, _I, _P, _P]),
+    "affnet_probe_affnet_poly_layer": (_I, [_P, _I, _P, _P, _I, _P, _P]),
+    "affnet_probe_affnet_poly_partials": (_I, [_P, _P, _P, _I, _P, _P]),
+    "affnet_probe_trunk16_poly_u": (_I, [_P, _I, _P, _I, _P, _P]),
     "affnet_probe_hardnet_poly_layer": (_I, [_P, _P, _P, _I, _P, _P]),
     "affnet_probe_hardnet_poly_forward": (_I, [_P, _P, _P, _I, _P, _P, _P]),
     "affnet_probe_hardnet_poly_u": (_I, [_P, _P, _I, _P, _P]),
diff --git a/affnet_amd/csrc/cnn32.hip b/affnet_amd/csrc/cnn32.hip
--- a/affnet_amd/csrc/cnn32.hip
+++ b/affnet_amd/csrc/cnn32.hip
@@ -28,7 +28,7 @@
     return ctx->arith == AFFNET_ARITH_FP32_SPLIT2H ? 2 : (ctx->arith == AFFNET_ARITH_FP32_SPLIT3 ? 1 : 0);
 }
 
-static int trunk_launch(affnet_ctx* ctx, const CnnCall& c, const NetLayout& L, dim3 grid, bool wino, const int32_t* reeval, int shape_op) {
+static int trunk_launch(affnet_ctx* ctx, const CnnCall& c, const NetLayout& L, dim3 grid, int wino, const int32_t* reeval, int shape_op) {
     CnnArgs a;
     a.packed = c.packed; a.off = to_offsets(L, ctx->arith);
     a.wino_u = nullptr; a.reeval = reeval;
@@ -54,7 +54,7 @@
     static_assert(AFFNET_NET_AFFNET == 0 && AFFNET_NET_ORINET == 1 && AFFNET_NET_HARDNET == 2, "trunk getter order");
     static TrunkKernel (*const trunk_of[3])(int, bool) = {aff_trunk_affnet, aff_trunk_orinet, aff_trunk_hardnet};
     const bool stamps = a.dbg_time || c.dbg_layer >= 0;
-    hipLaunchKernelGGL(wino ? aff_trunk_affnet_wino(stamps) : (poly ? (f43 ? aff_trunk_hardnet_f43(stamps) : aff_trunk_hardnet_poly(stamps)) : trunk_of[c.kind](aff_arith_index(ctx), stamps)), grid, dim3(512), 0, c.st, a, ps);
+    hipLaunchKernelGGL(wino == 2 ? aff_trunk_affnet_poly(stamps) : wino ? aff_trunk_affnet_wino(stamps) : (poly ? (f43 ? aff_trunk_hardnet_f43(stamps) : aff_trunk_hardnet_poly(stamps)) : trunk_of[c.kind](aff_arith_index(ctx), stamps)), grid, dim3(512), 0, c.st, a, ps);
     AFF_LAUNCH_CHECK(ctx);
     return AFFNET_OK;
 }
@@ -66,13 +66,13 @@
     const NetLayout L = net_layout(c.kind);
     const int B = c.patches ? 1 : ctx->B;
     const bool form1 = c.wino_reeval && c.kind == AFFNET_NET_AFFNET && c.fuse && c.dbg_layer < 0 && ctx->arith == AFFNET_ARITH_FP32_MFMA;
-    rc = trunk_launch(ctx, c, L, dim3(rows, B), form1, nullptr, c.shape_op);
+    rc = trunk_launch(ctx, c, L, dim3(rows, B), form1 ? c.wino_reeval : 0, nullptr, c.shape_op);
     if (rc) return rc;
     if (form1) {
         int32_t* flags = reinterpret_cast<int32_t*>(c.scratch + (size_t)B * c.n_max * HEAD_PART_AFF);
         rc = aff_margin_affnet(ctx, c, L, rows, B, flags);
         if (rc) return rc;
-        rc = trunk_launch(ctx, c, L, dim3(rows, B), false, flags, 0);
+        rc = trunk_launch(ctx, c, L, dim3(rows, B), 0, flags, 0);
         if (rc) return rc;
     }
     if (c.dbg_layer < 0 && c.kind != AFFNET_NET_HARDNET) {
@@ -111,7 +111,7 @@
     c.row_begin = row_begin; c.row_count = row_count;
     c.skip_cnt = lazy ? ctx->cnt : nullptr; c.skip_n = ctx->cfg.num_features;
     c.fuse = &sf; c.shape_op = shape_op;
-    c.wino_reeval = ctx->shape_form == AFFNET_SHAPE_FORM_WINOGRAD;
+    c.wino_reeval = ctx->shape_form;
     return cnn_launch(ctx, c);
 }
 
diff --git a/affnet_amd/csrc/cnn_mfma.h b/affnet_amd/csrc/cnn_mfma.h
--- a/affnet_amd/csrc/cnn_mfma.h
+++ b/affnet_amd/csrc/cnn_mfma.h
@@ -1606,3 +1606,94 @@
         step(IntC<S + 1>{}, Vb, Va, Ub);
     });
 }
+
+template <int CIN, int COUT>
+__device__ __forceinline__ int poly16_u_lane(int cb, int G, int lane) {
+    return ((lane >> 4) * COUT + cb * 16 + (lane & 15)) * 16 + G * (16 * COUT * 4);
+}
+template <int CIN, int COUT>
+__device__ __forceinline__ void poly16_prefetch_u(const float* __restrict__ Wu, f32x4 (&Ua)[3], f32x4 (&Ub)[3], int cb, int G, int lane) {
+    const __amdgpu_buffer_rsrc_t r = weight_rsrc(Wu, POLY_XI * CIN * COUT);
+    const int u_lane = poly16_u_lane<CIN, COUT>(cb, G, lane);
+    static_assert(poly_row_np(0) == 3 && poly_row_np(1) == 3, "rows 0 and 1 fill both sets");
+#pragma unroll
+    for (int k = 0; k < 3; ++k) Ua[k] = wino_load_u<CIN, COUT>(r, u_lane, k, 0);
+#pragma unroll
+    for (int k = 0; k < 3; ++k) Ub[k] = wino_load_u<CIN, COUT>(r, u_lane, poly_row_xi0(1) + k, 0);
+}
+
+template <int CIN, int COUT, typename LI>
+__device__ __forceinline__ void conv3x3_poly16_mfma_rows(const float* act, const float* __restrict__ Wu, f32x4 (&Ua)[3], f32x4 (&Ub)[3], f32x4 (&y)[4], int ty, int tx, int cb, int G,
+                                                         int lane) {
+    static_assert(LI::H % 4 == 0 && COUT % 16 == 0 && CIN % 16 == 0, "polyphase tiling");
+    const int kq = lane >> 4;
+    const __amdgpu_buffer_rsrc_t wrsrc = weight_rsrc(Wu, POLY_XI * CIN * COUT);
+    const int u_lane = poly16_u_lane<CIN, COUT>(cb, G, lane);
+    unsigned ab = lds_byte_addr(act) + (((4 * G + kq) * LI::PSG + (4 * ty * LI::WP + 4 * tx) * 4) * 4);
+    asm("" : "+v"(ab));
+    f32x4 t0[5], t1[5], acc[3], da[3], db[3], V[3];
+    poly_read_row<LI, 0>(ab, da, db);
+    poly_transform_row<0>(da, db, V);
+    auto step = [&](auto rc, f32x4 (&U)[3]) {
+        constexpr int R = decltype(rc)::v, R2 = R + 2 < 10 ? R + 2 : R;
+        constexpr int NP = poly_row_np(R), NP2 = R + 2 < 10 ? poly_row_np(R2) : 0, XI2 = poly_row_xi0(R2);
+#pragma unroll
+        for (int k = 0; k < NP; ++k) acc[k] = (f32x4){0.f, 0.f, 0.f, 0.f};
+        __builtin_amdgcn_sched_barrier(0);
+#pragma unroll
+        for (int s4 = 0; s4 < 4; ++s4)
+#pragma unroll
+            for (int k = 0; k < NP; ++k) acc[k] = __builtin_amdgcn_mfma_f32_16x16x4f32(U[k][s4], V[k][s4], acc[k], 0, 0, 0);
+#pragma unroll
+        for (int k = 0; k < NP2; ++k) U[k] = wino_load_u<CIN, COUT>(wrsrc, u_lane, XI2 + k, 0);
+        if constexpr (R < 9) poly_read_row<LI, (R < 9 ? R + 1 : R)>(ab, da, db);
+        __builtin_amdgcn_sched_barrier(0);
+        constexpr int C0 = NP == 3 ? 0 : 3, yi = poly_row_yi(R);
+#pragma unroll
+        for (int j = 0; j < NP; ++j)
+#pragma unroll
+            for (int e = 0; e < 4; ++e) {
+                if constexpr (poly_row_oddy(R)) {
+                    if (yi == 0) t0[C0 + j][e] = acc[j][e];
+                    else if (yi == 1) { t0[C0 + j][e] = wadd(t0[C0 + j][e], acc[j][e]); t1[C0 + j][e] = acc[j][e]; }
+                    else t1[C0 + j][e] = wsub(t1[C0 + j][e], acc[j][e]);
+                } else {
+                    if (yi == 0) t0[C0 + j][e] = wadd(t0[C0 + j][e], acc[j][e]);
+                    else t1[C0 + j][e] = wadd(t1[C0 + j][e], acc[j][e]);
+                }
+            }
+        if constexpr (R == 9) {
+#pragma unroll
+            for (int e = 0; e < 4; ++e) {
+                y[0][e] = wadd(wadd(t0[0][e], t0[1][e]), t0[3][e]);
+                y[1][e] = wadd(wsub(t0[1][e], t0[2][e]), t0[4][e]);
+                y[2][e] = wadd(wadd(t1[0][e], t1[1][e]), t1[3][e]);
+                y[3][e] = wadd(wsub(t1[1][e], t1[2][e]), t1[4][e]);
+            }
+        }
+        if constexpr (R < 9) poly_transform_row<(R < 9 ? R + 1 : R)>(da, db, V);
+    };
+    static_for<5>([&](auto hc) {
+        constexpr int R = 2 * decltype(hc)::v;
+        step(IntC<R>{}, Ua);
+        step(IntC<R + 1>{}, Ub);
+    });
+}
+
+struct Poly16 {
+    static constexpr int X = 8 * LayC3::PSG, X_FLOATS = 8 * 2 * 256;
+};
+__device__ __forceinline__ void poly16_combine(float* lds, const f32x4 (&y)[4], f32x4 (&yo)[2], int wave, int lane) {
+    const int h = wave & 1;
+    float* xw = lds + Poly16::X + (wave * 2 * 64 + lane) * 4;
+    const float* xr = lds + Poly16::X + ((wave ^ 1) * 2 * 64 + lane) * 4;
+#pragma unroll
+    for (int k = 0; k < 2; ++k) *reinterpret_cast<f32x4*>(&xw[k * 256]) = h == 0 ? y[2 + k] : y[k];
+    __syncthreads();
+#pragma unroll
+    for (int k = 0; k < 2; ++k) {
+        const f32x4 o = *reinterpret_cast<const f32x4*>(&xr[k * 256]);
+#pragma unroll
+        for (int e = 0; e < 4; ++e) yo[k][e] = h == 0 ? wadd(y[k][e], o[e]) : wadd(o[e], y[2 + k][e]);
+    }
+}
diff --git a/affnet_amd/csrc/cnn_trunk.h b/affnet_amd/csrc/cnn_trunk.h
--- a/affnet_amd/csrc/cnn_trunk.h
+++ b/affnet_amd/csrc/cnn_trunk.h
@@ -139,6 +139,8 @@
     }
     ori_head_reduce<TM>(w, pbase, part, act, wave, lane);
 }
+
+constexpr bool ORINET_POLY16 = true;
 
 #define CNN_STAMP(k)                                                                                     \
     do {                                                                                                 \
@@ -188,12 +190,13 @@
 
 template <int KIND, int NW, bool STAMPS, int S3 = 0>
 __global__ __launch_bounds__(NW * 64, (KIND == AFFNET_NET_HARDNET) ? NW / 4 : 4) void cnn32_trunk_kernel(CnnArgs a, PyrSrc ps) {
-    static_assert(S3 == 0 || S3 == 2 || S3 == 3 || (S3 == 1 && KIND != AFFNET_NET_ORINET) || (S3 == 4 && KIND == AFFNET_NET_HARDNET),
+    static_assert(S3 == 0 || S3 == 2 || S3 == 3 || (S3 == 1 && KIND != AFFNET_NET_ORINET) || (S3 == 4 && KIND == AFFNET_NET_HARDNET) || (S3 == 5 && KIND == AFFNET_NET_AFFNET),
                   "S3 = number of terms of the split arithmetic; 1 = exact AffNet with Winograd conv1 / conv3 / conv5, exact HardNet with polyphase conv2 / conv4; "
-                  "4 = exact HardNet as 1 with conv3 as Winograd F(4x4, 3x3)");
-    constexpr bool EXACT = S3 <= 1 || S3 == 4;
-    constexpr bool WINO13 = (S3 == 0 && KIND == AFFNET_NET_ORINET) || (S3 == 1 && KIND == AFFNET_NET_AFFNET);
+                  "4 = exact HardNet as 1 with conv3 as Winograd F(4x4, 3x3); 5 = exact AffNet as 1 with polyphase conv2 / conv4");
+    constexpr bool EXACT = S3 <= 1 || S3 == 4 || S3 == 5;
+    constexpr bool WINO13 = (S3 == 0 && KIND == AFFNET_NET_ORINET) || ((S3 == 1 || S3 == 5) && KIND == AFFNET_NET_AFFNET);
     constexpr bool WINO5 = WINO13;
+    constexpr bool POLY16 = (S3 == 0 && KIND == AFFNET_NET_ORINET && ORINET_POLY16) || (S3 == 5 && KIND == AFFNET_NET_AFFNET);
     constexpr bool POLY = (S3 == 1 || S3 == 4) && KIND == AFFNET_NET_HARDNET;
     constexpr bool F43_1 = false;
     constexpr bool F43_3 = S3 == 4 && KIND == AFFNET_NET_HARDNET;
@@ -445,6 +448,8 @@
         f32x4 bias1[T1N];
         f32x4 b3[S::G3][T2N];
         f32x4 bias3[T2N];
+        f32x4 Upa[3], Upb[3];
+        static_assert(!POLY16 || WINO13, "the polyphase stride-2 layers sit between the Winograd stride-1 layers");
         {
             f32x4 acc[T1M][T1N];
             conv0_mfma<NW, CB, T1M, T1N>(patch, w0, bias0, acc, wave, lane);
@@ -463,8 +468,11 @@
             f32x4 y[NB1][4], bw[NB1];
             conv3x3_wino_mfma_rows<NW, CB, CB, LayC0, NB1>(act, a.wino_u, Ur, y, wave, lane);
             CNN_STAMP(3);
-            prefetch_b0<NW, 2 * CB, 16, T2M, T2N, S::G2>(a.packed + a.off.w[2], b2, wave, lane);
-            prefetch_bias<NW, 16, T2M, T2N>(a.packed + a.off.b[2], bias2, wave, lane);
+            if constexpr (POLY16) poly16_prefetch_u<CB, 2 * CB>(a.wino_u + Wino16::offset(2), Upa, Upb, wave & 1, 0, lane);
+            else {
+                prefetch_b0<NW, 2 * CB, 16, T2M, T2N, S::G2>(a.packed + a.off.w[2], b2, wave, lane);
+                prefetch_bias<NW, 16, T2M, T2N>(a.packed + a.off.b[2], bias2, wave, lane);
+            }
             wino_bias<NW, 32, CB, NB1>(a.packed + a.off.b[1], bw, wave, lane);
             __syncthreads();
             CNN_STAMP(21);
@@ -489,7 +497,21 @@
         }
         if (STAMPS && a.dbg_layer == 1) { dump_planes<CB, LayC1, NTHR>(act, a.dbg_out); return; }
 
-        {
+        if constexpr (POLY16) {
+            f32x4 y[1][4], bw[1];
+            int ty, tx, cb;
+            wino_tile<16, 2 * CB, 1>(wave, 0, lane & 15, ty, tx, cb);
+            static_assert((16 / 2) * (16 / 2) / 16 * (2 * CB / 16) == NW, "conv2: one unit per wave");
+            conv3x3_poly16_mfma_rows<CB, 2 * CB, LayC1>(act, a.wino_u + Wino16::offset(2), Upa, Upb, y[0], ty, tx, cb, 0, lane);
+            CNN_STAMP(5);
+            wino_prefetch_u_row<NW, 2 * CB, 2 * CB, 16, NB3>(a.wino_u + Wino16::offset(3), Ur, wave, lane);
+            wino_bias<NW, 16, 2 * CB, 1>(a.packed + a.off.b[2], bw, wave, lane);
+            __syncthreads();
+            zero_halo<LayC2, NTHR>(act, 2 * CB);
+            wino_store_lds<2 * CB, LayC2, 1>(act, bw, y, wave, lane);
+            __syncthreads();
+            CNN_STAMP(6);
+        } else {
             f32x4 acc[T2M][T2N];
             conv3x3_mfma<NW, CB, 2 * CB, LayC1, 2, T2M, T2N, S::G2>(act, a.packed + a.off.w[2], b2, acc, wave, lane);
             CNN_STAMP(5);
@@ -510,8 +532,11 @@
             f32x4 y[NB3][4], bw[NB3];
             conv3x3_wino_mfma_rows<NW, 2 * CB, 2 * CB, LayC2, NB3>(act, a.wino_u + Wino16::offset(3), Ur, y, wave, lane);
             CNN_STAMP(7);
-            prefetch_b0<NW, 4 * CB, 8, T4M, T4N, S::G4>(a.packed + a.off.w[4], b4, wave, lane);
-            prefetch_bias<NW, 8, T4M, T4N>(a.packed + a.off.b[4], bias4, wave, lane);
+            if constexpr (POLY16) poly16_prefetch_u<2 * CB, 4 * CB>(a.wino_u + Wino16::offset(4), Upa, Upb, wave >> 1, wave & 1, lane);
+            else {
+                prefetch_b0<NW, 4 * CB, 8, T4M, T4N, S::G4>(a.packed + a.off.w[4], b4, wave, lane);
+                prefetch_bias<NW, 8, T4M, T4N>(a.packed + a.off.b[4], bias4, wave, lane);
+            }
             wino_bias<NW, 16, 2 * CB, NB3>(a.packed + a.off.b[3], bw, wave, lane);
             __syncthreads();
             zero_halo<LayC3, NTHR>(act, 2 * CB);
@@ -534,7 +559,21 @@
 
         f32x4 b5[S::G5][T4N];
         f32x4 bias5[T4N];
-        {
+        if constexpr (POLY16) {
+            static_assert(Poly16::X >= (2 * CB / 4) * LayC3::PSG && Poly16::X + Poly16::X_FLOATS <= TrunkLds<CB>::TOTAL && (4 * CB / 4) * LayC4::PSG <= Poly16::X,
+                          "polyphase conv4: the exchange lies behind conv3's output inside the LDS array, and conv4's output in front of the exchange");
+            f32x4 y[4], yo[2];
+            conv3x3_poly16_mfma_rows<2 * CB, 4 * CB, LayC3>(act, a.wino_u + Wino16::offset(4), Upa, Upb, y, (lane & 15) >> 2, lane & 3, wave >> 1, wave & 1, lane);
+            CNN_STAMP(24);
+            wino5_prefetch_u(a.wino_u + Wino16::offset(5), Ur, wave, lane);
+            const f32x4 bw = *reinterpret_cast<const f32x4*>(&a.packed[a.off.b[4] + (wave >> 1) * 16 + 4 * (lane >> 4)]);
+            poly16_combine(lds, y, yo, wave, lane);
+            CNN_STAMP(9);
+            zero_halo<LayC4, NTHR>(act, 4 * CB);
+            wino5_store_lds<LayC4::WP, 4, LayC4::PSG>(act + (LayC4::WP + 1) * 4, bw, yo, wave, lane);
+            __syncthreads();
+            CNN_STAMP(10);
+        } else {
             f32x4 acc[T4M][T4N];
             conv3x3_mfma<NW, 2 * CB, 4 * CB, LayC3, 2, T4M, T4N, S::G4>(act, a.packed + a.off.w[4], b4, acc, wave, lane);
             CNN_STAMP(9);
diff --git a/affnet_amd/csrc/cnn_trunk_affnet_poly.hip b/affnet_amd/csrc/cnn_trunk_affnet_poly.hip
--- /dev/null
+++ b/affnet_amd/csrc/cnn_trunk_affnet_poly.hip
@@ -0,0 +1,5 @@
+#include "cnn_trunk.h"
+
+TrunkKernel aff_trunk_affnet_poly(bool stamps) {
+    return stamps ? cnn32_trunk_kernel<AFFNET_NET_AFFNET, 8, true, 5> : cnn32_trunk_kernel<AFFNET_NET_AFFNET, 8, false, 5>;
+}
diff --git a/affnet_amd/csrc/cnn_trunk_orinet.hip b/affnet_amd/csrc/cnn_trunk_orinet.hip
--- a/affnet_amd/csrc/cnn_trunk_orinet.hip
+++ b/affnet_amd/csrc/cnn_trunk_orinet.hip
@@ -1,8 +1,25 @@
 #include "cnn_trunk.h"
 
-__global__ __launch_bounds__(256) void wino_derive_u_kernel(const float* __restrict__ packed, int w1, int w3, int w5, float* __restrict__ U) {
+static_assert(POLY_XI * 16 * 32 == Wino16::P2 && POLY_XI * 32 * 64 == Wino16::P4, "Wino16's polyphase sections hold POLY_XI positions");
+__global__ __launch_bounds__(256) void wino_derive_u_kernel(const float* __restrict__ packed, int w1, int w3, int w5, int w2, int w4, float* __restrict__ U) {
     int e = blockIdx.x * 256 + threadIdx.x;
-    if (e >= Wino16::PAIRS) return;
+    if (e >= Wino16::PAIRS + Wino16::PAIRS_POLY) return;
+    if (e >= Wino16::PAIRS) {
+        e -= Wino16::PAIRS;
+        const int l = e >= 16 * 32 ? 4 : 2;
+        const int cin = 8 * l, cout = 16 * l;
+        const float* src = packed + (l == 4 ? w4 : w2);
+        float* dst = U + Wino16::offset(l);
+        e -= l == 4 ? 16 * 32 : 0;
+        const int n = (e >> 2) % cout, c = (e >> 2) / cout * 4 + (e & 3);
+        float g[9], u[POLY_XI];
+#pragma unroll
+        for (int t = 0; t < 9; ++t) g[t] = src[w_tap_index(t, c, n, cin, cout)];
+        poly_weight_transform(g, u);
+#pragma unroll
+        for (int xi = 0; xi < POLY_XI; ++xi) dst[w_tap_index(xi, c, n, cin, cout)] = u[xi];
+        return;
+    }
     const int l = e >= 256 + 1024 ? 5 : (e >= 256 ? 3 : 1);
     const int ch = 8 << ((l + 1) >> 1);
     const float* src = packed + (l == 5 ? w5 : (l == 3 ? w3 : w1));
@@ -27,7 +44,8 @@
     const int rc = aff_wino_u_ensure(ctx);
     if (rc) return rc;
     float* dst = ctx->wino_u + (size_t)kind * Wino16::FLOATS;
-    hipLaunchKernelGGL(wino_derive_u_kernel, dim3((Wino16::PAIRS + 255) / 256), dim3(256), 0, st, packed, (int)L.w_off[1], (int)L.w_off[3], (int)L.w_off[5], dst);
+    hipLaunchKernelGGL(wino_derive_u_kernel, dim3((Wino16::PAIRS + Wino16::PAIRS_POLY + 255) / 256), dim3(256), 0, st, packed, (int)L.w_off[1], (int)L.w_off[3], (int)L.w_off[5],
+                       (int)L.w_off[2], (int)L.w_off[4], dst);
     AFF_LAUNCH_CHECK(ctx);
     *u = dst;
     return AFFNET_OK;
diff --git a/affnet_amd/csrc/common.h b/affnet_amd/csrc/common.h
--- a/affnet_amd/csrc/common.h
+++ b/affnet_amd/csrc/common.h
@@ -219,11 +219,16 @@
 }
 
 struct Wino16 {
-    static constexpr int U1 = 16 * 16 * 16, U3 = 16 * 32 * 32, U5 = 16 * 64 * 64, FLOATS = U1 + U3 + U5;
+    static constexpr int U1 = 16 * 16 * 16, U3 = 16 * 32 * 32, U5 = 16 * 64 * 64;
     static constexpr int PAIRS = 16 * 16 + 32 * 32 + 64 * 64;
+    static constexpr int P2 = 25 * 16 * 32, P4 = 25 * 32 * 64;
+    static constexpr int PAIRS_POLY = 16 * 32 + 32 * 64;
+    static constexpr int FLOATS = U1 + U3 + U5 + P2 + P4;
     static constexpr int NB1 = 2, NB3 = 1;
-    static constexpr int offset(int layer) { return layer == 1 ? 0 : (layer == 3 ? U1 : U1 + U3); }
-    static constexpr int floats(int layer) { return layer == 1 ? U1 : (layer == 3 ? U3 : U5); }
+    static constexpr int offset(int layer) {
+        return layer == 1 ? 0 : (layer == 3 ? U1 : (layer == 5 ? U1 + U3 : (layer == 2 ? U1 + U3 + U5 : U1 + U3 + U5 + P2)));
+    }
+    static constexpr int floats(int layer) { return layer == 1 ? U1 : (layer == 3 ? U3 : (layer == 5 ? U5 : (layer == 2 ? P2 : P4))); }
 };
 
 struct ShapeFuse {
@@ -244,7 +249,7 @@
     const int32_t* skip_cnt = nullptr; int skip_n = 0;
     const ShapeFuse* fuse = nullptr; int shape_op = 0;
     int desc_form = AFFNET_DESC_FORM_DIRECT;
-    bool wino_reeval = false;
+    int wino_reeval = 0;
     float* rot_lafs = nullptr; const DenormSel* denorm = nullptr;
 };
 
@@ -292,6 +297,7 @@
 TrunkKernel aff_trunk_affnet_wino(bool stamps);
 TrunkKernel aff_trunk_orinet(int arith_index, bool stamps);
 TrunkKernel aff_trunk_hardnet(int arith_index, bool stamps);
+TrunkKernel aff_trunk_affnet_poly(bool stamps);
 TrunkKernel aff_trunk_hardnet_poly(bool stamps);
 int aff_poly_u_ensure(affnet_ctx* ctx);
 int aff_poly_derive_u(affnet_ctx* ctx, const float* packed, const NetLayout& L, hipStream_t st, const float** u);
diff --git a/affnet_amd/csrc/context.hip b/affnet_amd/csrc/context.hip
--- a/affnet_amd/csrc/context.hip
+++ b/affnet_amd/csrc/context.hip
@@ -218,7 +218,7 @@
 
 extern "C" int affnet_set_shape_form(affnet_ctx* ctx, int form) {
     if (!ctx) return AFFNET_ERR_INVALID;
-    if (form != AFFNET_SHAPE_FORM_DIRECT && form != AFFNET_SHAPE_FORM_WINOGRAD) return aff_fail(ctx, AFFNET_ERR_INVALID, "shape form=%d (AFFNET_SHAPE_FORM_*)", form);
+    if (form != AFFNET_SHAPE_FORM_DIRECT && form != AFFNET_SHAPE_FORM_WINOGRAD && form != AFFNET_SHAPE_FORM_POLYPHASE) return aff_fail(ctx, AFFNET_ERR_INVALID, "shape form=%d (AFFNET_SHAPE_FORM_*)", form);
     ctx->shape_form = form;
     return AFFNET_OK;
 }
diff --git a/affnet_amd/csrc/debug.hip b/affnet_amd/csrc/debug.hip
--- a/affnet_amd/csrc/debug.hip
+++ b/affnet_amd/csrc/debug.hip
@@ -73,7 +73,7 @@
     return AFFNET_OK;
 }
 
-static int probe_affnet_wino(affnet_ctx* ctx, const float* d_packed, const float* d_patches, int n, float* d_out, int layer, hipStream_t st) {
+static int probe_affnet_wino(affnet_ctx* ctx, const float* d_packed, const float* d_patches, int n, float* d_out, int layer, hipStream_t st, bool poly = false) {
     if (ctx->arith != AFFNET_ARITH_FP32_MFMA) return aff_fail(ctx, AFFNET_ERR_INVALID, "probe_affnet_wino: AFFNET_ARITH_FP32_MFMA only");
     const NetLayout L = net_layout(AFFNET_NET_AFFNET);
     CnnArgs a;
@@ -84,7 +84,7 @@
     a.patches = d_patches; a.n_max = n; a.out = d_out; a.dbg_layer = layer; a.dbg_out = d_out; a.dbg_time = ctx->dbg_time;
     PyrSrc ps;
     memset(&ps, 0, sizeof(ps));
-    hipLaunchKernelGGL(aff_trunk_affnet_wino(layer >= 0 || a.dbg_time), dim3(n, 1), dim3(512), 0, st, a, ps);
+    hipLaunchKernelGGL(poly ? aff_trunk_affnet_poly(layer >= 0 || a.dbg_time) : aff_trunk_affnet_wino(layer >= 0 || a.dbg_time), dim3(n, 1), dim3(512), 0, st, a, ps);
     AFF_LAUNCH_CHECK(ctx);
     return AFFNET_OK;
 }
@@ -100,6 +100,29 @@
     AFF_DEVICE(ctx);
     if (!ctx || !d_packed || !d_patches || !d_partials || n < 1 || n > 65535) return aff_fail(ctx, AFFNET_ERR_INVALID, "probe_affnet_wino_partials: bad argument");
     return probe_affnet_wino(ctx, d_packed, d_patches, n, d_partials, -1, (hipStream_t)stream);
+}
+
+extern "C" int affnet_probe_affnet_poly_layer(affnet_ctx* ctx, int net_kind, const float* d_packed, const float* d_patch, int layer, float* d_out, void* stream) {
+    AFF_DEVICE(ctx);
+    if (!ctx || !d_packed || !d_patch || !d_out || net_kind != AFFNET_NET_AFFNET || layer < 0 || layer > 5)
+        return aff_fail(ctx, AFFNET_ERR_INVALID, "probe_affnet_poly_layer: AffNet, layer 0 .. 5");
+    return probe_affnet_wino(ctx, d_packed, d_patch, 1, d_out, layer, (hipStream_t)stream, true);
+}
+
+extern "C" int affnet_probe_affnet_poly_partials(affnet_ctx* ctx, const float* d_packed, const float* d_patches, int n, float* d_partials, void* stream) {
+    AFF_DEVICE(ctx);
+    if (!ctx || !d_packed || !d_patches || !d_partials || n < 1 || n > 65535) return aff_fail(ctx, AFFNET_ERR_INVALID, "probe_affnet_poly_partials: bad argument");
+    return probe_affnet_wino(ctx, d_packed, d_patches, n, d_partials, -1, (hipStream_t)stream, true);
+}
+
+extern "C" int affnet_probe_trunk16_poly_u(affnet_ctx* ctx, int net_kind, const float* d_packed, int layer, float* d_out, void* stream) {
+    AFF_DEVICE(ctx);
+    if (!ctx || !d_packed || !d_out || (net_kind != AFFNET_NET_AFFNET && net_kind != AFFNET_NET_ORINET) || (layer != 2 && layer != 4))
+        return aff_fail(ctx, AFFNET_ERR_INVALID, "probe_trunk16_poly_u: AffNet / OriNet, layer 2 or 4");
+    const float* u;
+    const int rc = aff_wino_derive_u(ctx, net_kind, d_packed, net_layout(net_kind), (hipStream_t)stream, &u);
+    if (rc) return rc;
+    return aff_copy_async(ctx, d_out, u + Wino16::offset(layer), (size_t)Wino16::floats(layer) * sizeof(float), (hipStream_t)stream);
 }
 
 extern "C" int affnet_probe_hardnet_poly_layer(affnet_ctx* ctx, const float* d_packed, const float* d_patch, int layer, float* d_out, void* stream) {
diff --git a/include/affnet_hip.h b/include/affnet_hip.h
--- a/include/affnet_hip.h
+++ b/include/affnet_hip.h
@@ -70,6 +70,7 @@
 
 #define AFFNET_SHAPE_FORM_DIRECT 0
 #define AFFNET_SHAPE_FORM_WINOGRAD 1
+#define AFFNET_SHAPE_FORM_POLYPHASE 2
 int affnet_set_shape_form(affnet_ctx* ctx, int form);
 int affnet_get_shape_form(const affnet_ctx* ctx);
 
diff --git a/include/affnet_hip_probes.h b/include/affnet_hip_probes.h
--- a/include/affnet_hip_probes.h
+++ b/include/affnet_hip_probes.h
@@ -20,6 +20,10 @@
 
 int affnet_probe_affnet_wino_partials(affnet_ctx* ctx, const float* d_packed, const float* d_patches, int n, float* d_partials, void* stream);
 
+int affnet_probe_affnet_poly_layer(affnet_ctx* ctx, int net_kind, const float* d_packed, const float* d_patch, int layer, float* d_out, void* stream);
+int affnet_probe_affnet_poly_partials(affnet_ctx* ctx, const float* d_packed, const float* d_patches, int n, float* d_partials, void* stream);
+int affnet_probe_trunk16_poly_u(affnet_ctx* ctx, int net_kind, const float* d_packed, int layer, float* d_out, void* stream);
+
 int affnet_probe_hardnet_poly_layer(affnet_ctx* ctx, const float* d_packed, const float* d_patch, int layer, float* d_out, void* stream);
 int affnet_probe_hardnet_poly_forward(affnet_ctx* ctx, const float* d_packed, const float* d_patches, int n, float* d_out, float* d_scratch, void* stream);
 int affnet_probe_hardnet_poly_u(affnet_ctx* ctx, const float* d_packed, int layer, float* d_out, void* stream);
```
